# fmidev/RoadSurf

Measured on AMD Instinct MI355X. Metric: point_timesteps_per_s, higher is better.
Workload: dtype f64

## Files before the change

### roadsurf_amd/csrc/rs_cluster.hip

```cpp
#include <hip/hip_runtime.h>
#include <hipcub/hipcub.hpp>

#include <algorithm>

#include "rs_ens_table.hpp"
#include "rs_group_rule.hpp"
#include "rs_kernels.h"
#include "rs_state.h"

namespace {

constexpr int KEY_BITS = RS_SORT_KEY_BITS;

template <typename T>
__global__ void __launch_bounds__(RS_BLOCK) keys_kernel(const T *__restrict__ state,
                                                        int64_t np_pad, int64_t npoints,
                                                        uint32_t *keys, uint32_t *slots) {
  const int64_t s = (int64_t)blockIdx.x * RS_BLOCK + threadIdx.x;
  if (s >= npoints) return;
  double v = (double)state[(int64_t)RS_ST_BLSCORE * np_pad + s];
  if (!(v >= 0.0)) v = 0.0;
  const double top = (double)((1u << KEY_BITS) - 1u);
  keys[s] = (uint32_t)top - (uint32_t)(v > top ? top : v);
  slots[s] = (uint32_t)s;
// ... 783 lines not shown
}
}

int32_t rs_cluster_ens_waves(const RsEnsSpec *sp) {
  if (rs_ens::cols(sp) < 0) return -1;
  const int32_t entries = 64 * sp->max_members * (int32_t)(sizeof(int32_t) + sizeof(uint16_t)),
                row = ENS_ROW * sp->max_members * (int32_t)sizeof(double);
  return std::max(1, std::min(ENS_MAX_WAVES, (ENS_LDS_BUDGET - entries) / row));
}

size_t rs_cluster_ens_lds_bytes(const RsEnsSpec *sp) {
  const int32_t waves = rs_cluster_ens_waves(sp);
  if (waves < 0) return 0;
  return (size_t)sp->max_members * ((size_t)waves * ENS_ROW * sizeof(double) + 64 * (sizeof(int32_t) + sizeof(uint16_t)));
}

hipError_t rs_cluster_outputs_ens(const void *const src[6], bool f32, const int32_t *table, const int32_t *inv,
                                  int64_t npoints, int64_t src_stride, int32_t nrows, const RsEnsSpec &spec,
                                  double *acc_row0, hipStream_t stream) {
  const int32_t waves = rs_cluster_ens_waves(&spec);
  if (waves < 0 || nrows < 1 || npoints < 1) return hipErrorInvalidValue;
  EnsArgs a;
  for (int f = 0; f < 6; ++f) a.src[f] = src[f];
  a.table = table;
  a.inv = inv;
  a.acc = acc_row0;
  a.npoints = npoints;
  a.stride = src_stride;
  a.nrows = nrows;
  a.ngroups = spec.ngroups;
  a.max_members = spec.max_members;
  a.nquant = spec.nquant;
  a.cols = rs_ens::cols(&spec);
  a.waves = waves;
  for (int j = 0; j < RS_ENS_MAX_QUANT; ++j) a.quant[j] = j < spec.nquant ? spec.quant[j] : 0.0;
  const int64_t station_blocks = ((int64_t)spec.ngroups + 63) / 64;
  const int64_t want_row_blocks = std::max<int64_t>(1, 6144 / station_blocks);
  const int64_t rows_each = std::max<int64_t>(1, ((int64_t)nrows + want_row_blocks - 1) / want_row_blocks);
  a.rows_per_block = (int32_t)std::min<int64_t>(INT32_MAX / 2, (rows_each + waves - 1) / waves * waves);
  const int64_t row_blocks = ((int64_t)nrows + a.rows_per_block - 1) / a.rows_per_block;
  const dim3 grid((unsigned)station_blocks, (unsigned)row_blocks);
  const size_t lds = rs_cluster_ens_lds_bytes(&spec);
  if (f32)
    hipLaunchKernelGGL(ens_stats_kernel<float>, grid, dim3(64 * waves), lds, stream, a);
  else
    hipLaunchKernelGGL(ens_stats_kernel<double>, grid, dim3(64 * waves), lds, stream, a);
  return hipGetLastError();
}

int32_t rs_cluster_prob_cols(const RsProbSpec *sp) {
  if (!sp || sp->ngroups < 1 || sp->max_members < 1 || sp->max_members > RS_ENS_MAX_MEMBERS || sp->nconds < 1 ||
      sp->nconds > RS_PROB_MAX_CONDS)
    return -1;
  for (int32_t c = 0; c < sp->nconds; ++c) {
    const RsProbCond &k = sp->cond[c];
    if (k.use <= 0 || (k.use >> RS_EPI_VARS) != 0) return -1;
    for (int v = 0; v < RS_EPI_VARS; ++v)
      if (k.above[v] != k.above[v] || k.below[v] != k.below[v]) return -1;
  }
  return 1 + 2 * sp->nconds;
}

int32_t rs_cluster_prob_needs_deficit(const RsProbSpec *sp) {
  if (rs_cluster_prob_cols(sp) < 0) return -1;
  for (int32_t c = 0; c < sp->nconds; ++c)
    if ((sp->cond[c].use >> 6) & 1) return 1;
  return 0;
}

namespace {
constexpr int PROB_ROWS = 4;
constexpr int PROB_WAVES = 4;
constexpr int PROB_WORDS = 4;

struct ProbBitsArgs {
  const void *src[RS_EPI_VARS];
  const int32_t *order;
  int32_t *ever;
  uint32_t *words;
  int64_t npoints, stride, wstride;
  int32_t nrows, nconds;
  RsProbCond cond[RS_PROB_MAX_CONDS];
};

template <typename T>
__global__ void __launch_bounds__(RS_BLOCK) prob_bits_kernel(const ProbBitsArgs a) {
  const int64_t s = (int64_t)blockIdx.x * RS_BLOCK + threadIdx.x;
  if (s >= a.npoints) return;
  const int64_t p = a.order ? (int64_t)a.order[s] : s;
  const bool own = p >= 0 && p < a.npoints;
  uint32_t ever = own ? (uint32_t)a.ever[p] : 0u;
  const bool with_deficit = a.src[6] != nullptr;
#pragma unroll 1
  for (int32_t r0 = 0; r0 < a.nrows; r0 += PROB_ROWS) {
    T x[PROB_ROWS][RS_EPI_VARS];
#pragma unroll
    for (int q = 0; q < PROB_ROWS; ++q) {
      const int32_t r = r0 + q < a.nrows ? r0 + q : a.nrows - 1;
#pragma unroll
      for (int f = 0; f < 6; ++f) x[q][f] = static_cast<const T *>(a.src[f])[(int64_t)r * a.stride + s];
      x[q][6] = with_deficit ? static_cast<const T *>(a.src[6])[(int64_t)r * a.stride + s] : (T)0;
    }
#pragma unroll
    for (int q = 0; q < PROB_ROWS; ++q) {
      if (r0 + q >= a.nrows) break;
      const double v[RS_EPI_VARS] = {(double)x[q][0], (double)x[q][1], (double)x[q][2], (double)x[q][3],
                                     (double)x[q][4], (double)x[q][5], (double)x[q][6]};
      const bool valid = v[0] != -9999.0;
      uint32_t now = 0;
#pragma unroll
      for (int c = 0; c < RS_PROB_MAX_CONDS; ++c) {
        if (c >= a.nconds) break;
        const int32_t use = a.cond[c].use;
        bool ok = valid;
#pragma unroll
        for (int k = 0; k < RS_EPI_VARS; ++k)
          if ((use >> k) & 1) ok = ok && a.cond[c].above[k] < v[k] && v[k] < a.cond[c].below[k];
        if ((use >> 6) & 1) ok = ok && v[6] != -9999.0;
        now |= (ok ? 1u : 0u) << c;
      }
      ever |= now;
      a.words[(int64_t)(r0 + q) * a.wstride + s] = valid ? (now | ((ever & 0xffu) << 8) | (1u << 16)) : 0u;
    }
  }
  if (own) a.ever[p] = (int32_t)ever;
}

struct ProbCountArgs {
  const uint32_t *words;
  const int32_t *table;
  const int32_t *inv;
  double *acc;
  int64_t npoints, wstride;
  int32_t nrows, ngroups, max_members, nconds, cols, rows_per_block;
};

__global__ void __launch_bounds__(64 * PROB_WAVES) prob_count_kernel(const ProbCountArgs a) {
  extern __shared__ int32_t prob_slot[];
  const int lane = threadIdx.x & 63, wave = threadIdx.x >> 6;
  const int64_t g = (int64_t)blockIdx.x * 64 + lane;
  const bool live = g < a.ngroups;
  int32_t first = 0, cnt = 0;
  if (live) {
    const int64_t s0 = a.table[g], s1 = a.table[g + 1];
    if (s0 >= 0 && s0 < a.npoints && s1 > s0) {
      int64_t c = s1 - s0;
      if (c > a.max_members) c = a.max_members;
      if (c > a.npoints - s0) c = a.npoints - s0;
      first = (int32_t)s0;
      cnt = (int32_t)c;
    }
  }
  int32_t incl = cnt;
#pragma unroll
  for (int d = 1; d < 64; d <<= 1) {
    const int32_t u = __shfl_up(incl, d, 64);
    if (lane >= d) incl += u;
  }
  const int32_t off = incl - cnt;
  const int32_t *entry = a.table + ((int64_t)a.ngroups + 1);
  for (int32_t j = wave; j < cnt; j += PROB_WAVES) {
    const int64_t p = entry[(int64_t)first + j];
    int32_t s = -1;
    if (p >= 0 && p < a.npoints) {
      const int64_t q = a.inv[p];
      if (q >= 0 && q < a.npoints) s = (int32_t)q;
    }
    prob_slot[off + j] = s;
  }
  __syncthreads();

  const int32_t r_lo = (int32_t)blockIdx.y * a.rows_per_block,
                r_hi = a.nrows - r_lo < a.rows_per_block ? a.nrows : r_lo + a.rows_per_block;
  const int32_t *mine = prob_slot + off;
#pragma unroll 1
  for (int32_t r = r_lo + wave; r < r_hi; r += PROB_WAVES) {
    const uint32_t *w = a.words + (int64_t)r * a.wstride;
    int32_t nvalid = 0, now[RS_PROB_MAX_CONDS], by[RS_PROB_MAX_CONDS];
#pragma unroll
    for (int c = 0; c < RS_PROB_MAX_CONDS; ++c) now[c] = by[c] = 0;
    for (int32_t j0 = 0; j0 < cnt; j0 += PROB_WORDS) {
      uint32_t x[PROB_WORDS];
#pragma unroll
      for (int q = 0; q < PROB_WORDS; ++q) {
        const int32_t s = j0 + q < cnt ? mine[j0 + q] : -1;
        x[q] = s >= 0 ? w[s] : 0u;
      }
#pragma unroll
      for (int q = 0; q < PROB_WORDS; ++q) {
        nvalid += (int32_t)((x[q] >> 16) & 1u);
#pragma unroll
        for (int c = 0; c < RS_PROB_MAX_CONDS; ++c) {
          if (c >= a.nconds) break;
          now[c] += (int32_t)((x[q] >> c) & 1u);
          by[c] += (int32_t)((x[q] >> (8 + c)) & 1u);
        }
      }
    }
    if (live) {
      double *cell = a.acc + ((int64_t)r * a.ngroups + g) * a.cols;
      cell[0] = (double)nvalid;
#pragma unroll
      for (int c = 0; c < RS_PROB_MAX_CONDS; ++c) {
        if (c >= a.nconds) break;
        cell[1 + c] = (double)now[c];
        cell[1 + a.nconds + c] = (double)by[c];
      }
    }
  }
}
}

hipError_t rs_cluster_outputs_prob(const void *const src[6], const void *deficit, bool f32, const int32_t *order,
                                   const int32_t *table, const int32_t *inv, int64_t npoints, int64_t src_stride,
                                   int32_t nrows, const RsProbSpec &spec, int32_t *ever, uint32_t *words,
                                   int64_t wstride, double *acc_row0, hipStream_t stream) {
  const int32_t cols = rs_cluster_prob_cols(&spec);
  if (cols < 0 || nrows < 1 || npoints < 1 || wstride < npoints) return hipErrorInvalidValue;
  ProbBitsArgs b;
  for (int f = 0; f < 6; ++f) b.src[f] = src[f];
  b.src[6] = rs_cluster_prob_needs_deficit(&spec) == 1 ? deficit : nullptr;
  b.order = order;
  b.ever = ever;
  b.words = words;
  b.npoints = npoints;
  b.stride = src_stride;
  b.wstride = wstride;
  b.nrows = nrows;
  b.nconds = spec.nconds;
  for (int c = 0; c < RS_PROB_MAX_CONDS; ++c) b.cond[c] = spec.cond[c < spec.nconds ? c : 0];
  if (f32)
    hipLaunchKernelGGL(prob_bits_kernel<float>, grid1(npoints), dim3(RS_BLOCK), 0, stream, b);
  else
    hipLaunchKernelGGL(prob_bits_kernel<double>, grid1(npoints), dim3(RS_BLOCK), 0, stream, b);
  if (hipError_t e = hipGetLastError(); e != hipSuccess) return e;
  ProbCountArgs a;
  a.words = words;
  a.table = table;
  a.inv = inv;
  a.acc = acc_row0;
  a.npoints = npoints;
  a.wstride = wstride;
  a.nrows = nrows;
  a.ngroups = spec.ngroups;
  a.max_members = spec.max_members;
  a.nconds = spec.nconds;
  a.cols = cols;
  const int64_t station_blocks = ((int64_t)spec.ngroups + 63) / 64;
  const int64_t want_row_blocks = std::max<int64_t>(1, 6144 / station_blocks);
  const int64_t rows_each = std::max<int64_t>(1, ((int64_t)nrows + want_row_blocks - 1) / want_row_blocks);
  a.rows_per_block = (int32_t)std::min<int64_t>(INT32_MAX / 2, (rows_each + PROB_WAVES - 1) / PROB_WAVES * PROB_WAVES);
  const int64_t row_blocks = ((int64_t)nrows + a.rows_per_block - 1) / a.rows_per_block;
  const dim3 grid((unsigned)station_blocks, (unsigned)row_blocks);
  const size_t lds = (size_t)64 * spec.max_members * sizeof(int32_t);
  hipLaunchKernelGGL(prob_count_kernel, grid, dim3(64 * PROB_WAVES), lds, stream, a);
  return hipGetLastError();
}

hipError_t rs_cluster_identity(int32_t *order, int64_t np_pad, hipStream_t stream) {
  hipLaunchKernelGGL(iota_kernel, grid1(np_pad), dim3(RS_BLOCK), 0, stream, order, np_pad);
  return hipGetLastError();
}

size_t rs_cluster_scratch_bytes(int64_t npoints) {
  size_t bytes = 0;
  uint32_t *k = nullptr;
  (void)hipcub::DeviceRadixSort::SortPairs(nullptr, bytes, k, k, k, k, (int)npoints, 0, KEY_BITS);
  return bytes;
}

hipError_t rs_cluster_sort(const double *state, bool f32, int64_t np_pad, int64_t npoints,
                           uint32_t *scratch, void *tmp, size_t tmp_bytes, hipStream_t stream) {
  uint32_t *kin = scratch, *kout = scratch + np_pad, *sin = scratch + 2 * np_pad,
           *sout = scratch + 3 * np_pad;
  if (f32)
    hipLaunchKernelGGL(keys_kernel<float>, grid1(npoints), dim3(RS_BLOCK), 0, stream,
                       reinterpret_cast<const float *>(state), np_pad, npoints, kin, sin);
  else
    hipLaunchKernelGGL(keys_kernel<double>, grid1(npoints), dim3(RS_BLOCK), 0, stream, state, np_pad,
                       npoints, kin, sin);
  hipError_t e = hipGetLastError();
  if (e != hipSuccess) return e;
  return hipcub::DeviceRadixSort::SortPairs(tmp, tmp_bytes, kin, kout, sin, sout, (int)npoints, 0,
                                            KEY_BITS, stream);
}

namespace {
constexpr int CS_TILE = 1024;

__device__ __forceinline__ uint32_t wave_incl_scan(uint32_t v, uint32_t lane) {
#pragma unroll
  for (int off = 1; off < 64; off <<= 1) {
    const uint32_t u = (uint32_t)__shfl_up((int)v, off, 64);
    if (lane >= (uint32_t)off) v += u;
  }
  return v;
}

__global__ void __launch_bounds__(256) cs_hist_kernel(const uint32_t *__restrict__ keys,
                                                      const uint32_t *__restrict__ via, int64_t n, int shift,
                                                      int nbins, int ntiles, uint32_t *__restrict__ H) {
  __builtin_amdgcn_s_setprio(3);
  extern __shared__ uint32_t cs_h[];
  for (int b = threadIdx.x; b < nbins; b += 256) cs_h[b] = 0u;
  __syncthreads();
  const int64_t base = (int64_t)blockIdx.x * CS_TILE;
  for (int i = threadIdx.x; i < CS_TILE; i += 256) {
    const int64_t idx = base + i;
    if (idx < n) atomicAdd(&cs_h[(keys[via ? (int64_t)via[idx] : idx] >> shift) & (uint32_t)(nbins - 1)], 1u);
  }
  __syncthreads();
  for (int b = threadIdx.x; b < nbins; b += 256) H[(int64_t)blockIdx.x * nbins + b] = cs_h[b];
}

__global__ void __launch_bounds__(64) cs_binscan_kernel(uint32_t *H, uint32_t *T, int nbins, int ntiles,
                                                        uint32_t *class_total, int class_shift) {
  __builtin_amdgcn_s_setprio(3);
  const int bin = (int)blockIdx.x * 64 + (int)threadIdx.x;
  uint32_t run = 0u;
  if (bin < nbins) {
#pragma unroll 8
    for (int t = 0; t < ntiles; ++t) {
      const uint32_t v = H[(int64_t)t * nbins + bin];
      H[(int64_t)t * nbins + bin] = run;
      run += v;
    }
    T[bin] = run;
  }
  if (class_total) {
    uint32_t sum = run;
#pragma unroll
    for (int off = 32; off > 0; off >>= 1) sum += (uint32_t)__shfl_xor((int)sum, off, 64);
    if (threadIdx.x == 0 && (int)blockIdx.x * 64 < nbins) atomicAdd(&class_total[((int)blockIdx.x * 64) >> class_shift], sum);
  }
}

__global__ void __launch_bounds__(64) cs_scatter_kernel(const uint32_t *__restrict__ keys,
                                                        const uint32_t *__restrict__ via, int64_t n,
                                                        int shift, int nbits, int ntiles,
                                                        const uint32_t *__restrict__ H,
                                                        const uint32_t *__restrict__ T,
                                                        uint32_t *__restrict__ perm_out) {
  __builtin_amdgcn_s_setprio(3);
  extern __shared__ uint32_t cs_cur[];
  const int nbins = 1 << nbits;
  const uint32_t lane = threadIdx.x;
  const int64_t base = (int64_t)blockIdx.x * CS_TILE;
  {
    constexpr int ROWS = 16;
    uint32_t carry = 0u;
    for (int r0 = 0; r0 < nbins; r0 += 64 * ROWS) {
      uint32_t tv[ROWS], hv[ROWS];
#pragma unroll
      for (int q = 0; q < ROWS; ++q) {
        const int b = r0 + q * 64 + (int)lane;
        tv[q] = b < nbins ? T[b] : 0u;
        hv[q] = b < nbins ? H[(int64_t)blockIdx.x * nbins + b] : 0u;
      }
#pragma unroll
      for (int q = 0; q < ROWS; ++q) {
        const int b = r0 + q * 64 + (int)lane;
        const uint32_t incl = wave_incl_scan(tv[q], lane);
        if (b < nbins) cs_cur[b] = carry + incl - tv[q] + hv[q];
        carry += (uint32_t)__shfl((int)incl, 63, 64);
      }
    }
  }
  __syncthreads();
  constexpr int CS_BATCH = 8;
  for (int r0 = 0; r0 < CS_TILE / 64; r0 += CS_BATCH) {
    if (base + (int64_t)r0 * 64 >= n) break;
    uint32_t kreg[CS_BATCH], sreg[CS_BATCH];
#pragma unroll
    for (int q = 0; q < CS_BATCH; ++q) {
      const int64_t idx = base + (int64_t)(r0 + q) * 64 + lane;
      sreg[q] = (idx < n && via) ? via[idx] : (uint32_t)idx;
    }
#pragma unroll
    for (int q = 0; q < CS_BATCH; ++q) {
      const int64_t idx = base + (int64_t)(r0 + q) * 64 + lane;
      kreg[q] = idx < n ? ((keys[sreg[q]] >> shift) & (uint32_t)(nbins - 1)) : 0u;
    }
#pragma unroll
  for (int q = 0; q < CS_BATCH; ++q) {
    const int64_t idx = base + (int64_t)(r0 + q) * 64 + lane;
    const bool valid = idx < n;
    const uint32_t key = kreg[q];
    unsigned long long same = __ballot(valid);
    for (int bit = 0; bit < nbits; ++bit) {
      const bool one = (key >> bit) & 1u;
      const unsigned long long b = __ballot(one);
      same &= one ? b : ~b;
    }
    const uint32_t rank = (uint32_t)__popcll(same & ((1ull << lane) - 1ull));
    uint32_t start = 0u;
    if (valid) {
      start = cs_cur[key];
      perm_out[start + rank] = sreg[q];
    }
    __builtin_amdgcn_wave_barrier();
    if (valid && rank == 0u) cs_cur[key] = start + (uint32_t)__popcll(same);
    __builtin_amdgcn_wave_barrier();
  }
  }
}
}

__global__ void __launch_bounds__(64) cs_wave_table_kernel(uint32_t *__restrict__ class_total,
                                                           int class_bits, int32_t *__restrict__ wstart,
                                                           int32_t *__restrict__ wcnt, int32_t maxw) {
  __builtin_amdgcn_s_setprio(3);
  const uint32_t lane = threadIdx.x;
  const int nclasses = 1 << class_bits;
  uint32_t n = 0u;
  if ((int)lane < nclasses) {
    n = class_total[lane];
    class_total[lane] = 0u;
  }
  const uint32_t waves = (n + 63u) >> 6;
  const uint32_t sbase = wave_incl_scan(n, lane) - n, wbase = wave_incl_scan(waves, lane) - waves;
  uint32_t total = 0u;
  for (int c = 0; c < nclasses; ++c) {
    const uint32_t nc = (uint32_t)__shfl((int)n, c, 64), sb = (uint32_t)__shfl((int)sbase, c, 64),
                   wb = (uint32_t)__shfl((int)wbase, c, 64), wc = (nc + 63u) >> 6;
    for (uint32_t k = lane; k < wc; k += 64u) {
      const uint32_t idx = wb + k;
      if ((int32_t)idx < maxw) {
        wstart[idx] = (int32_t)(sb + 64u * k);
        const uint32_t left = nc - 64u * k;
        wcnt[idx] = (int32_t)(left < 64u ? left : 64u);
      }
    }
    total = wb + wc;
  }
  for (uint32_t idx = total + lane; (int32_t)idx < maxw; idx += 64u) {
    wstart[idx] = 0;
    wcnt[idx] = 0;
  }
}

hipError_t rs_cluster_wave_table(int class_bits, uint32_t *class_total, int32_t *wstart, int32_t *wcnt,
                                 int32_t maxw, hipStream_t stream) {
  if (class_bits < 1 || class_bits > 6 || !class_total) return hipErrorInvalidValue;
  hipLaunchKernelGGL(cs_wave_table_kernel, dim3(1), dim3(64), 0, stream, class_total, class_bits, wstart, wcnt, maxw);
  return hipGetLastError();
}

size_t rs_cluster_count_scratch_bytes(int64_t npoints, int nbits) {
  const int64_t ntiles = (npoints + CS_TILE - 1) / CS_TILE;
  return ((size_t)(1 << nbits) * (size_t)ntiles + (size_t)(1 << nbits)) * sizeof(uint32_t);
}

hipError_t rs_cluster_count_sort(int64_t np_pad, int64_t npoints, int nbits, uint32_t *scratch, void *tmp,
                                 size_t tmp_bytes, hipStream_t stream, uint32_t *class_total, int class_bits,
                                 int low_bits) {
  if (nbits < 1 || nbits > 12 || low_bits < 0 || low_bits > 12 ||
      tmp_bytes < rs_cluster_count_scratch_bytes(npoints, nbits > low_bits ? nbits : low_bits))
    return hipErrorInvalidValue;
  const int ntiles = (int)((npoints + CS_TILE - 1) / CS_TILE);
  uint32_t *H = static_cast<uint32_t *>(tmp);
  const uint32_t *via = nullptr;
  if (low_bits > 0) {
    const int nb = 1 << low_bits;
    uint32_t *T = H + (size_t)nb * ntiles;
    hipLaunchKernelGGL(cs_hist_kernel, dim3(ntiles), dim3(256), nb * sizeof(uint32_t), stream, scratch, via,
                       npoints, 0, nb, ntiles, H);
    hipLaunchKernelGGL(cs_binscan_kernel, dim3((nb + 63) / 64), dim3(64), 0, stream, H, T, nb, ntiles,
                       (uint32_t *)nullptr, 0);
    hipLaunchKernelGGL(cs_scatter_kernel, dim3(ntiles), dim3(64), nb * sizeof(uint32_t), stream, scratch, via,
                       npoints, 0, low_bits, ntiles, H, T, scratch + np_pad);
    via = scratch + np_pad;
  }
  const int nbins = 1 << nbits;
  uint32_t *T = H + (size_t)nbins * ntiles;
  hipLaunchKernelGGL(cs_hist_kernel, dim3(ntiles), dim3(256), nbins * sizeof(uint32_t), stream, scratch, via,
                     npoints, low_bits, nbins, ntiles, H);
  const bool classes = class_total && class_bits >= 1 && nbits - class_bits >= 6;
  hipLaunchKernelGGL(cs_binscan_kernel, dim3((nbins + 63) / 64), dim3(64), 0, stream, H, T, nbins, ntiles,
                     classes ? class_total : nullptr, nbits - class_bits);
  hipLaunchKernelGGL(cs_scatter_kernel, dim3(ntiles), dim3(64), nbins * sizeof(uint32_t), stream, scratch, via,
                     npoints, low_bits, nbits, ntiles, H, T, scratch + 3 * np_pad);
  return hipGetLastError();
}

hipError_t rs_cluster_sort_keys(int64_t np_pad, int64_t npoints, uint32_t *scratch, void *tmp,
                                size_t tmp_bytes, hipStream_t stream) {
  uint32_t *kin = scratch, *kout = scratch + np_pad, *sin = scratch + 2 * np_pad,
           *sout = scratch + 3 * np_pad;
  return hipcub::DeviceRadixSort::SortPairs(tmp, tmp_bytes, kin, kout, sin, sout, (int)npoints, 0,
                                            KEY_BITS, stream);
}

namespace {
__global__ void __launch_bounds__(RS_BLOCK) again_flags_kernel(const double *__restrict__ state,
                                                               int64_t np_pad, int64_t npoints,
                                                               int32_t *flags, int32_t *iota) {
  const int64_t p = (int64_t)blockIdx.x * RS_BLOCK + threadIdx.x;
  if (p >= npoints) return;
  flags[p] = ((int32_t)state[(int64_t)RS_ST_CPL_FLAGS * np_pad + p]) & 1;
  iota[p] = (int32_t)p;
}
}

size_t rs_cpl_select_scratch_bytes(int64_t npoints) {
  size_t bytes = 0;
  int32_t *x = nullptr;
  (void)hipcub::DeviceSelect::Flagged(nullptr, bytes, x, x, x, x, (int)npoints);
  return bytes;
}

hipError_t rs_cpl_select_again(const double *state, int64_t np_pad, int64_t npoints, int32_t *flags,
                               int32_t *list, int32_t *count_dev, void *tmp, size_t tmp_bytes,
                               hipStream_t stream) {
  int32_t *iota = flags + npoints;
  hipLaunchKernelGGL(again_flags_kernel, grid1(npoints), dim3(RS_BLOCK), 0, stream, state, np_pad,
                     npoints, flags, iota);
  hipError_t e = hipGetLastError();
  if (e != hipSuccess) return e;
  return hipcub::DeviceSelect::Flagged(tmp, tmp_bytes, iota, flags, list, count_dev, (int)npoints, stream);
}

static RowMap row_map(int nlayers, int cpl_rows) {
  RowMap rows;
  rows.nlayers = nlayers;
  rows.nscal = RS_ST_BLSCORE - RS_ST_TNW1 + 1;
  rows.ncpl = cpl_rows >= 1 ? RS_ST_CPL_RESUME - RS_ST_CPL_ITER + 1 : 0;
  rows.nsave = cpl_rows >= 2 ? RS_ST_CPL_SAVE_ALBEDO - RS_ST_CPL_SAVE_TSURF + 1 : 0;
  return rows;
}

hipError_t rs_cluster_inverse(const int32_t *order, int64_t npoints, int32_t *inv, hipStream_t stream) {
  hipLaunchKernelGGL(inverse_kernel, grid1(npoints), dim3(RS_BLOCK), 0, stream, order, npoints, inv);
  return hipGetLastError();
}

hipError_t rs_cluster_fanout(const double *state_src, double *state_dst, bool f32, const int32_t *order_dst,
                             const int32_t *parent, const int32_t *inv_src, int64_t np_pad_src, int64_t npoints_src,
                             int64_t np_pad_dst, int64_t npoints_dst, int nlayers, int cpl_rows, hipStream_t stream) {
  dim3 g = grid1(npoints_dst);
  const RowMap rows = row_map(nlayers, cpl_rows);
  g.y = (unsigned)rows.total();
  if (f32)
    hipLaunchKernelGGL(fanout_kernel<float>, g, dim3(RS_BLOCK), 0, stream, reinterpret_cast<const float *>(state_src),
                       reinterpret_cast<float *>(state_dst), order_dst, parent, inv_src, np_pad_src, npoints_src,
                       np_pad_dst, npoints_dst, rows);
  else
    hipLaunchKernelGGL(fanout_kernel<double>, g, dim3(RS_BLOCK), 0, stream, state_src, state_dst, order_dst, parent,
                       inv_src, np_pad_src, npoints_src, np_pad_dst, npoints_dst, rows);
  return hipGetLastError();
}

hipError_t rs_cluster_apply(const double *state_src, double *state_dst, bool f32,
                            const int32_t *order_src, int32_t *order_dst, const uint32_t *perm,
                            int64_t np_pad, int64_t npoints, int nlayers, int cpl_rows,
                            hipStream_t stream) {
  dim3 g = grid1(np_pad);
  const RowMap rows = row_map(nlayers, cpl_rows);
  g.y = (unsigned)rows.total();
  if (f32)
    hipLaunchKernelGGL(apply_kernel<float>, g, dim3(RS_BLOCK), 0, stream,
                       reinterpret_cast<const float *>(state_src), reinterpret_cast<float *>(state_dst),
                       order_src, order_dst, perm, np_pad, npoints, rows);
  else
    hipLaunchKernelGGL(apply_kernel<double>, g, dim3(RS_BLOCK), 0, stream, state_src, state_dst,
                       order_src, order_dst, perm, np_pad, npoints, rows);
  return hipGetLastError();
}
```

### roadsurf_amd/csrc/rs_kernels.h

```cpp
#pragma once
#include <hip/hip_runtime.h>
#include <cstddef>
#include <type_traits>
#include "../../include/roadsurf.h"
#include "rs_synth.h"
#include "rs_raw.hpp"
#include "rs_step_select.hpp"

namespace rs {

struct Writeback {
  double *sw, *sw_dir, *lw;
  int64_t t_stride;
};

struct StepArgs {
  const void *consts = nullptr;
  RsForcing f{};
  RsOutputs o{};
  RsPointParams pp{};
  double *state = nullptr;
  int64_t npoints = 0, np_pad = 0;
  int32_t t0 = 0, nsteps = 0;
  Writeback wb{};
  const int32_t *cpl_list = nullptr;
  int32_t cpl_nlist = 0, cpl_stop = 0;
  int32_t cpl_inner = 0, cpl_prio = 0;
  const int32_t *out_index = nullptr;
  const int32_t *wave_start = nullptr, *wave_cnt = nullptr;
  int32_t wave_n = 0;
  int32_t knots_tdew = 0;
  int32_t surface_prio = 0;
  const double *knots = nullptr;
  const int32_t *knot_gather = nullptr;
  int32_t knot_k0 = 0, knot_n = 0, spk = 0, start_hour = 0;
  double r_spk = 0.0;
  RawForcing raw{};
  double *diag = nullptr;
};
static_assert(std::is_trivially_copyable<StepArgs>::value, "StepArgs is a kernel argument");
static_assert(sizeof(StepArgs) == 912 && offsetof(StepArgs, f) == 8 && offsetof(StepArgs, o) == 136 &&
                  offsetof(StepArgs, pp) == 208 && offsetof(StepArgs, state) == 328 && offsetof(StepArgs, t0) == 352 &&
                  offsetof(StepArgs, wb) == 360 && offsetof(StepArgs, cpl_list) == 392 &&
                  offsetof(StepArgs, out_index) == 416 && offsetof(StepArgs, wave_n) == 440 &&
                  offsetof(StepArgs, knots_tdew) == 444 && offsetof(StepArgs, surface_prio) == 448 &&
                  offsetof(StepArgs, knots) == 456 && offsetof(StepArgs, r_spk) == 488 &&
                  offsetof(StepArgs, raw) == 496 && offsetof(StepArgs, diag) == 904,
              "the kernels' view of StepArgs");

struct InitArgs {
  const void *consts;
  RsForcing f;
  RsPointParams pp;
  double *state;
  int64_t npoints, np_pad;
};

struct ForecastArgs {
  const void *consts;
  const void *state;
  int32_t f32;
  int64_t npoints, np_pad;
  RsPreview pv;
  uint32_t *keys, *slots;
  int32_t compact;
  int32_t low_bits;
  int32_t extra_log;
};

struct KnotArgs {
  RsSynthSpec spec;
  double *knots;
  int64_t npoints, np_pad;
  int32_t k0, nknots;
};

struct ExpandArgs {
  RsForcing f;
  const double *knots;
  int64_t npoints, np_pad;
  int32_t k0, t0, spk, start_hour;
  int32_t kfirst, nsteps;
  double r_spk;
  const int32_t *gather;
};

}

hipError_t rs_read_div_mismatch(unsigned long long *out , hipStream_t stream);
hipError_t rs_read_div_samples(double *out , hipStream_t stream);
hipError_t rs_read_bl_stats(unsigned long long *out , hipStream_t stream);
hipError_t rs_launch_math_test(int fn, int64_t n, const double *x, double *y, hipStream_t stream);
hipError_t rs_launch_humidity_fill(const double *tair, double *tdew, double *rhz, int64_t n,
                                   hipStream_t stream);
hipError_t rs_upload_math_tables(hipStream_t stream);
hipError_t rs_launch_step(const rs::StepArgs &a, const rs::StepLaunch &l, hipStream_t stream);
struct RsPlan;
int rs_cpl_replay_raw(RsPlan *pl, const rs::RawForcing *raw, const RsOutputs *o, const RsPointParams *pp,
                      int32_t t0, int32_t nsteps, bool out_by_point, int32_t *rounds);
uint64_t rs_a32_limit(void);
bool rs_step_raw_ok(const RsPlan *pl);
int rs_step_raw(RsPlan *pl, const rs::RawForcing *raw, const double *sun, const RsOutputs *o,
                const RsPointParams *pp, int32_t t0, int32_t nsteps, bool out_by_point);
hipError_t rs_launch_cpl_window_bounds(const rs::StepArgs &a, int32_t *out, hipStream_t stream);
size_t rs_cpl_select_scratch_bytes(int64_t npoints);
hipError_t rs_cpl_select_again(const double *state, int64_t np_pad, int64_t npoints, int32_t *flags,
                               int32_t *list, int32_t *count_dev, void *tmp, size_t tmp_bytes,
                               hipStream_t stream);
hipError_t rs_launch_init(const rs::InitArgs &a, hipStream_t stream);
hipError_t rs_launch_knots(const rs::KnotArgs &a, int32_t nknots, hipStream_t stream);
hipError_t rs_launch_expand(const rs::ExpandArgs &a, int32_t nintervals, hipStream_t stream);
#define RS_CLOCK_PROBE_MAX_US 10000u
hipError_t rs_launch_clock_probe(uint64_t *out, uint32_t spin_us, hipStream_t stream);
hipError_t rs_launch_count_failed(const double *st, int64_t np_pad, int64_t npoints,
                                  unsigned long long *out, hipStream_t stream);

hipError_t rs_launch_forecast_keys(const rs::ForecastArgs &a, hipStream_t stream);

#define RS_SORT_KEY_BITS 24
hipError_t rs_cluster_identity(int32_t *order, int64_t np_pad, hipStream_t stream);
hipError_t rs_cluster_outputs_by_point(const double *const src[6], double *const dst[6], const int32_t *order,
                                       int64_t npoints, int64_t src_stride, int32_t nrows, int64_t dst_rows,
                                       int64_t dst_row0, hipStream_t stream);
hipError_t rs_cluster_summary_reset(double *acc, int64_t np_pad, hipStream_t stream);
hipError_t rs_cluster_outputs_summary(const void *const src[6], bool f32, const int32_t *order, int64_t npoints,
                                      int64_t src_stride, int32_t nrows, int32_t index0, int32_t index_step,
                                      const RsSummarySpec &spec, double *acc, int64_t np_pad, hipStream_t stream);
int32_t rs_cluster_group_cols(const RsGroupSpec *spec);
int32_t rs_cluster_group_path(const RsGroupSpec *spec);
hipError_t rs_cluster_group_reset(double *acc, int64_t acc_rows, const RsGroupSpec &spec, hipStream_t stream);
hipError_t rs_cluster_outputs_groups(const void *const src[6], bool f32, const int32_t *order, const int32_t *group,
                                     int64_t npoints, int64_t src_stride, int32_t nrows, const RsGroupSpec &spec,
                                     double *acc_row0, hipStream_t stream);
int32_t rs_cluster_ens_waves(const RsEnsSpec *spec);
size_t rs_cluster_ens_lds_bytes(const RsEnsSpec *spec);
hipError_t rs_cluster_outputs_ens(const void *const src[6], bool f32, const int32_t *table, const int32_t *inv,
                                  int64_t npoints, int64_t src_stride, int32_t nrows, const RsEnsSpec &spec,
                                  double *acc_row0, hipStream_t stream);
int32_t rs_cluster_episode_cols(const RsEpisodeSpec *spec);
hipError_t rs_cluster_episodes_reset(double *acc, int64_t np_pad, const RsEpisodeSpec &spec, hipStream_t stream);
hipError_t rs_cluster_outputs_episodes(const void *const src[6], const void *deficit, bool f32, const int32_t *order,
                                       int64_t npoints, int64_t src_stride, int32_t nrows, int32_t index0,
                                       int32_t index_step, const RsEpisodeSpec &spec, double *acc, int64_t np_pad,
                                       hipStream_t stream);
hipError_t rs_cluster_episodes_finish(double *acc, int64_t npoints, int64_t np_pad, const RsEpisodeSpec &spec,
                                      hipStream_t stream);
int32_t rs_cluster_prob_cols(const RsProbSpec *spec);
int32_t rs_cluster_prob_needs_deficit(const RsProbSpec *spec);
hipError_t rs_cluster_outputs_prob(const void *const src[6], const void *deficit, bool f32, const int32_t *order,
                                   const int32_t *table, const int32_t *inv, int64_t npoints, int64_t src_stride,
                                   int32_t nrows, const RsProbSpec &spec, int32_t *ever, uint32_t *words,
                                   int64_t wstride, double *acc_row0, hipStream_t stream);
hipError_t rs_grid_gather(const double *src, int32_t nrows, int64_t n_nodes, int64_t src_stride, const int32_t *node,
                          const double *weight, int32_t stencil, const int32_t *order, double present_above,
                          double missing, double *dst, int64_t dst_stride, int64_t npoints, hipStream_t stream);
size_t rs_cluster_scratch_bytes(int64_t npoints);
hipError_t rs_cluster_sort(const double *state, bool f32, int64_t np_pad, int64_t npoints,
                           uint32_t *scratch, void *tmp, size_t tmp_bytes, hipStream_t stream);
hipError_t rs_cluster_sort_keys(int64_t np_pad, int64_t npoints, uint32_t *scratch, void *tmp,
                                size_t tmp_bytes, hipStream_t stream);
size_t rs_cluster_count_scratch_bytes(int64_t npoints, int nbits);
hipError_t rs_cluster_wave_table(int class_bits, uint32_t *class_total, int32_t *wstart, int32_t *wcnt,
                                 int32_t maxw, hipStream_t stream);
hipError_t rs_cluster_count_sort(int64_t np_pad, int64_t npoints, int nbits, uint32_t *scratch, void *tmp,
                                 size_t tmp_bytes, hipStream_t stream, uint32_t *class_total = nullptr,
                                 int class_bits = 0, int low_bits = 0);
int rs_forecast_key_bits(int32_t mode);
int rs_forecast_key_low_bits(int32_t mode);
hipError_t rs_cluster_apply(const double *state_src, double *state_dst, bool f32,
                            const int32_t *order_src, int32_t *order_dst, const uint32_t *perm,
                            int64_t np_pad, int64_t npoints, int nlayers, int cpl_rows,
                            hipStream_t stream);
hipError_t rs_cluster_inverse(const int32_t *order, int64_t npoints, int32_t *inv, hipStream_t stream);
hipError_t rs_cluster_fanout(const double *state_src, double *state_dst, bool f32, const int32_t *order_dst,
                             const int32_t *parent, const int32_t *inv_src, int64_t np_pad_src, int64_t npoints_src,
                             int64_t np_pad_dst, int64_t npoints_dst, int nlayers, int cpl_rows, hipStream_t stream);

size_t rs32_constants_bytes(void);
hipError_t rs32_upload_constants(void *dst, const RsConstants *c, hipStream_t stream);
hipError_t rs32_launch_step(const rs::StepArgs &a, const rs::StepLaunch &l, hipStream_t stream);
hipError_t rs32_launch_init(const rs::InitArgs &a, hipStream_t stream);
hipError_t rs32_launch_expand(const rs::ExpandArgs &a, int32_t nintervals, hipStream_t stream);
```

### roadsurf_amd/csrc/rs_kernels.hip

```cpp
#include <hip/hip_runtime.h>
#include <cstdlib>
#include "rs_physics.hpp"
#include "rs_state.h"
#include "rs_synth.h"
#include "rs_kernels.h"

#ifndef RS_CPL_WAVES
#define RS_CPL_WAVES 2
#endif
#ifndef RS_REGIME_WINDOW
#define RS_REGIME_WINDOW 30
#endif

namespace rs {

constexpr int kBlock = RS_BLOCK;

typedef RsConstantsDev __attribute__((address_space(4))) ConstsAS;
template <class Args>
__device__ __forceinline__ const ConstsAS &consts_of(Args a) {
  return *(const ConstsAS *)a->consts;
}

template <int NL, int NREG>
// ... 206 lines not shown
      dg[(int64_t)RS_DG_MAXIT_OLD * np + p] = old;
      dg[(int64_t)RS_DG_MAXIT_BL * np + p] = x.BLCond;
    }
    dg[(int64_t)RS_DG_MAXIT_N * np + p] = n + 1.0;
  }
}

#include "rs_general_body.inc"

template <bool FULL, class Prof, bool SKY = false, bool SCORE = true, bool CPL = false,
          bool REPLAY = false, bool A32 = false, bool DIAG = false>
__device__ __forceinline__ void time_loop(const MathTab &mt, Prof &T, Scalars &s, int32_t &score,
                                          uint32_t point = 0u) {
  static_assert(!A32 || (!SKY && !CPL), "32-bit window offsets: the plain lock-step kernels only");
  static_assert(FULL || !SKY, "sky view belongs to the FULL feature set");
  static_assert(FULL || !CPL, "coupling belongs to the FULL feature set");
  static_assert(CPL || !REPLAY, "replays belong to coupling");
  KernArgs ka = kernargs();
  const uint32_t lane = REPLAY ? point : threadIdx.x;
  const int64_t row0 = REPLAY ? 0 : (int64_t)blockIdx.x * kBlock;
  const int32_t nsteps = ka->nsteps, t0 = ka->t0;
  const double tbot = (ka->pp.tbottom + row0)[lane];
  SkyPoint sky;
  if (SKY) sky = sky_point(ka, row0, lane);
  const bool sky_on = sky.on;
  int32_t initlen = 0;
  bool relax = false;
  double relax_dt = 0, relax_dv = 0, relax_dr = 0;
  if (FULL) {
    initlen = ka->pp.initlen ? (ka->pp.initlen + row0)[lane] : 0;
    if (consts_of(ka).use_relaxation && ka->pp.tair_relax) {
      double tairR, vzR, rhR;
      relax_targets(ka, row0, lane, tairR, vzR, rhR);
      relax = !(tairR < R4(-100.0) || tairR > R4(100.0) || vzR < R4(0.0) || vzR > R4(100.0) ||
                rhR < R4(0.0) || rhR > 110);
      relax_dt = tairR - s.tair_end;
      relax_dv = vzR - s.vz_end;
      relax_dr = rhR - s.rh_end;
    }
  }

  auto fail_at = [&](int32_t idx) {
    s.failed = true;
    ka->state[(int64_t)RS_ST_FAILED * ka->np_pad + row0 + lane] = (double)idx;
  };
  CplWindow cw;
  if (CPL) cpl_window(ka, consts_of(ka), row0, lane, cw);
  const bool cpl_on = cw.on;
  const int32_t cpl_cs = cw.cs, cpl_ce = cw.ce;
  bool parked = false;
  int32_t next_i = t0;
  double cpl_lastobs = 0.0, cpl_swcorr = 0.0, cpl_lwcorr = 0.0;
  if (CPL) {
    double *st = ka->state;
    const int64_t np = ka->np_pad, p = row0 + lane;
    cpl_lastobs = st[(int64_t)RS_ST_CPL_LASTOBS * np + p];
    cpl_swcorr = st[(int64_t)RS_ST_CPL_SWCORR * np + p];
    cpl_lwcorr = st[(int64_t)RS_ST_CPL_LWCORR * np + p];
    parked = (((int32_t)st[(int64_t)RS_ST_CPL_FLAGS * np + p]) & 1) != 0;
    next_i = (int32_t)st[(int64_t)RS_ST_CPL_RESUME * np + p];
    if (REPLAY) {
      parked = false;
      next_i = cpl_cs;
    }
  }
  double r_swcof = R4(1.0), r_lwcof = R4(1.0);
  bool stale_now = false;
  auto blank_rows = [&](int32_t i_from) {
    for (int32_t ii = i_from; ii < t0 + nsteps; ++ii) {
      int64_t r;
      if (output_row<false>(ka, ii, r)) store_outputs<false, false>(ka, r, row0, lane, s, false);
    }
  };
  if (!CPL && s.failed) blank_rows(t0);
  Forcing nxt = load_forcing<FULL, A32>(ka, row0, lane, 0);
  for (int32_t kv = 0; kv < nsteps; ++kv) {
    asm volatile("" : "+s"(ka));
    const ConstsAS &c = consts_of(ka);
    const int32_t k = __builtin_amdgcn_readfirstlane(kv);
    const int32_t i = t0 + k;
    const Forcing f = nxt;
    int64_t orow = 0;
    const bool owrite = output_row<true>(ka, i, orow);

    if (CPL && (parked || i != next_i)) {
      if (k + 1 < nsteps) nxt = load_forcing<FULL, A32>(ka, row0, lane, k + 1);
      continue;
    }
    if (CPL) next_i = i + 1;
    if (s.failed) {
      if (CPL && owrite && (!REPLAY || i > cpl_ce)) store_outputs<CPL, A32>(ka, orow, row0, lane, s, false);
      continue;
    }
    double tair = f.tair, vz = f.vz, rhz = f.rhz;
    s.tnw1 = T.get(1);
    s.tnw2 = T.get(2);
    if (i == 1 && vz < R4(0.4)) vz = R4(0.4);
    const double prec_ts = RS_DIVC(f.prec, 3600.0, r_3600) * c.DTSecs;

    double sw_dir = 0.0, lw_net = 0.0;
    if (SKY) {
      const int64_t row = (int64_t)k * ka->f.t_stride + row0;
      const LaneOff L(lane);
      sw_dir = L.ld(ka->f.sw_dir + row);
      lw_net = L.ld(ka->f.lw_net + row);
    }
    CouplingInputs cp;
    if (i < c.SimLen) {
      if (REPLAY && i == cpl_cs) {
        const Forcing g = gather_forcing(ka, row0 + lane, cpl_ce + 1, t0);
        if (check_values(c, g, s.tsurf, FULL && ka->f.tdew != nullptr)) fail_at(cpl_ce + 1);
      } else {
        Forcing chk = f;
        chk.vz = vz;
        if (check_values(c, chk, s.tsurf, FULL && ka->f.tdew != nullptr)) fail_at(i);
      }
      if (SKY) {
        if (REPLAY && i == cpl_cs) {
          if (sky_on) {
            const int64_t off = (int64_t)(cpl_ce + 1 - t0) * ka->f.t_stride + row0 + lane;
            if (sky_limits_bad(ka->f.sw_dir[off], ka->f.lw_net[off])) fail_at(cpl_ce + 1);
          }
        } else if (sky_on && sky_limits_bad(sw_dir, lw_net))
          fail_at(i);
        sw_dir = sky_clamp_direct(sw_dir, f.sw);
      }
      if (CPL && cpl_on) {
        cp.in_phase = (i >= cpl_cs && i <= cpl_ce);
        if (REPLAY && i == cpl_cs) cp.in_phase = false;
        if (REPLAY && i == cpl_cs) {
          double *st = ka->state;
          const int64_t np = ka->np_pad, p = row0 + lane;
          cpl_restore_surface<true>(st, np, p, s);
          const int N = T.nlayers();
          for (int j = 1; j <= N; ++j) {
            st[(int64_t)(RS_ST_CPL_STALE_TMP0 + j - 1) * np + p] = T.get(j);
            T.set(j, st[(int64_t)(RS_ST_CPL_SAVE_TMP0 + j - 1) * np + p]);
          }
          stale_now = true;
          cpl_rewind_coefs(st[(int64_t)RS_ST_CPL_RADCOEFF * np + p], f.sw, f.lw, SKY && sky_on, r_swcof, r_lwcof);
          st[(int64_t)RS_ST_CPL_SWCOF * np + p] = r_swcof;
          st[(int64_t)RS_ST_CPL_LWCOF * np + p] = r_lwcof;
        }
        if (!REPLAY && i == cpl_cs) {
          double *st = ka->state;
          const int64_t np = ka->np_pad, p = row0 + lane;
          cpl_save_surface(st, np, p, s);
          const int N = T.nlayers();
          for (int j = 1; j <= N; ++j) st[(int64_t)(RS_ST_CPL_SAVE_TMP0 + j - 1) * np + p] = T.get(j);
        }
        if (i > cpl_ce) cpl_decayed_coefs(c, mt, i, cpl_ce, cpl_swcorr, cpl_lwcorr, cp.sw_cof, cp.lw_cof);
        if (REPLAY && i >= cpl_cs && i <= cpl_ce) {
          cp.sw_cof = r_swcof;
          cp.lw_cof = r_lwcof;
        }
        if (cp.in_phase) snow_ice_check(c, cpl_lastobs, s);
      }
      if (FULL) {
        if ((i <= initlen || c.force_tsurf) && f.tsurfobs > R4(-100.0) &&
            (!CPL || !cpl_on || i < cpl_cs)) {
          T.set(1, f.tsurfobs);
          T.set(2, f.tsurfobs);
          const double depth = (c.tsurfOutputDepth >= R4(0.0)) ? c.tsurfOutputDepth : f.depth;
          s.tsurf = surface_temperature(c, T, tbot, depth);
        }
        if (relax) {
          if (i == initlen) {
            double tairR, vzR, rhR;
            relax_targets(ka, row0, lane, tairR, vzR, rhR);
            relax_dt = tairR - tair;
            relax_dv = vzR - vz;
            relax_dr = rhR - rhz;
            double *st = ka->state;
            const int64_t np = ka->np_pad, p = row0 + lane;
            st[(int64_t)RS_ST_TAIR_END * np + p] = tair;
            st[(int64_t)RS_ST_VZ_END * np + p] = vz;
            st[(int64_t)RS_ST_RH_END * np + p] = rhz;
          }
          if (i > initlen) relax_apply(relax_factor(c, mt, i, initlen), relax_dt, relax_dv, relax_dr, tair, vz, rhz);
        }
      }
    } else {
      if (FULL) s.tsurf = surface_temperature(c, T, tbot, f.depth);
      if (CPL && cpl_on) cpl_last_values(c, mt, cw, cpl_swcorr, cpl_lwcorr, ka->state, ka->np_pad, row0 + lane, cp);
    }
    if (CPL) cp.last_tsurf_obs = cpl_lastobs;
    double sw_in = f.sw, lw_in = f.lw;
    if (SKY && sky_on) {
      int64_t hstride;
      const double *hrow = horizon_row(ka, sky.hcol, hstride);
      if (!sky_view_radiation(ka->f.sun + (int64_t)k * RS_SUN_COLS, sky.sinlat, sky.coslat, sky.lonrad, sky.coslon,
                              sky.sinlon, sky.skyv, ka->pp.albedo_surroundings, hrow, hstride, sw_in, sw_dir, lw_in, lw_net))
        fail_at(i);
    }
    if (SKY) sky_write_back(ka, k, row0, sky_on, sw_dir, sw_in, lw_in, [&](double *base, double v) { base[lane] = v; });
    if (DIAG)
      bl_diagnose(&c, mt.expT, mt.logT, mt.K, s.tsurf, tair, vz, rhz, f.hour, i, ka->diag, ka->np_pad, row0 + lane);
    const Fluxes fx =
        model_step_fluxes<SCORE>(c, mt, s, tair, vz, rhz, prec_ts, sw_in, lw_in, f.phase, f.hour, cp);
    if (SCORE) {
      score += (fx.trips & 63) - 5;
      if ((fx.trips & 64) && k >= nsteps - RS_REGIME_WINDOW) score |= 1 << 30;
    }
    if (k + 1 < nsteps) nxt = load_forcing<FULL, A32>(ka, row0, lane, k + 1);
    if (REPLAY) {
      const GlobalProfile Tstale{ka->state + (int64_t)RS_ST_CPL_STALE_TMP0 * ka->np_pad + row0 + lane,
                                 ka->np_pad};
      model_step_ground<Prof, GlobalProfile>(c, s, T, tbot, tair, fx, f.depth, cp,
                                             stale_now ? &Tstale : nullptr);
      stale_now = false;
    } else {
      model_step_ground<Prof, Prof, FULL>(c, s, T, tbot, tair, fx, f.depth, cp);
    }
    if (owrite) store_outputs<CPL, A32>(ka, orow, row0, lane, s, true);
    if (!CPL && s.failed) blank_rows(i + 1);
    if (CPL && cpl_on && i < c.SimLen && i == cpl_ce)
      cpl_window_end(ka->state, ka->np_pad, row0 + lane, cw, s, cpl_swcorr, cpl_lwcorr, cpl_lastobs, parked);
  }
  if (CPL) ka->state[(int64_t)RS_ST_CPL_RESUME * ka->np_pad + row0 + lane] = (double)next_i;
}

__device__ __forceinline__ double bl_score_key(int32_t score, const Scalars &s) {
  const int32_t extra = score & 0x3fffffff;
  const int32_t lo = extra > 0x7ffff ? 0x7ffff : extra;
  const int32_t covered = (s.wat > 0.0 || s.snow > 0.0 || s.ice > 0.0 || s.ice2 > 0.0 || s.dep > 0.0) ? 1 : 0;
  return (double)(lo | (covered << 19) | (((score >> 30) & 1) << 20));
}

template <int NL>
__device__ __forceinline__ void lane_profile(RegProfile<NL> &, double *, const StepArgs &) {}
template <int NL, int NREG>
__device__ __forceinline__ void lane_profile(HybridProfile<NL, NREG> &T, double *lds, const StepArgs &) {
  T.col = lds + threadIdx.x;
}
__device__ __forceinline__ void lane_profile(LdsProfile &T, double *lds, const StepArgs &a) {
  T.col = lds + threadIdx.x;
  T.n = consts_of(&a).NLayers;
}

template <class Prof, bool FULL, bool SKY = false, bool SCORE = true, bool CPL = false, bool REPLAY = false,
          bool A32 = false, bool DIAG = false>
__device__ __forceinline__ void step_lanes(const StepArgs &a, double *math_lds, double *prof_lds) {
  const MathTab mt = fill_math_tables(math_lds);
  __syncthreads();
  const int64_t g = (int64_t)blockIdx.x * kBlock + threadIdx.x;
  if (g >= (REPLAY ? (int64_t)a.cpl_nlist : a.npoints)) return;
  const int64_t p = REPLAY ? (int64_t)a.cpl_list[g] : g;
  if (REPLAY && a.cpl_prio) __builtin_amdgcn_s_setprio(2);
  Prof T;
  lane_profile(T, prof_lds, a);
  Scalars s;
  int32_t score = 0;
#ifdef RS_WAVE_TIMING
  constexpr bool WT = !FULL && std::is_same<Prof, RegProfile<15>>::value;
  const uint64_t wt0 = WT ? __builtin_amdgcn_s_memrealtime() : 0;
#endif
  for (int32_t rnd = 0;; ++rnd) {
    load_state<FULL>(a.state, a.np_pad, p, T, s);
    time_loop<FULL, Prof, SKY, SCORE, CPL, REPLAY, A32, DIAG>(mt, T, s, score, REPLAY ? (uint32_t)p : 0u);
    store_state<FULL>(a.state, a.np_pad, p, T, s);
    if (!REPLAY || rnd + 1 >= a.cpl_inner) break;
    if ((((int32_t)a.state[(int64_t)RS_ST_CPL_FLAGS * a.np_pad + p]) & 1) == 0) break;
  }
  if (SCORE) a.state[(int64_t)RS_ST_BLSCORE * a.np_pad + p] = bl_score_key(score, s);
#ifdef RS_WAVE_TIMING
  if (WT) {
    a.state[(int64_t)RS_ST_VZ_END * a.np_pad + p] = (double)(wt0 & 0xffffffffffffull);
    a.state[(int64_t)RS_ST_RH_END * a.np_pad + p] = (double)(__builtin_amdgcn_s_memrealtime() & 0xffffffffffffull);
  }
#endif
}

template <int NL, bool FULL, bool SCORE = true, bool A32 = false>
__global__ void __launch_bounds__(kBlock, FULL ? 3 : 4) step_kernel_reg(const StepArgs a) {
  __shared__ double math_lds[RS_MATH_LDS_DOUBLES];
  step_lanes<RegProfile<NL>, FULL, false, SCORE, false, false, A32>(a, math_lds, nullptr);
}

#ifndef RS_HYBRID_REG
#define RS_HYBRID_REG 7
#endif
template <bool SCORE, bool A32>
__global__ void __launch_bounds__(kBlock, 4) step_kernel_hybrid(const StepArgs a) {
  __shared__ double math_lds[RS_MATH_LDS_DOUBLES];
  __shared__ double prof_lds[(15 - RS_HYBRID_REG) * kBlock];
  step_lanes<HybridProfile<15, RS_HYBRID_REG>, true, false, SCORE, false, false, A32>(a, math_lds, prof_lds);
}

template <bool FULL, bool DIAG = false>
__global__ void __launch_bounds__(kBlock, 4) step_kernel_lds(const StepArgs a) {
  extern __shared__ double lds[];
  __shared__ double math_lds[RS_MATH_LDS_DOUBLES];
  step_lanes<LdsProfile, FULL, false, true, false, false, false, DIAG>(a, math_lds, lds);
}

#ifdef RS_EAIR_SURFACE
enum { PR_TAIR = 0, PR_VZ, PR_RHZ, PR_RAIN, PR_SNOW, PR_AVC, PR_SW, PR_LW, PR_OBS, PR_LEAN = PR_OBS, PR_FULL = PR_OBS + 1 };
#else
enum { PR_TAIR = 0, PR_VZ, PR_RHZ, PR_RAIN, PR_SNOW, PR_AVC, PR_EAIR, PR_SW, PR_LW, PR_OBS, PR_LEAN = PR_OBS, PR_FULL = PR_OBS + 1 };
#endif
template <int NPREP>
struct DuoMailT {
  double v[2][2][64];
  uint32_t failed[64];
  double prep[2][NPREP][64];
  uint32_t prep_bad[2][64];
};

template <bool FULL, bool SKYG = false, class Mail>
__device__ __forceinline__ void duo_put_prep(Mail &mail, int buf, uint32_t lane, const ForcingPrep &q) {
  double (*w)[64] = mail.prep[buf];
  w[PR_TAIR][lane] = q.tair; w[PR_VZ][lane] = q.vz; w[PR_RHZ][lane] = q.rhz; w[PR_RAIN][lane] = q.rain;
  w[PR_SNOW][lane] = q.snow;
  w[PR_AVC][lane] = q.AirHCap * q.AirDens;
#ifndef RS_EAIR_SURFACE
  w[PR_EAIR][lane] = q.EAir;
#endif
  if (!SKYG) {
    w[PR_SW][lane] = q.sw;
    w[PR_LW][lane] = q.lw;
  }
  if (FULL) w[PR_OBS][lane] = q.tsurfobs;
  mail.prep_bad[buf][lane] = (q.bad ? 1u : 0u) | (q.night ? 2u : 0u) | (q.bad_rw ? 8u : 0u);
}
template <bool FULL, bool SKYG = false, class C, class Mail>
__device__ __forceinline__ ForcingPrep duo_get_prep(const C &c, const Mail &mail, int buf, uint32_t lane,
                                                    const uint32_t *skyfl = nullptr) {
  const double (*w)[64] = mail.prep[buf];
  ForcingPrep q;
  q.tair = w[PR_TAIR][lane]; q.vz = w[PR_VZ][lane]; q.rhz = w[PR_RHZ][lane]; q.rain = w[PR_RAIN][lane];
  q.snow = w[PR_SNOW][lane];
  const double AirVCap = w[PR_AVC][lane];
  q.AirVCap = AirVCap;
#ifndef RS_EAIR_SURFACE
  q.EAir = w[PR_EAIR][lane];
#endif
  q.sw = w[PR_SW][lane]; q.lw = w[PR_LW][lane];
  if (FULL) q.tsurfobs = w[PR_OBS][lane];
  uint32_t flags = mail.prep_bad[buf][lane];
  if (SKYG) flags |= skyfl[buf * 64 + lane];
  {
    const double fricN = c.TrfFricNgt, fricD = c.TrFfricDay;
    q.night = (flags & 2u) != 0u;
    q.trffric = q.night ? fricN : fricD;
  }
#ifndef RS_BL_LAST
  q.PsychC = R4(0.1) * (R4(0.00063) * (q.tair + R4(273.15)) + R4(0.47496));
#endif
  q.den0 = AirVCap * (q.tair + R4(273.15));
  q.vkvz = c.VK_Const * q.vz;
  q.avk = AirVCap * c.VK_Const;
  q.bad = (flags & 1u) != 0u;
  q.stop = SKYG && (flags & 4u) != 0u;
  q.bad_rw = (flags & 8u) != 0u;
  return q;
}

__device__ __forceinline__ void duo_meet() { asm volatile("s_waitcnt lgkmcnt(0)\n\ts_barrier" ::: "memory"); }

template <int NL, bool SCORE, bool FULL = false, bool SKY = false, bool SKYG = false, bool OUTIDX = false,
          bool CPL = false, bool REPLAY = false>
__device__ __forceinline__ void duo_surface(const MathTab &mt, DuoMailT<FULL ? PR_FULL : PR_LEAN> &mail, const StepArgs &a,
                                            const uint32_t *skyfl = nullptr) {
  static_assert(FULL || !SKY, "sky view belongs to the FULL feature set");
  static_assert(!(SKY && SKYG), "the sky view is this wave's or the ground wave's");
  static_assert(FULL || !CPL, "coupling belongs to the FULL feature set");
  static_assert(CPL || !REPLAY, "replays belong to coupling");
  KernArgs ka = kernargs();
  const uint32_t ml = threadIdx.x & 63u;
  const int64_t listed = REPLAY ? (int64_t)blockIdx.x * 64 + ml : 0;
  const int64_t row0 = REPLAY ? 0 : a.wave_start ? (int64_t)a.wave_start[blockIdx.x] : (int64_t)blockIdx.x * 64;
  const uint32_t lane = REPLAY ? (listed < a.cpl_nlist ? (uint32_t)a.cpl_list[listed] : 0u) : ml;
  const int64_t p = row0 + lane;
  const bool live = REPLAY ? listed < a.cpl_nlist
                           : a.wave_start ? (int32_t)lane < a.wave_cnt[blockIdx.x] : p < a.npoints;
  RegProfile<2> T;
  Scalars s;
  {
    RegProfile<NL> all;
    if (live) {
      load_state<false>(a.state, a.np_pad, p, all, s);
    } else {
      for (int j = 1; j <= NL; ++j) all.set(j, 0.0);
      s = Scalars();
      s.failed = true;
    }
    T.set(1, all.get(1));
    T.set(2, all.get(2));
  }
  SkyPoint sky;
  if (SKY && live) sky = sky_point(ka, p);
  const bool sky_on = sky.on;
  const int32_t nsteps = ka->nsteps, t0 = ka->t0;
  CplWindow cw;
  if (CPL && live) cpl_window(ka, consts_of(ka), p, 0u, cw);
  const bool cpl_on = cw.on;
  const int32_t cpl_cs = cw.cs, cpl_ce = cw.ce;
  bool parked = false;
  int32_t next_i = t0;
  double cpl_lastobs = 0.0, cpl_swcorr = 0.0, cpl_lwcorr = 0.0;
  if (CPL && live) {
    const double *st = a.state;
    const int64_t np = a.np_pad;
    cpl_lastobs = st[(int64_t)RS_ST_CPL_LASTOBS * np + p];
    cpl_swcorr = st[(int64_t)RS_ST_CPL_SWCORR * np + p];
    cpl_lwcorr = st[(int64_t)RS_ST_CPL_LWCORR * np + p];
    parked = (((int32_t)st[(int64_t)RS_ST_CPL_FLAGS * np + p]) & 1) != 0;
    next_i = (int32_t)st[(int64_t)RS_ST_CPL_RESUME * np + p];
    if (REPLAY) {
      parked = false;
      next_i = cpl_cs;
    }
  }
  double r_swcof = R4(1.0), r_lwcof = R4(1.0);
  mail.v[0][0][ml] = T.get(2);
  mail.failed[ml] = (s.failed || (CPL && (parked || t0 != next_i))) ? 1u : 0u;
  duo_meet();
  auto fail_at = [&](int32_t idx) {
    s.failed = true;
    ka->state[(int64_t)RS_ST_FAILED * ka->np_pad + row0 + lane] = (double)idx;
    mail.failed[ml] = 1u;
  };
  auto blank_rows = [&](int32_t i_from) {
    for (int32_t ii = i_from; ii < t0 + nsteps; ++ii) {
      int64_t r;
      if (output_row<false>(ka, ii, r)) {
        if (OUTIDX && ka->out_index) store_outputs<true, false>(ka, r, row0, lane, s, false);
        else store_outputs<false, false>(ka, r, row0, lane, s, false);
      }
    }
  };
  if (live && s.failed && !REPLAY) blank_rows(CPL && next_i > t0 ? next_i : t0);
  int32_t score = 0;
  const int32_t odec = ka->o.decimate > 1 ? ka->o.decimate : 1;
  const int64_t ostride = ka->o.t_stride;
  int32_t owait = 0;
  int64_t orow_next = 0;
  if (!OUTIDX) {
    const int32_t r = t0 - 1, m = r % odec;
    owait = __builtin_amdgcn_readfirstlane(m == 0 ? 0 : odec - m);
    const int32_t row = __builtin_amdgcn_readfirstlane(r / odec + (m == 0 ? 0 : 1));
    orow_next = ((int64_t)row - ka->o.row0) * ostride;
  }
  for (int32_t kv = 0; kv < nsteps; ++kv) {
    asm volatile("" : "+s"(ka));
    const ConstsAS &c = consts_of(ka);
    const int32_t k = __builtin_amdgcn_readfirstlane(kv);
    const int32_t i = t0 + k;
    int64_t orow = orow_next;
    bool owrite = owait == 0;
    if (OUTIDX) owrite = output_row<true>(ka, i, orow);
    double t3 = mail.v[k & 1][1][ml];
    bool go = true;
    if (CPL) {
      go = !(parked || i != next_i);
      if (go) next_i = i + 1;
    }
    if (go && !s.failed) {
      const ForcingPrep q = duo_get_prep<FULL, SKYG>(c, mail, k & 1, ml, skyfl);
      if (i < c.SimLen) {
        const bool rewind = REPLAY && i == cpl_cs;
        if ((rewind ? q.bad_rw : q.bad) | check_values_tsurf(c, s.tsurf)) fail_at(rewind ? cpl_ce + 1 : i);
      }
      if (SKYG && q.stop) fail_at(i);
      s.tnw1 = T.get(1);
      s.tnw2 = T.get(2);
      CouplingInputs cp;
      if (CPL && cpl_on) {
        if (i < c.SimLen) {
          cp.in_phase = (i >= cpl_cs && i <= cpl_ce);
          if (REPLAY && i == cpl_cs) {
            cp.in_phase = false;
            double *st = ka->state;
            const int64_t np = ka->np_pad, pp_ = row0 + lane;
            cpl_restore_surface<true>(st, np, pp_, s);
            T.set(1, st[(int64_t)(RS_ST_CPL_SAVE_TMP0 + 0) * np + pp_]);
            T.set(2, st[(int64_t)(RS_ST_CPL_SAVE_TMP0 + 1) * np + pp_]);
            t3 = st[(int64_t)(RS_ST_CPL_SAVE_TMP0 + 2) * np + pp_];
            cpl_rewind_coefs(st[(int64_t)RS_ST_CPL_RADCOEFF * np + pp_], q.sw, q.lw, false, r_swcof, r_lwcof);
            st[(int64_t)RS_ST_CPL_SWCOF * np + pp_] = r_swcof;
            st[(int64_t)RS_ST_CPL_LWCOF * np + pp_] = r_lwcof;
          }
          if (!REPLAY && i == cpl_cs) {
            double *st = ka->state;
            const int64_t np = ka->np_pad, pp_ = row0 + lane;
            cpl_save_surface(st, np, pp_, s);
            st[(int64_t)(RS_ST_CPL_SAVE_TMP0 + 0) * np + pp_] = T.get(1);
            st[(int64_t)(RS_ST_CPL_SAVE_TMP0 + 1) * np + pp_] = T.get(2);
          }
          if (i > cpl_ce) cpl_decayed_coefs(c, mt, i, cpl_ce, cpl_swcorr, cpl_lwcorr, cp.sw_cof, cp.lw_cof);
          if (REPLAY && i >= cpl_cs && i <= cpl_ce) {
            cp.sw_cof = r_swcof;
            cp.lw_cof = r_lwcof;
          }
          if (cp.in_phase) snow_ice_check(c, cpl_lastobs, s);
        } else {
          cpl_last_values(c, mt, cw, cpl_swcorr, cpl_lwcorr, ka->state, ka->np_pad, row0 + lane, cp);
        }
      }
      if (CPL) cp.last_tsurf_obs = cpl_lastobs;
      if (FULL) {
        if (i < c.SimLen) {
          if (q.tsurfobs > R4(-100.0)) {
            T.set(1, q.tsurfobs);
            T.set(2, q.tsurfobs);
            s.tsurf = (T.get(1) + T.get(2)) / R4(2.0);
          }
        } else {
          s.tsurf = (T.get(1) + T.get(2)) / R4(2.0);
        }
      }
      const double tair = q.tair;
      ForcingPrep qs = q;
      if (SKY) {
        const int64_t row = (int64_t)k * ka->f.t_stride + row0;
        const LaneOff L(lane);
        double sw_dir = L.ld(ka->f.sw_dir + row), lw_net = L.ld(ka->f.lw_net + row);
        if (i < c.SimLen) {
          if (sky_on && sky_limits_bad(sw_dir, lw_net)) fail_at(i);
          sw_dir = sky_clamp_direct(sw_dir, q.sw);
        }
        if (sky_on) {
          int64_t hstride;
          const double *hrow = horizon_row(ka, sky.hcol, hstride);
          if (!sky_view_radiation(ka->f.sun + (int64_t)k * RS_SUN_COLS, sky.sinlat, sky.coslat, sky.lonrad, sky.coslon,
                                  sky.sinlon, sky.skyv, ka->pp.albedo_surroundings, hrow, hstride, qs.sw, sw_dir, qs.lw,
                                  lw_net))
            fail_at(i);
        }
        sky_write_back(ka, k, row0, sky_on, sw_dir, qs.sw, qs.lw, [&](double *base, double v) { L.st(base, v); });
      }
      const Fluxes fx = model_step_fluxes_prepped<SCORE ? 1 : 2>(c, mt, s, qs, cp);
      if (SCORE) {
        score += (fx.trips & 63) - 5;
        if ((fx.trips & 64) && k >= nsteps - RS_REGIME_WINDOW) score |= 1 << 30;
      } else if (k == nsteps - 1) {
        score = fx.trips;
      }
      model_step_ground<RegProfile<2>, RegProfile<2>, false>(c, s, T, t3, tair, fx, R4(-9999.9), cp);
      if (owrite) {
        if (OUTIDX && ka->out_index) store_outputs<true, false>(ka, orow, row0, lane, s, true);
        else store_outputs<false, true>(ka, orow, row0, lane, s, true);
      }
      if (s.failed) blank_rows(REPLAY && cpl_ce + 1 > i + 1 ? cpl_ce + 1 : i + 1);
      if (CPL && cpl_on && i < c.SimLen && i == cpl_ce)
        cpl_window_end(ka->state, ka->np_pad, row0 + lane, cw, s, cpl_swcorr, cpl_lwcorr, cpl_lastobs, parked);
    }
    if (CPL) mail.failed[ml] = (s.failed || parked || (i + 1) != next_i) ? 1u : 0u;
    mail.v[(k & 1) ^ 1][0][ml] = T.get(2);
    if (!OUTIDX) {
      if (owrite) {
        orow_next += ostride;
        owait = odec - 1;
      } else {
        --owait;
      }
    }
    duo_meet();
  }
  if (CPL && live) a.state[(int64_t)RS_ST_CPL_RESUME * a.np_pad + p] = (double)next_i;
  if (live) {
    double *st = a.state;
    const int64_t np = a.np_pad;
    st[(int64_t)(RS_ST_TMP0 + 0) * np + p] = T.get(1);
    st[(int64_t)(RS_ST_TMP0 + 1) * np + p] = T.get(2);
    st[(int64_t)RS_ST_TNW1 * np + p] = s.tnw1;
    st[(int64_t)RS_ST_TNW2 * np + p] = s.tnw2;
    st[(int64_t)RS_ST_TSURF * np + p] = s.tsurf;
    st[(int64_t)RS_ST_WAT * np + p] = s.wat;
    st[(int64_t)RS_ST_SNOW * np + p] = s.snow;
    st[(int64_t)RS_ST_ICE * np + p] = s.ice;
    st[(int64_t)RS_ST_ICE2 * np + p] = s.ice2;
    st[(int64_t)RS_ST_DEP * np + p] = s.dep;
    st[(int64_t)RS_ST_Q2MELT * np + p] = s.q2melt;
    st[(int64_t)RS_ST_T4MELT * np + p] = s.t4melt;
    st[(int64_t)RS_ST_ALBEDO * np + p] = s.albedo;
    st[(int64_t)RS_ST_VERYCOLD * np + p] = s.verycold ? 1.0 : 0.0;
    st[(int64_t)RS_ST_BLSCORE * np + p] = SCORE ? bl_score_key(score, s) : (double)score;
  }
}

template <bool FULL>
struct KnotLerp {
  double v0[FULL ? 7 : 6], dv[FULL ? 7 : 6];
  int32_t ph0, ph1;
  int32_t spk, k, r, hour, night;
  double span, r_spk;
};
template <bool FULL>
__device__ __forceinline__ void knot_begin(KernArgs ka, KnotLerp<FULL> &K, int32_t i0) {
  K.spk = ka->spk;
  {
    const uint64_t u = (uint64_t)__double_as_longlong((double)K.spk);
    const uint32_t lo = __builtin_amdgcn_readfirstlane((uint32_t)u), hi = __builtin_amdgcn_readfirstlane((uint32_t)(u >> 32));
    K.span = __longlong_as_double((long long)(((uint64_t)hi << 32) | lo));
  }
  K.r_spk = ka->r_spk;
  const int32_t t = i0 - 1;
  K.k = __builtin_amdgcn_readfirstlane(t / K.spk);
  K.r = t - K.k * K.spk;
  K.hour = 0;
  K.night = 0;
}
template <bool FULL>
__device__ __forceinline__ Forcing knot_forcing(KernArgs ka, int64_t col, bool live, KnotLerp<FULL> &K,
                                                int32_t &kcur, int32_t i) {
  const int32_t k = K.k, r = K.r;
  if (k != kcur) {
    kcur = k;
    const ConstsAS &c = consts_of(ka);
    K.hour = (k + ka->start_hour) % 24;
    const bool night = ((double)K.hour >= c.NightOn) || ((double)K.hour <= c.NightOff);
    K.night = __builtin_amdgcn_readfirstlane(night ? 1 : 0);
    const int fld[7] = {0, 2, 3, 4, 5, 6, 1};
    const int64_t np = ka->np_pad;
    const double *ka_ = ka->knots + ((int64_t)(k - ka->knot_k0) * RS_KNOT_FIELDS) * np + col;
    const bool has_b = (k + 1 - ka->knot_k0) < ka->knot_n;
    const double *kb_ = ka_ + (int64_t)RS_KNOT_FIELDS * np;
#pragma unroll
    for (int q = 0; q < (FULL ? 7 : 6); ++q) {
      K.v0[q] = live ? ka_[(int64_t)fld[q] * np] : 0.0;
      const double v1 = (live && has_b) ? kb_[(int64_t)fld[q] * np] : K.v0[q];
      K.dv[q] = v1 - K.v0[q];
    }
    K.ph0 = live ? (int32_t)ka_[8 * np] : 0;
    K.ph1 = (live && has_b) ? (int32_t)kb_[8 * np] : K.ph0;
  }
  const int32_t spk = FULL ? ka->spk : K.spk;
  const double secs = (double)r, span = FULL ? (double)spk : K.span, r_spk = FULL ? ka->r_spk : K.r_spk;
  Forcing f;
  f.tair = K.v0[0] + rs_div_u(secs * K.dv[0], span, r_spk);
  f.vz = K.v0[1] + rs_div_u(secs * K.dv[1], span, r_spk);
  f.rhz = K.v0[2] + rs_div_u(secs * K.dv[2], span, r_spk);
  f.prec = K.v0[3] + rs_div_u(secs * K.dv[3], span, r_spk);
  f.sw = K.v0[4] + rs_div_u(secs * K.dv[4], span, r_spk);
  f.lw = K.v0[5] + rs_div_u(secs * K.dv[5], span, r_spk);
  f.phase = (r == 0) ? K.ph0 : K.ph1;
  f.hour = K.hour;
  f.tdew = 0.0;
  f.tsurfobs = R4(-9999.9);
  if (FULL) {
    f.tdew = K.v0[6] + rs_div_u(secs * K.dv[6], span, r_spk);
    if (i == 1 && live) f.tsurfobs = (ka->knots + ((int64_t)(k - ka->knot_k0) * RS_KNOT_FIELDS + 7) * ka->np_pad)[col];
  }
  f.depth = R4(-9999.9);
  K.r = r + 1;
  if (K.r == spk) {
    K.r = 0;
    K.k = k + 1;
  }
  return f;
}

enum { FSET_ALL = 0, FSET_GROUND = 1, FSET_SKY = 2 };
__device__ __forceinline__ constexpr int raw_nfields(int fset) { return fset == FSET_ALL ? 8 : fset == FSET_GROUND ? 6 : 4; }
__device__ __forceinline__ constexpr int raw_field_of(int fset, int q) {
  return fset == FSET_SKY ? (q == 0 ? RAW_SW : q == 1 ? RAW_LW : q == 2 ? RAW_SWDIR : RAW_LWNET)
                          : (q == 0 ? RAW_TAIR : q == 1 ? RAW_VZ : q == 2 ? RAW_RHZ : q == 3 ? RAW_PREC
                             : q == 4 ? RAW_TDEW : q == 5 ? RAW_OBS : q == 6 ? RAW_SW : RAW_LW);
}
constexpr int kRawObs = 5;
template <int NF>
struct RawLerp {
  double v0[NF], dv[NF];
  uint64_t mode;
  int32_t single;
  int32_t seg, seg_end;
  uint32_t mixed, imask;
  uint32_t wsel;
};

__device__ __forceinline__ double raw_slow_value(KernArgs ka, int fld, int64_t col, int32_t i) {
  const double thr = raw_threshold(fld);
  double v = raw_miss();
  const int nsrc = ka->raw.nsrc;
  const int64_t np = ka->raw.np_pad;
  for (int s = 0; s < nsrc; ++s) {
    const double *x = ka->raw.src[s].fld[fld];
    if (!x) continue;
    const RawPlanStep st = raw_plan_at(ka->raw.src[s].plan, i);
    if (st.kind == RAW_NONE) continue;
    const double a = x[(int64_t)st.rp * np + col], b = x[(int64_t)(st.rp + 1) * np + col];
    double vs;
    if (raw_source_value(st, a, b, thr, vs)) v = vs;
  }
  return v;
}

template <int FSET>
__device__ __forceinline__ void raw_resolve(KernArgs ka, int64_t col, bool live, RawLerp<raw_nfields(FSET)> &R) {
  constexpr int NF = raw_nfields(FSET);
  const RawSeg __attribute__((address_space(4))) *sg =
      (const RawSeg __attribute__((address_space(4))) *)ka->raw.segs + R.seg;
  R.seg_end = sg->i1;
  const int32_t i0 = sg->i0;
  const int nsrc = ka->raw.nsrc;
  const int64_t np = ka->raw.np_pad;
  uint64_t mode = 0;
  uint32_t mixed = 0u, imask = 0u, wsel = 0u;
  for (int s = 0; s < nsrc; ++s)
    if (sg->kind[s] == RAW_INTERP) imask |= 1u << s;
#pragma unroll
  for (int q = 0; q < NF; ++q) {
    const int fld = raw_field_of(FSET, q);
    const double thr = raw_threshold(fld);
    int32_t wl = 4;
    bool okl = true;
    double a_w = raw_miss(), d_w = 0.0;
    for (int s = 0; s < nsrc; ++s) {
      const double *x = ka->raw.src[s].fld[fld];
      const int32_t kind = sg->kind[s], rp = sg->rp[s];
      if (!x || kind == RAW_NONE) continue;
      const double *xa = x + (int64_t)rp * np + col;
      const double a = *xa;
      if (kind == RAW_COPY) {
        if (a > thr) {
          wl = 4;
          a_w = a;
          d_w = 0.0;
          okl = !rs_is_neg_zero(a);
        }
      } else {
        const double b = xa[np];
        if (a > thr && b > thr) {
          const double d = b - a;
          const double den = raw_plan_at(ka->raw.src[s].plan, i0).den;
          const double ad = __builtin_fabs(d);
          wl = s;
          a_w = a;
          d_w = d;
          okl = (__builtin_fabs(a) < __builtin_inf()) && (__builtin_fabs(b) < __builtin_inf()) &&
                (den * ad < 1e290) && (d == 0.0 || ad >= 1e-290);
        }
      }
    }
    const int32_t w0 = __builtin_amdgcn_readfirstlane(wl);
    const bool all_ok = __builtin_amdgcn_ballot_w64(live && !okl) == 0ull;
    const bool same = __builtin_amdgcn_ballot_w64(live && wl != w0) == 0ull;
    if (all_ok && same) mode |= 1ull << (10 * w0 + q);
    else if (all_ok) mixed |= 1u << q;
    else mode |= 1ull << (50 + q);
    wsel |= (uint32_t)wl << (3 * q);
    R.v0[q] = a_w;
    R.dv[q] = d_w;
  }
  R.mode = mode;
  R.mixed = mixed;
  R.imask = imask;
  R.wsel = wsel;
  int32_t single = (((mode >> 50) & 1023ull) || mixed) ? -1 : 4;
  for (int s = 0; s < RS_MAX_SOURCES; ++s)
    if ((mode >> (10 * s)) & 1023ull) single = (single == 4) ? s : -1;
  R.single = single;
}

template <int FSET>
__device__ __forceinline__ void raw_values(KernArgs ka, int64_t col, bool live, RawLerp<raw_nfields(FSET)> &R,
                                           int32_t i, bool need_obs, double (&val)[raw_nfields(FSET)]) {
  constexpr int NF = raw_nfields(FSET);
  const int32_t t = i - 1;
  if (t >= R.seg_end) {
    R.seg += 1;
    raw_resolve<FSET>(ka, col, live, R);
  }
  if (R.single >= 0) {
    double num = 0.0, den = 1.0, rden = 1.0;
    if (R.single < RS_MAX_SOURCES) {
      const RawPlanStep st = raw_plan_at(ka->raw.src[R.single].plan, t);
      num = st.num;
      den = st.den;
      rden = st.rden;
    }
    if (rden != 0.0) {
#pragma unroll
      for (int q = 0; q < NF; ++q) val[q] = R.v0[q] + raw_quot(num * R.dv[q], den, rden);
      return;
    }
  }
#pragma unroll
  for (int q = 0; q < NF; ++q) asm volatile("" : "=v"(val[q]));
  const uint32_t keep = (FSET != FSET_SKY && !need_obs) ? ~(1u << kRawObs) : ~0u;
  uint32_t slow = (uint32_t)(R.mode >> 50) & 1023u & keep;
#pragma nounroll
  for (int s = 0; s < RS_MAX_SOURCES; ++s) {
    const uint32_t m = (uint32_t)(R.mode >> (10 * s)) & 1023u & keep;
    if (m == 0u) continue;
    const RawPlanStep st = raw_plan_at(ka->raw.src[s].plan, t);
    if (st.rden == 0.0) {
      slow |= m;
      continue;
    }
#pragma unroll
    for (int q = 0; q < NF; ++q)
      if (m & (1u << q)) val[q] = R.v0[q] + raw_quot(st.num * R.dv[q], st.den, st.rden);
  }
  {
    const uint32_t m = (uint32_t)(R.mode >> 40) & 1023u & keep;
#pragma unroll
    for (int q = 0; q < NF; ++q)
      if (m & (1u << q)) val[q] = R.v0[q] + 0.0;
  }
  uint32_t mix = R.mixed & keep;
  if (mix) {
    for (int s = 0; s < RS_MAX_SOURCES; ++s)
      if ((R.imask & (1u << s)) && raw_plan_at(ka->raw.src[s].plan, t).rden == 0.0) {
        slow |= mix;
        mix = 0u;
      }
  }
  if (mix) {
#pragma unroll
    for (int q = 0; q < NF; ++q)
      if (mix & (1u << q)) val[q] = R.v0[q] + 0.0;
#pragma nounroll
    for (int s = 0; s < RS_MAX_SOURCES; ++s) {
      if (!(R.imask & (1u << s))) continue;
      const RawPlanStep st = raw_plan_at(ka->raw.src[s].plan, t);
#pragma unroll
      for (int q = 0; q < NF; ++q)
        if (mix & (1u << q)) {
          const double cand = R.v0[q] + raw_quot(st.num * R.dv[q], st.den, st.rden);
          if (((R.wsel >> (3 * q)) & 7u) == (uint32_t)s) val[q] = cand;
        }
    }
  }
  if (slow) {
#pragma unroll
    for (int q = 0; q < NF; ++q)
      if (slow & (1u << q)) val[q] = raw_slow_value(ka, raw_field_of(FSET, q), col, t);
  }
}

template <int FSET>
__device__ __forceinline__ Forcing raw_forcing(KernArgs ka, int64_t col, bool live, bool rejected,
                                               RawLerp<raw_nfields(FSET)> &R, int32_t i, bool need_obs) {
  double val[raw_nfields(FSET)];
  raw_values<FSET>(ka, col, live, R, i, need_obs, val);
  Forcing f;
  f.tair = rejected ? raw_miss() : val[0];
  f.vz = val[1];
  f.rhz = val[2];
  f.prec = val[3];
  f.tdew = val[4];
  f.tsurfobs = need_obs ? val[kRawObs] : raw_miss();
  f.sw = FSET == FSET_ALL ? val[FSET == FSET_ALL ? 6 : 0] : 0.0;
  f.lw = FSET == FSET_ALL ? val[FSET == FSET_ALL ? 7 : 0] : 0.0;
  f.phase = -9999;
  f.hour = ((const int32_t __attribute__((address_space(4))) *)ka->raw.hour)[i - 1];
  f.depth = raw_miss();
  return f;
}

enum { SRC_WINDOW = 0, SRC_KNOTS = 1, SRC_RAW = 2 };
template <int NL, int SRC = SRC_WINDOW, bool FULL = false, bool SKYG = false, bool CPL = false, bool REPLAY = false>
__device__ __forceinline__ void duo_ground(const MathTab &mt, DuoMailT<FULL ? PR_FULL : PR_LEAN> &mail, const StepArgs &a) {
  constexpr bool KNOTS = SRC == SRC_KNOTS, RAW = SRC == SRC_RAW;
  static_assert(FULL || !CPL, "coupling belongs to the FULL feature set");
  static_assert(!RAW || FULL, "the driver's series carry the FULL feature set");
  static_assert(!SKYG || RAW, "a sky wave exists only where the forcing is made from the raw series");
  static_assert(!REPLAY || (CPL && RAW && !SKYG), "replay rounds in this flavour: raw series, no sky view");
  static_assert(!KNOTS || (!CPL && !REPLAY), "the knot-reading source steps every index of the launch in order");
  KernArgs ka = kernargs();
  const uint32_t ml = threadIdx.x & 63u;
  const int64_t listed = REPLAY ? (int64_t)blockIdx.x * 64 + ml : 0;
  const int64_t row0 = REPLAY ? 0 : a.wave_start ? (int64_t)a.wave_start[blockIdx.x] : (int64_t)blockIdx.x * 64;
  const uint32_t lane = REPLAY ? (listed < a.cpl_nlist ? (uint32_t)a.cpl_list[listed] : 0u) : ml;
  const int64_t p = row0 + lane;
  const bool live = REPLAY ? listed < a.cpl_nlist
                           : a.wave_start ? (int32_t)lane < a.wave_cnt[blockIdx.x] : p < a.npoints;
  double Tg[NL - 2];
#pragma unroll
  for (int j = 3; j <= NL; ++j) Tg[j - 3] = live ? a.state[(int64_t)(RS_ST_TMP0 + j - 1) * a.np_pad + p] : 0.0;
  const double tbot = live ? ka->pp.tbottom[p] : 0.0;
  mail.v[0][1][ml] = Tg[0];
  const int32_t nsteps = ka->nsteps, t0 = ka->t0;
  int32_t initlen = 0;
  bool relax = false;
  double relax_dt = 0, relax_dv = 0, relax_dr = 0;
  auto relax_targets = [&](double &tairR, double &vzR, double &rhR) {
    tairR = (double)(float)ka->pp.tair_relax[p];
    vzR = (double)(float)ka->pp.vz_relax[p];
    rhR = (double)(float)ka->pp.rh_relax[p];
  };
  if (FULL && live) {
    initlen = ka->pp.initlen ? ka->pp.initlen[p] : 0;
    if (consts_of(ka).use_relaxation && ka->pp.tair_relax) {
      double tairR, vzR, rhR;
      relax_targets(tairR, vzR, rhR);
      relax = !(tairR < R4(-100.0) || tairR > R4(100.0) || vzR < R4(0.0) || vzR > R4(100.0) ||
                rhR < R4(0.0) || rhR > 110);
      relax_dt = tairR - a.state[(int64_t)RS_ST_TAIR_END * a.np_pad + p];
      relax_dv = vzR - a.state[(int64_t)RS_ST_VZ_END * a.np_pad + p];
      relax_dr = rhR - a.state[(int64_t)RS_ST_RH_END * a.np_pad + p];
    }
  }
  int32_t cpl_cs = 0x7fffffff, cpl_ce = 0x7ffffff0;
  if (CPL && live) {
    const int32_t cidx = ka->pp.coupling_index ? ka->pp.coupling_index[p] : 0;
    if (consts_of(ka).use_coupling && ka->pp.coupling_index && !(ka->pp.coupling_tsurf[p] < -100 || cidx < 1)) {
      cpl_cs = ((double)cidx <= consts_of(ka).cplLenR) ? 1 : cidx - consts_of(ka).cplLenI;
      cpl_ce = cidx;
    }
  }
  const int64_t rcol_ = (RAW && live) ? (ka->raw.col ? (int64_t)ka->raw.col[p] : p) : 0;
  bool anchor_due = false;
  double anchor_t = 0, anchor_v = 0, anchor_r = 0;
  double obs_cur = R4(-9999.9);
  KnotLerp<FULL> klerp;
  klerp.night = 0;
  auto prep = [&](const ConstsAS &c, const Forcing &f, int32_t in, double &obs) -> ForcingPrep {
    if (!FULL) return forcing_prep<KNOTS>(c, mt, f, in, in < c.SimLen, klerp.night != 0);
    bool bad;
    const bool has_tdew = RAW ? true : KNOTS ? (ka->knots_tdew & 2) != 0 : ka->f.tdew != nullptr;
    double vz = forcing_prep_head(c, f, in, in < c.SimLen, has_tdew, bad);
    double tair = f.tair, rhz = f.rhz;
    obs = R4(-9999.9);
    if (in < c.SimLen) {
      if ((in <= initlen || c.force_tsurf) && f.tsurfobs > R4(-100.0) && (!CPL || in < cpl_cs)) obs = f.tsurfobs;
      if (relax) {
        if (in == initlen) {
          double tairR, vzR, rhR;
          relax_targets(tairR, vzR, rhR);
          relax_dt = tairR - tair;
          relax_dv = vzR - vz;
          relax_dr = rhR - rhz;
          anchor_due = true;
          anchor_t = tair;
          anchor_v = vz;
          anchor_r = rhz;
        }
        if (in > initlen) {
          double e;
          const uint32_t d = (uint32_t)(in - initlen);
          if (c.relax_tab && d <= (uint32_t)c.SimLen) {
            e = ((const double *)c.relax_tab)[d];
          } else {
            const double den = (double)(4.f * 3600.f);
            e = rs_exp(mt, rs_div(-((c.DTSecs * in) - (c.DTSecs * initlen)), den));
          }
          tair = tair - relax_dt * e;
          vz = vz - relax_dv * e;
          rhz = rhz - relax_dr * e;
          if (rhz > R4(100.)) rhz = R4(100.0);
        }
      }
    }
    ForcingPrep q = forcing_prep_tail<KNOTS>(c, mt, f, tair, vz, rhz, bad, klerp.night != 0);
    q.tsurfobs = obs;
    if (REPLAY && live && in == cpl_cs && in < c.SimLen) {
      Forcing g = Forcing();
      const int32_t tb = cpl_ce;
      g.tair = ka->raw.status && ka->raw.status[rcol_] != 0 ? raw_miss() : raw_slow_value(ka, RAW_TAIR, rcol_, tb);
      g.vz = raw_slow_value(ka, RAW_VZ, rcol_, tb);
      g.rhz = raw_slow_value(ka, RAW_RHZ, rcol_, tb);
      g.prec = raw_slow_value(ka, RAW_PREC, rcol_, tb);
      g.sw = raw_slow_value(ka, RAW_SW, rcol_, tb);
      g.lw = raw_slow_value(ka, RAW_LW, rcol_, tb);
      g.tdew = raw_slow_value(ka, RAW_TDEW, rcol_, tb);
      q.bad_rw = check_values_forcing(c, g) | (g.tdew < -90) | (g.tdew > R4(100.0));
    }
    return q;
  };
  Forcing nxt = Forcing();
  int32_t kcur = -1;
  const int64_t kcol = (KNOTS && live) ? (ka->knot_gather ? (int64_t)ka->knot_gather[p] : p) : 0;
  constexpr int FSET = SKYG ? FSET_GROUND : FSET_ALL;
  RawLerp<raw_nfields(FSET)> rlerp;
  const int64_t rcol = rcol_;
  const bool rejected = RAW && live && ka->raw.status && ka->raw.status[rcol] != 0;
  auto obs_wanted = [&](const ConstsAS &c, int32_t in) -> bool {
    return c.force_tsurf || __builtin_amdgcn_ballot_w64(live && in <= initlen) != 0ull;
  };
  if (RAW) {
    rlerp.seg = ka->raw.seg0;
    raw_resolve<FSET>(ka, rcol, live, rlerp);
  }
  {
    const ConstsAS &c0 = consts_of(ka);
    if (KNOTS) {
      knot_begin<FULL>(ka, klerp, t0);
      nxt = knot_forcing<FULL>(ka, kcol, live, klerp, kcur, t0);
    } else if (RAW) nxt = raw_forcing<FSET>(ka, rcol, live, rejected, rlerp, t0, obs_wanted(c0, t0));
    else if (live) nxt = load_forcing<FULL, true>(ka, row0, lane, 0);
    duo_put_prep<FULL, SKYG>(mail, 0, ml, prep(c0, nxt, t0, obs_cur));
  }
  duo_meet();
  for (int32_t kv = 0; kv < nsteps; ++kv) {
    asm volatile("" : "+s"(ka));
    const ConstsAS &c = consts_of(ka);
    const int32_t k = __builtin_amdgcn_readfirstlane(kv);
    if (!KNOTS && !RAW && k + 1 < nsteps && live) nxt = load_forcing<FULL, true>(ka, row0, lane, k + 1);
    double t2 = mail.v[k & 1][0][ml];
    if (REPLAY && !mail.failed[ml] && t0 + k == cpl_cs && t0 + k < c.SimLen && live) {
      const double *sv = ka->state + (int64_t)RS_ST_CPL_SAVE_TMP0 * ka->np_pad + p;
      const int64_t np = ka->np_pad;
      double cur = sv[(int64_t)2 * np];
      double Gprev = c.lk[2].condDZ * (cur - sv[np]);
#pragma unroll
      for (int j = 3; j <= NL; ++j) {
        const double tnext = (j == NL) ? tbot : sv[(int64_t)j * np];
        const double stale = Tg[j - 3];
        Tg[j - 3] = layer_step(c, j, cur, stale, tnext, Gprev, nullptr);
        cur = tnext;
      }
    } else
    if (!mail.failed[ml]) {
      if (CPL && !REPLAY && t0 + k == cpl_cs && t0 + k < c.SimLen && live) {
#pragma unroll
        for (int j = 3; j <= NL; ++j) ka->state[(int64_t)(RS_ST_CPL_SAVE_TMP0 + j - 1) * ka->np_pad + p] = Tg[j - 3];
      }
      if (FULL) {
        if (obs_cur > R4(-100.0)) t2 = obs_cur;
        if (anchor_due && live) {
          double *st = ka->state;
          st[(int64_t)RS_ST_TAIR_END * ka->np_pad + p] = anchor_t;
          st[(int64_t)RS_ST_VZ_END * ka->np_pad + p] = anchor_v;
          st[(int64_t)RS_ST_RH_END * ka->np_pad + p] = anchor_r;
        }
      }
      double Gprev = c.lk[2].condDZ * (Tg[0] - t2);
#pragma unroll
      for (int j = 3; j <= NL; ++j) {
        const double tj = Tg[j - 3];
        const double tnext = (j == NL) ? tbot : Tg[j - 2];
        Tg[j - 3] = layer_step(c, j, tj, tj, tnext, Gprev, nullptr);
      }
    }
    if (FULL) anchor_due = false;
    mail.v[(k & 1) ^ 1][1][ml] = Tg[0];
    if (k + 1 < nsteps) {
      const int32_t in = t0 + k + 1;
      if (KNOTS) nxt = knot_forcing<FULL>(ka, kcol, live, klerp, kcur, in);
      if (RAW) nxt = raw_forcing<FSET>(ka, rcol, live, rejected, rlerp, in, obs_wanted(c, in));
      duo_put_prep<FULL, SKYG>(mail, (k & 1) ^ 1, ml, prep(c, nxt, in, obs_cur));
    }
    duo_meet();
  }
  if (live) {
#pragma unroll
    for (int j = 3; j <= NL; ++j) a.state[(int64_t)(RS_ST_TMP0 + j - 1) * a.np_pad + p] = Tg[j - 3];
  }
}

__device__ __forceinline__ void duo_sky(DuoMailT<PR_FULL> &mail, uint32_t *skyfl, const StepArgs &a) {
  KernArgs ka = kernargs();
  const uint32_t lane = threadIdx.x & 63u;
  const int64_t row0 = a.wave_start ? (int64_t)a.wave_start[blockIdx.x] : (int64_t)blockIdx.x * 64;
  const int64_t p = row0 + lane;
  const bool live = a.wave_start ? (int32_t)lane < a.wave_cnt[blockIdx.x] : p < a.npoints;
  SkyPoint sky;
  if (live) sky = sky_point(ka, p);
  const bool sky_on = sky.on;
  const int64_t rcol = live ? (ka->raw.col ? (int64_t)ka->raw.col[p] : p) : 0;
  RawLerp<4> R;
  R.seg = ka->raw.seg0;
  raw_resolve<FSET_SKY>(ka, rcol, live, R);
  const int32_t nsteps = ka->nsteps, t0 = ka->t0;
  auto put = [&](int buf, int32_t in) {
    const ConstsAS &c = consts_of(ka);
    double val[4];
    raw_values<FSET_SKY>(ka, rcol, live, R, in, false, val);
    double sw = val[0], lw = val[1], sw_dir = val[2], lw_net = val[3];
    bool bad = false, stop = false;
    if (in < c.SimLen) {
      bad = (sw < c.chk[1]) | (lw < c.chk[1]) | (sw > c.chk[5]) | (lw > c.chk[6]);
      if (sky_on && sky_limits_bad(sw_dir, lw_net)) bad = true;
      sw_dir = sky_clamp_direct(sw_dir, sw);
    }
    if (sky_on) {
      const double *sunrow = ka->f.sun + (int64_t)(in - t0) * RS_SUN_COLS;
      int64_t hstride;
      const double *hrow = horizon_row(ka, sky.hcol, hstride);
      if (!sky_view_radiation(sunrow, sky.sinlat, sky.coslat, sky.lonrad, sky.coslon, sky.sinlon, sky.skyv,
                              ka->pp.albedo_surroundings, hrow, hstride, sw, sw_dir, lw, lw_net))
        stop = true;
    }
    mail.prep[buf][PR_SW][lane] = sw;
    mail.prep[buf][PR_LW][lane] = lw;
    skyfl[buf * 64 + lane] = (bad ? 1u : 0u) | (stop ? 4u : 0u);
  };
  put(0, t0);
  duo_meet();
  for (int32_t kv = 0; kv < nsteps; ++kv) {
    asm volatile("" : "+s"(ka));
    const int32_t k = __builtin_amdgcn_readfirstlane(kv);
    if (k + 1 < nsteps) put((k & 1) ^ 1, t0 + k + 1);
    duo_meet();
  }
}

template <int NL, bool SCORE, int SRC = SRC_WINDOW, bool FULL = false, bool SKY = false, bool CPL = false,
          bool REPLAY = false>
#ifndef RS_DUO_LEAN_WAVES
#define RS_DUO_LEAN_WAVES 4
#endif
__global__ void __launch_bounds__((SKY && SRC == SRC_RAW) ? 192 : 128, REPLAY ? 3 : FULL ? 4 : RS_DUO_LEAN_WAVES) step_kernel_duo(const StepArgs a) {
  static_assert(!CPL || SRC == SRC_RAW, "coupling in the two-wavefront flavour: the driver path's lock-step chunks");
  constexpr bool SKYG = SKY && SRC == SRC_RAW;
  __shared__ double math_lds[RS_MATH_LDS_DOUBLES];
  __shared__ DuoMailT<FULL ? PR_FULL : PR_LEAN> mail;
  __shared__ uint32_t skyfl[SKYG ? 2 * 64 : 1];
  const MathTab mt = fill_math_tables(math_lds);
  __syncthreads();
  if (a.wave_start && a.wave_cnt[blockIdx.x] == 0) return;
  if (threadIdx.x < 64) {
    if (a.surface_prio) __builtin_amdgcn_s_setprio(1);
    duo_surface<NL, SCORE, FULL, SKY && !SKYG, SKYG, SRC == SRC_RAW, CPL, REPLAY>(mt, mail, a, skyfl);
  } else if (!SKYG || threadIdx.x < 128) {
    duo_ground<NL, SRC, FULL, SKYG, CPL, REPLAY>(mt, mail, a);
  } else {
    if constexpr (SKYG) duo_sky(mail, skyfl, a);
  }
}

template <bool DIAG = false>
__global__ void __launch_bounds__(kBlock, 3) step_kernel_sky(const StepArgs a) {
  extern __shared__ double lds[];
  __shared__ double math_lds[RS_MATH_LDS_DOUBLES];
  step_lanes<LdsProfile, true, true, true, false, false, false, DIAG>(a, math_lds, lds);
}

template <int W>
__global__ void __launch_bounds__(kBlock, W) step_kernel_sky_h(const StepArgs a) {
  __shared__ double math_lds[RS_MATH_LDS_DOUBLES];
  __shared__ double prof_lds[(15 - RS_HYBRID_REG) * kBlock];
  step_lanes<HybridProfile<15, RS_HYBRID_REG>, true, true>(a, math_lds, prof_lds);
}

template <bool SKY>
__global__ void __launch_bounds__(kBlock, 3) step_kernel_cpl(const StepArgs a) {
  extern __shared__ double lds[];
  __shared__ double math_lds[RS_MATH_LDS_DOUBLES];
  step_lanes<LdsProfile, true, SKY, true, true>(a, math_lds, lds);
}

template <int W, bool SKY = false>
__global__ void __launch_bounds__(kBlock, W) step_kernel_cpl_h(const StepArgs a) {
  __shared__ double math_lds[RS_MATH_LDS_DOUBLES];
  __shared__ double prof_lds[(15 - RS_HYBRID_REG) * kBlock];
  step_lanes<HybridProfile<15, RS_HYBRID_REG>, true, SKY, true, true>(a, math_lds, prof_lds);
}

template <int W, bool SKY = false>
__global__ void __launch_bounds__(kBlock, W) step_kernel_cpl_replay_h(const StepArgs a) {
  __shared__ double math_lds[RS_MATH_LDS_DOUBLES];
  __shared__ double prof_lds[(15 - RS_HYBRID_REG) * kBlock];
  step_lanes<HybridProfile<15, RS_HYBRID_REG>, true, SKY, false, true, true>(a, math_lds, prof_lds);
}

template <bool SKY>
__global__ void __launch_bounds__(kBlock, 3) step_kernel_cpl_replay(const StepArgs a) {
  extern __shared__ double lds[];
  __shared__ double math_lds[RS_MATH_LDS_DOUBLES];
  const MathTab mt = fill_math_tables(math_lds);
  __syncthreads();
  const int64_t g = (int64_t)blockIdx.x * kBlock + threadIdx.x;
  if (g >= (int64_t)a.cpl_nlist) return;
  const int64_t p = (int64_t)a.cpl_list[g];
  if (a.cpl_prio) __builtin_amdgcn_s_setprio(2);
  LdsProfile T{lds + threadIdx.x, consts_of(&a).NLayers};
  Scalars s;
  int32_t score = 0;
  for (int32_t rnd = 0;; ++rnd) {
    load_state<true>(a.state, a.np_pad, p, T, s);
    time_loop<true, LdsProfile, SKY, false, true, true>(mt, T, s, score, (uint32_t)p);
    store_state<true>(a.state, a.np_pad, p, T, s);
    if (rnd + 1 >= a.cpl_inner) break;
    if ((((int32_t)a.state[(int64_t)RS_ST_CPL_FLAGS * a.np_pad + p]) & 1) == 0) break;
  }
}

template <bool DIAG = false>
__global__ void __launch_bounds__(kBlock, RS_CPL_WAVES) step_kernel_coupled(const StepArgs a) {
  extern __shared__ double lds[];
  __shared__ double math_lds[RS_MATH_LDS_DOUBLES];
  const MathTab mt = fill_math_tables(math_lds);
  __syncthreads();
  const int64_t g = (int64_t)blockIdx.x * kBlock + threadIdx.x;
  if (g >= (a.cpl_list ? (int64_t)a.cpl_nlist : a.npoints)) return;
  const int64_t p = a.cpl_list ? (int64_t)a.cpl_list[g] : g;
  if (a.cpl_prio) __builtin_amdgcn_s_setprio(2);
  const int NLc = consts_of(&a).NLayers;
  LdsProfile T{lds + threadIdx.x, NLc};
  Scalars s;
  Coupling q;
  load_state<true>(a.state, a.np_pad, p, T, s);
  load_coupling(a.state, a.np_pad, p, q);
  time_loop_coupled<LdsProfile, DIAG>(mt, T, s, q, a.state, a.np_pad, p);
  store_state<true, LdsProfile, true>(a.state, a.np_pad, p, T, s);
  store_coupling(a.state, a.np_pad, p, q);
}

__global__ void __launch_bounds__(kBlock) synth_knots_kernel(const KnotArgs a) {
  const int64_t p = (int64_t)blockIdx.x * kBlock + threadIdx.x;
  if (p >= a.npoints) return;
  const int64_t gid = a.spec.point_offset + (a.spec.order ? (int64_t)a.spec.order[p] : p);
  const RsSynthPoint pc = rs_sy_point(a.spec.seed, gid);
  for (int32_t y = 0; y < a.nknots; ++y) {
    const RsSynthKnot q = rs_sy_knot_of(&pc, a.spec.seed, gid, a.k0 + y, a.spec.start_hour);
    double *base = a.knots + ((int64_t)y * RS_KNOT_FIELDS) * a.np_pad + p;
    base[0 * a.np_pad] = q.tair;
    base[1 * a.np_pad] = q.tdew;
    base[2 * a.np_pad] = q.vz;
    base[3 * a.np_pad] = q.rhz;
    base[4 * a.np_pad] = q.prec;
    base[5 * a.np_pad] = q.sw;
    base[6 * a.np_pad] = q.lw;
    base[7 * a.np_pad] = q.tsurf0;
    base[8 * a.np_pad] = (double)q.phase;
  }
}

__device__ __forceinline__ bool knot_interval_fast(double v0, double dv) {
  const double ad = __builtin_fabs(dv);
  return (dv == 0.0 || (ad >= 0x1p-1015 && ad < 0x1p1017)) && !(v0 == 0.0 && __builtin_signbit(v0));
}
__device__ __forceinline__ double knot_value_ieee(double v0, double dv, int32_t r, double secs, double span) {
  return r == 0 ? v0 : v0 + (secs * dv) / span;
}

__global__ void __launch_bounds__(kBlock) expand_kernel(const ExpandArgs a) {
  const bool TDEW = a.f.tdew != nullptr, OBS = a.f.tsurfobs != nullptr, DEPTH = a.f.depth != nullptr;
  __builtin_amdgcn_s_setprio(3);
  const int64_t p = (int64_t)blockIdx.x * kBlock + threadIdx.x;
  if (p >= a.npoints) return;
  const int32_t k = a.kfirst + (int32_t)blockIdx.y;
  int32_t tlo = k * a.spk, thi = tlo + a.spk;
  if (tlo < a.t0 - 1) tlo = a.t0 - 1;
  if (thi > a.t0 - 1 + a.nsteps) thi = a.t0 - 1 + a.nsteps;
  if (tlo >= thi) return;
  const int64_t kcol = a.gather ? (int64_t)a.gather[p] : p;
  const double *ka = a.knots + ((int64_t)(k - a.k0) * RS_KNOT_FIELDS) * a.np_pad + kcol;
  const double *kb = ka + (int64_t)RS_KNOT_FIELDS * a.np_pad;
  const bool need_b = (thi - 1) > k * a.spk;
  double v0[7], dv[7];
  bool fast = true;
#pragma unroll
  for (int q = 0; q < 7; ++q) {
    v0[q] = ka[(int64_t)q * a.np_pad];
    const double v1 = need_b ? kb[(int64_t)q * a.np_pad] : v0[q];
    dv[q] = v1 - v0[q];
    fast = fast && knot_interval_fast(v0[q], dv[q]);
  }
  const bool ieee = a.spk > 128 || __builtin_amdgcn_ballot_w64(!fast) != 0ull;
  const double ts0 = ka[7 * a.np_pad];
  const int32_t ph0 = (int32_t)ka[8 * a.np_pad];
  const int32_t ph1 = need_b ? (int32_t)kb[8 * a.np_pad] : ph0;
  const double span = (double)a.spk;
  const int64_t col0 = (int64_t)blockIdx.x * kBlock;
  for (int32_t t = tlo; t < thi; ++t) {
    const int32_t r = t - k * a.spk;
    const double secs = (double)r;
    const int64_t row = (int64_t)(t - (a.t0 - 1)) * a.f.t_stride + col0;
    const LaneOff L(threadIdx.x);
    double v[7];
    if (!ieee) {
#pragma unroll
      for (int q = 0; q < 7; ++q) v[q] = v0[q] + rs_div_u(secs * dv[q], span, a.r_spk);
    } else {
#pragma unroll
      for (int q = 0; q < 7; ++q) v[q] = knot_value_ieee(v0[q], dv[q], r, secs, span);
    }
    L.st((double *)a.f.tair + row, v[0]);
    if (TDEW) L.st((double *)a.f.tdew + row, v[1]);
    L.st((double *)a.f.vz + row, v[2]);
    L.st((double *)a.f.rhz + row, v[3]);
    L.st((double *)a.f.prec + row, v[4]);
    L.st((double *)a.f.sw + row, v[5]);
    L.st((double *)a.f.lw + row, v[6]);
    if (OBS) L.st((double *)a.f.tsurfobs + row, (t == 0) ? ts0 : -9999.9);
    if (DEPTH) L.st((double *)a.f.depth + row, -9999.9);
    L.st((int32_t *)a.f.precphase + row, (r == 0) ? ph0 : ph1);
  }
  if (p == 0 && !a.f.hour_pstride)
    for (int32_t t = tlo; t < thi; ++t)
      ((int32_t *)a.f.hour)[t - (a.t0 - 1)] = rs_sy_hour(t + 1, a.spk, a.start_hour);
}

__global__ void __launch_bounds__(kBlock) math_test_kernel(int fn, int64_t n, const double *x,
                                                           double *y) {
  __shared__ double math_lds[RS_MATH_LDS_DOUBLES];
  const MathTab mt = fill_math_tables(math_lds);
  __syncthreads();
  const int64_t i = (int64_t)blockIdx.x * kBlock + threadIdx.x;
  if (i >= n) return;
  if (fn == 2) y[i] = rs_div(x[i], x[n + i]);
  else if (fn == 3) y[i] = rs_sqrt(x[i]);
  else y[i] = fn == 0 ? rs_exp(mt, x[i]) : rs_log(mt, x[i]);
}

__device__ __forceinline__ double calc_tdew_or_rh(const MathTab &mt, double t, double tdew,
                                                  double rh) {
  const double Alphaw = 17.269, Alphai = 21.875, Betaw = 237.3, Betai = 265.5, AFact = 0.61078;
  const double Alpha = (t >= 0.0) ? Alphaw : Alphai;
  const double Beta = (t >= 0.0) ? Betaw : Betai;
  const double EsatT = AFact * rs_exp(mt, Alpha * t / (t + Beta));
  if (!(tdew != tdew) && tdew > -1000) {
    const double EsatTD = AFact * rs_exp(mt, Alpha * tdew / (tdew + Beta));
    const double x = (EsatTD / EsatT) * 100.0;
    return (100.0 < x) ? 100.0 : x;
  }
  if (!(rh != rh) && rh > -1) {
    const double Epr = 0.01 * rh * EsatT;
    const double XX = rs_log(mt, Epr / AFact);
    return Beta * XX / (Alpha - XX);
  }
  return __builtin_nan("");
}

__global__ void __launch_bounds__(kBlock) humidity_fill_kernel(const double *__restrict__ tair,
                                                               double *tdew, double *rhz,
                                                               int64_t n) {
  __shared__ double math_lds[RS_MATH_LDS_DOUBLES];
  const MathTab mt = fill_math_tables(math_lds);
  __syncthreads();
  const int64_t i = (int64_t)blockIdx.x * kBlock + threadIdx.x;
  if (i >= n) return;
  const double t = tair[i];
  double td = tdew[i], rh = rhz[i];
  if (td < -100 && rh > -100 && t > -100) td = calc_tdew_or_rh(mt, t, -9999.9, rh);
  if (rh < -100 && td > -100 && t > -100) rh = calc_tdew_or_rh(mt, t, td, -9999.9);
  tdew[i] = td;
  rhz[i] = rh;
}

__global__ void __launch_bounds__(kBlock) count_failed_kernel(const double *st, int64_t np_pad,
                                                              int64_t npoints,
                                                              unsigned long long *out) {
  const int64_t p = (int64_t)blockIdx.x * kBlock + threadIdx.x;
  const bool bad = p < npoints && st[(int64_t)RS_ST_FAILED * np_pad + p] != 0.0;
  const unsigned long long m = __ballot(bad);
  if ((threadIdx.x & 63) == 0 && m) atomicAdd(out, (unsigned long long)__popcll(m));
}

__global__ void __launch_bounds__(64) clock_probe_kernel(uint64_t *out, uint32_t spin_us) {
  const uint64_t c0 = __builtin_readcyclecounter();
  const uint64_t r0 = __builtin_amdgcn_s_memrealtime();
  uint64_t r1 = r0;
  bool ok = false;
  for (int it = 0; it < (1 << 16); ++it) {
    if (r1 - r0 >= (uint64_t)spin_us * 100ull) {
      ok = true;
      break;
    }
    __builtin_amdgcn_s_sleep(32);
    r1 = __builtin_amdgcn_s_memrealtime();
  }
  const uint64_t c1 = __builtin_readcyclecounter();
  if (threadIdx.x == 0) {
    out[0] = c1 - c0;
    out[1] = ok ? r1 - r0 : 0;
  }
}

__global__ void __launch_bounds__(kBlock) cpl_window_bounds_kernel(const StepArgs a, int32_t *out) {
  const int64_t p = (int64_t)blockIdx.x * kBlock + threadIdx.x;
  if (p >= a.npoints) return;
  const ConstsAS &c = consts_of(&a);
  if ((((int32_t)a.state[(int64_t)RS_ST_CPL_FLAGS * a.np_pad + p]) & 1) == 0) return;
  const int32_t cidx = a.pp.coupling_index[p];
  if (a.pp.coupling_tsurf[p] < -100 || cidx < 1) return;
  const int32_t cs = ((double)cidx <= c.cplLenR) ? 1 : cidx - c.cplLenI;
  atomicMin(&out[0], cs);
  atomicMax(&out[1], cidx);
}

__global__ void __launch_bounds__(kBlock) forecast_key_kernel(const ForecastArgs a) {
  __builtin_amdgcn_s_setprio(3);
  const int64_t s = (int64_t)blockIdx.x * kBlock + threadIdx.x;
  if (s >= a.npoints) return;
  const ConstsAS &c = consts_of(&a);
  const int64_t np = a.np_pad;
  auto st = [&](int row) -> double {
    return a.f32 ? (double)((const float *)a.state)[(int64_t)row * np + s]
                 : ((const double *)a.state)[(int64_t)row * np + s];
  };
  const double ts_now = st(RS_ST_TSURF);
  const bool has_snow = st(RS_ST_SNOW) > 0.0, has_ice = st(RS_ST_ICE) > 0.0 || st(RS_ST_ICE2) > 0.0,
             has_wet = st(RS_ST_WAT) > 0.0 || st(RS_ST_DEP) > 0.0;
  const int32_t cover = (has_snow || has_ice || has_wet) ? 1 : 0;
  const int32_t sclass = has_snow ? 3 : has_ice ? 2 : has_wet ? 1 : 0;
  const int64_t pq = a.pv.index ? (int64_t)a.pv.index[s] : s;
  auto preview = [&](const double *const *row, const double *const *row_b, int q) -> double {
    const double v = row[q][pq];
    return row_b[q] ? v + a.pv.w[q] * (row_b[q][pq] - v) : v;
  };
  const double ta_now = a.pv.tair_now ? a.pv.tair_now[pq] : preview(a.pv.tair, a.pv.tair_b, 0);
  const double stab_num = -c.VK_Const * c.ZRefT * c.Grav;
  int32_t unst = 0, farc = 0, extra = 0, maxtrip = 5;
  float stab_lo = 2.f, stab_hi = -2.f;
  for (int q = 0; q < a.pv.n; ++q) {
    const double ta = preview(a.pv.tair, a.pv.tair_b, q);
    double vz = preview(a.pv.vz, a.pv.vz_b, q);
    const double hour = (double)a.pv.hour[q];
    const double calm = (hour >= c.NightOn || hour <= c.NightOff) ? c.CalmLimNgt : c.CalmLimDay;
    if (vz < calm) vz = calm;
    const double ts = ts_now + a.pv.alpha * (ta - ta_now);
    const double TaK = ta + R4(273.15);
    const double dens = R4(100000.0) / (R4(287.05) * TaK);
    const double hcap = R4(1005.0) + (TaK - R4(250.0)) * (TaK - R4(250.0)) / R4(3364.);
    const double avc = hcap * dens;
    const float dT = (float)(ts - ta), den0 = (float)(avc * TaK), vkvz = (float)(c.VK_Const * vz),
                avk = (float)(avc * c.VK_Const), snum = (float)stab_num, lU = (float)c.logUstar,
                lC = (float)c.logCond;
    float psim = 0.f, psih = 0.f, bl = 0.f, stab_last = 0.f;
    int32_t nnear = 0, nfar = 0, j = 1;
    for (; j <= RS_BL_MAXIT; ++j) {
      const float old = bl;
      const float us = vkvz * __builtin_amdgcn_rcpf(lU + psim);
      bl = avk * us * __builtin_amdgcn_rcpf(lC + psih);
      float stab = snum * bl * dT * __builtin_amdgcn_rcpf(den0 * (us * us * us));
      if (stab > 1.f) stab = 1.f;
      stab_last = stab;
      if (stab > 0.f) {
        psih = 4.7f * stab;
        psim = psih;
      } else {
        const float arg = (1.f + __builtin_amdgcn_sqrtf(1.f - 16.f * stab)) * 0.5f;
        if (arg < 1.064453125f) ++nnear; else ++nfar;
        psih = -2.f * __logf(arg);
        psim = 0.6f * psih;
      }
      if (j >= 5 && __builtin_fabsf(bl - old) < 0.001f) break;
    }
    if (j > RS_BL_MAXIT) j = RS_BL_MAXIT;
    extra += j - 5;
    maxtrip = j > maxtrip ? j : maxtrip;
    stab_lo = stab_last < stab_lo ? stab_last : stab_lo;
    stab_hi = stab_last > stab_hi ? stab_last : stab_hi;
    if (nnear + nfar > 0) {
      ++unst;
      if (nfar >= nnear) ++farc;
    }
  }
  if (a.extra_log && stab_hi >= 1.f && stab_lo < 1.f) maxtrip = 31;
  if (a.extra_log) {
    const double last = st(RS_ST_BLSCORE);
    if (last >= 5.0 && last <= (double)RS_BL_MAXIT) {
      const int32_t lt = (int32_t)last;
      maxtrip = lt > maxtrip ? lt : maxtrip;
    }
  }
  if (extra > 4095) extra = 4095;
  uint32_t ground = 0u;
  {
    int32_t m9 = a.pv.mode;
    bool want = false;
    for (; m9 > 0; m9 /= 10) want |= (m9 % 10) == 9;
    if (want) {
      const int NL = c.NLayers;
      int32_t deepest = 0, first = 0;
      for (int j = NL; j >= 1; --j)
        if (st(RS_ST_TMP0 + j - 1) < 0.0) {
          if (!deepest) deepest = j;
          first = j;
        }
      if (NL > 15) deepest = (deepest * 15) / NL;
      const int32_t top = first > 0 ? first - 1 : 0;
      ground = ((uint32_t)deepest << 3) | (uint32_t)(top > 7 ? 7 : top);
    }
  }
  int32_t m = a.pv.mode;
  m = (m == 0) ? 14 : (m == 1) ? 124 : (m == 2) ? 134 : (m == 3) ? 1234 : m;
  int32_t div = 1;
  while (m / div >= 10) div *= 10;
  uint32_t key = 0;
  int bits = 0;
  for (; div >= 1; div /= 10) {
    const int d = (m / div) % 10;
    if (d == 1) { key = (key << 4) | (uint32_t)unst; bits += 4; }
    else if (d == 2) { key = (key << 4) | (uint32_t)farc; bits += 4; }
    else if (d == 3) { key = (key << 1) | (uint32_t)cover; bits += 1; }
    else if (d == 4) { key = (key << 12) | (uint32_t)extra; bits += 12; }
    else if (d == 5) { key = (key << 2) | (uint32_t)sclass; bits += 2; }
    else if (d == 6) { key = (key << 5) | (uint32_t)(extra > 31 ? 31 : extra); bits += 5; }
    else if (d == 0) {
      const int32_t t = maxtrip;
      const uint32_t cls = (uint32_t)(t <= 8 ? t - 5 : t <= 12 ? 4 : t <= 20 ? 5 : t <= 30 ? 6 : 7);
      key = (key << 3) | (a.extra_log ? cls : (uint32_t)(extra > 7 ? 7 : extra));
      bits += 3;
    }
    else if (d == 7) { key = (key << 2) | (uint32_t)(a.pv.n > 3 ? (unst * 3 + a.pv.n / 2) / a.pv.n : unst > 3 ? 3 : unst); bits += 2; }
    else if (d == 8) { key = (key << 2) | (uint32_t)(a.pv.n > 3 ? (farc * 3 + a.pv.n / 2) / a.pv.n : farc > 3 ? 3 : farc); bits += 2; }
  }
  if (a.pv.prec[0]) {
    uint32_t wet = 0u;
    for (int q = 0; q < RS_PREVIEW_MAX; ++q)
      if (a.pv.prec[q] && a.pv.prec[q][pq] > 0.0) wet = 1u;
    key |= wet << bits;
    bits += 1;
  }
  if (a.compact) {
    const int low = a.low_bits;
    a.keys[s] = ((((1u << bits) - 1u) - key) << low) | (low ? ground : 0u);
  } else if (a.low_bits && bits + a.low_bits <= RS_SORT_KEY_BITS) {
    const int low = a.low_bits;
    a.keys[s] = (((((1u << bits) - 1u) - key) << low) | ground) << (RS_SORT_KEY_BITS - bits - low);
  } else {
    if (bits < RS_SORT_KEY_BITS) key <<= (RS_SORT_KEY_BITS - bits);
    else key >>= (bits - RS_SORT_KEY_BITS);
    a.keys[s] = ((1u << RS_SORT_KEY_BITS) - 1u) - key;
  }
  a.slots[s] = (uint32_t)s;
}

}


static inline dim3 grid_for(int64_t n) { return dim3((unsigned)((n + RS_BLOCK - 1) / RS_BLOCK)); }

hipError_t rs_read_div_mismatch(unsigned long long *out , hipStream_t stream) {
  hipError_t e = hipMemcpyFromSymbolAsync(out, HIP_SYMBOL(rs::g_div_mismatch), 3 * sizeof(*out), 0,
                                          hipMemcpyDeviceToHost, stream);
  if (e != hipSuccess) return e;
  return hipStreamSynchronize(stream);
}

hipError_t rs_read_bl_stats(unsigned long long *out , hipStream_t stream) {
  hipError_t e = hipMemcpyFromSymbolAsync(out, HIP_SYMBOL(rs::g_bl_stats), RS_BL_NSTATS * sizeof(*out), 0,
                                          hipMemcpyDeviceToHost, stream);
  if (e != hipSuccess) return e;
  return hipStreamSynchronize(stream);
}

hipError_t rs_read_div_samples(double *out , hipStream_t stream) {
  hipError_t e = hipMemcpyFromSymbolAsync(out, HIP_SYMBOL(rs::g_div_samples), 64 * 4 * sizeof(double), 0,
                                          hipMemcpyDeviceToHost, stream);
  if (e != hipSuccess) return e;
  return hipStreamSynchronize(stream);
}

hipError_t rs_launch_math_test(int fn, int64_t n, const double *x, double *y, hipStream_t stream) {
  hipLaunchKernelGGL(rs::math_test_kernel, grid_for(n), dim3(RS_BLOCK), 0, stream, fn, n, x, y);
  return hipGetLastError();
}

hipError_t rs_launch_humidity_fill(const double *tair, double *tdew, double *rhz, int64_t n,
                                   hipStream_t stream) {
  hipLaunchKernelGGL(rs::humidity_fill_kernel, grid_for(n), dim3(RS_BLOCK), 0, stream, tair, tdew,
                     rhz, n);
  return hipGetLastError();
}

hipError_t rs_upload_math_tables(hipStream_t stream) {
  hipError_t e = hipMemcpyToSymbolAsync(HIP_SYMBOL(rs::c_gl_exp_tab), rs_gl_exp_tab,
                                        sizeof(rs_gl_exp_tab), 0, hipMemcpyHostToDevice, stream);
  if (e != hipSuccess) return e;
  return hipMemcpyToSymbolAsync(HIP_SYMBOL(rs::c_gl_log_tab), rs_gl_log_tab, sizeof(rs_gl_log_tab), 0,
                                hipMemcpyHostToDevice, stream);
}

int rs_forecast_key_low_bits(int32_t m) {
  for (; m > 0; m /= 10)
    if (m % 10 == 9) return 7;
  return 0;
}

int rs_forecast_key_bits(int32_t m) {
  m = (m == 0) ? 14 : (m == 1) ? 124 : (m == 2) ? 134 : (m == 3) ? 1234 : m;
  int bits = 0;
  for (; m > 0; m /= 10) {
    const int d = m % 10;
    bits += d == 1 ? 4 : d == 2 ? 4 : d == 3 ? 1 : d == 4 ? 12 : d == 5 ? 2 : d == 6 ? 5 : d == 7 ? 2 : d == 8 ? 2 : d == 0 ? 3 : 0;
  }
  return bits;
}

hipError_t rs_launch_forecast_keys(const rs::ForecastArgs &a, hipStream_t stream) {
  hipLaunchKernelGGL(rs::forecast_key_kernel, grid_for(a.npoints), dim3(RS_BLOCK), 0, stream, a);
  return hipGetLastError();
}

hipError_t rs_launch_step(const rs::StepArgs &a, const rs::StepLaunch &l, hipStream_t stream) {
  switch (l.kernel) {
#define RS_STEP_CASE(id, ...) \
  case rs::StepKernel::id: hipLaunchKernelGGL((__VA_ARGS__), dim3(l.grid), dim3(l.block), l.lds, stream, a); break;
    RS_STEP_KERNELS_F64(RS_STEP_CASE)
#undef RS_STEP_CASE
    default: return hipErrorInvalidValue;
  }
  return hipGetLastError();
}

hipError_t rs_launch_init(const rs::InitArgs &a, hipStream_t stream) {
  hipLaunchKernelGGL(rs::init_kernel, grid_for(a.npoints), dim3(RS_BLOCK), 0, stream, a);
  return hipGetLastError();
}

hipError_t rs_launch_knots(const rs::KnotArgs &a, int32_t nknots, hipStream_t stream) {
  rs::KnotArgs b = a;
  b.nknots = nknots;
  hipLaunchKernelGGL(rs::synth_knots_kernel, grid_for(a.npoints), dim3(RS_BLOCK), 0, stream, b);
  return hipGetLastError();
}

hipError_t rs_launch_expand(const rs::ExpandArgs &a, int32_t nintervals, hipStream_t stream) {
  dim3 g = grid_for(a.npoints);
  g.y = (unsigned)nintervals;
  hipLaunchKernelGGL(rs::expand_kernel, g, dim3(RS_BLOCK), 0, stream, a);
  return hipGetLastError();
}

hipError_t rs_launch_clock_probe(uint64_t *out, uint32_t spin_us, hipStream_t stream) {
  if (spin_us > RS_CLOCK_PROBE_MAX_US) spin_us = RS_CLOCK_PROBE_MAX_US;
  hipLaunchKernelGGL(rs::clock_probe_kernel, dim3(1), dim3(64), 0, stream, out, spin_us);
  return hipGetLastError();
}

hipError_t rs_launch_cpl_window_bounds(const rs::StepArgs &a, int32_t *out, hipStream_t stream) {
  hipLaunchKernelGGL(rs::cpl_window_bounds_kernel, grid_for(a.npoints), dim3(RS_BLOCK), 0, stream, a, out);
  return hipGetLastError();
}

hipError_t rs_launch_count_failed(const double *st, int64_t np_pad, int64_t npoints,
                                  unsigned long long *out, hipStream_t stream) {
  hipLaunchKernelGGL(rs::count_failed_kernel, grid_for(npoints), dim3(RS_BLOCK), 0, stream, st,
                     np_pad, npoints, out);
  return hipGetLastError();
}
```

### roadsurf_amd/csrc/rs_physics_body.inc

```
namespace RS_NS {

struct Scalars {
  RS_REAL tnw1, tnw2;
  RS_REAL tsurf;
  RS_REAL wat, snow, ice, ice2, dep;
  RS_REAL q2melt, t4melt, albedo;
  RS_REAL tair_end, vz_end, rh_end;
  bool verycold, failed;
};

struct Forcing {
  RS_REAL tair, tdew, vz, rhz, prec, sw, lw, tsurfobs, depth;
  int32_t phase, hour;
};

template <class Prof>
__device__ __forceinline__ RS_REAL temp_at_depth(const RS_CONSTS &c, const Prof &T, RS_REAL tbot,
                                                RS_REAL depth) {
  const int N = T.nlayers();
  if (rs_fabs(depth - R4(0.0)) < R4(0.00001)) return T.get(1);
  if (depth > c.ZDpth[N + 1]) return tbot;
  RS_REAL r = 0.0;
  bool found = false;
#pragma unroll
// ... 327 lines not shown
  return RS_LK(c, j, dryCap) + RS_LK(c, j, WCont) * CHWT;
}

template <class Prof>
__device__ __forceinline__ void melting(Scalars &s, Prof &T, RS_REAL hstor, RS_REAL hs1,
                                        bool in_coupling_phase, RS_REAL last_tsurf_obs) {
  if ((s.snow > R4(0.0)) || (s.ice > R4(0.0)) || (s.ice2 > R4(0.0))) {
    if ((hstor <= R4(0.00001)) || (s.tsurf <= s.t4melt) || (s.q2melt <= 0) ||
        (in_coupling_phase && last_tsurf_obs < s.t4melt)) {
      if (s.tsurf < R4(0.5)) {
        s.q2melt = R4(0.0);
        return;
      } else if (s.tsurf > R4(2.0)) {
        const RS_REAL QAvail = hs1 * (T.get(1) - s.t4melt);
        if (QAvail < s.q2melt) s.q2melt = QAvail;
        return;
      }
    }
    const RS_REAL QAvail = hs1 * (T.get(1) - s.t4melt);
    if (s.q2melt >= QAvail) {
      s.q2melt = QAvail;
      T.set(1, s.t4melt + R4(0.01));
      T.set(2, s.t4melt + R4(0.01));
    } else {
      const RS_REAL QLeftOver = QAvail - s.q2melt;
      T.set(1, s.t4melt + rs_div(QLeftOver, hs1));
      T.set(2, s.t4melt + R4(0.01));
    }
  } else {
    s.q2melt = R4(0.0);
  }
}

__device__ __forceinline__ void road_condition(const RS_CONSTS &c, Scalars &s, RS_REAL evap, bool real = false) {
#ifdef RS_EXP_SURFACE_LIGHT
  if (!real) {
    if (s.verycold && (s.tsurf > c.TLimColdH)) s.verycold = false;
    s.albedo = c.AlbDry;
    return;
  }
#endif
  {
    const bool bare = rs_is_pos_zero(s.wat) && rs_is_pos_zero(s.snow) && rs_is_pos_zero(s.ice) &&
                      rs_is_pos_zero(s.ice2) && rs_is_pos_zero(s.dep) && evap == R4(0.0);
#ifdef RS_BL_STATS
    {
      const unsigned long long act = __builtin_amdgcn_ballot_w64(true);
      const bool nosnow = rs_is_pos_zero(s.snow), noice = rs_is_pos_zero(s.ice) && rs_is_pos_zero(s.ice2);
      const bool nodep = rs_is_pos_zero(s.dep) && !(evap < R4(0.0)), nowat = rs_is_pos_zero(s.wat);
      const bool u11 = __builtin_amdgcn_ballot_w64(bare) == act, u12 = __builtin_amdgcn_ballot_w64(nosnow) == act,
                 u13 = __builtin_amdgcn_ballot_w64(noice) == act, u14 = __builtin_amdgcn_ballot_w64(nodep) == act,
                 u15 = __builtin_amdgcn_ballot_w64(nowat) == act,
                 u16 = __builtin_amdgcn_ballot_w64(nosnow && noice && nodep) == act;
      if ((unsigned long long)__builtin_ctzll(act) == (unsigned long long)(threadIdx.x & 63u)) {
        atomicAdd(&rs::g_bl_stats[10], 1ull);
        if (u11) atomicAdd(&rs::g_bl_stats[11], 1ull);
        if (u12) atomicAdd(&rs::g_bl_stats[12], 1ull);
        if (u13) atomicAdd(&rs::g_bl_stats[13], 1ull);
        if (u14) atomicAdd(&rs::g_bl_stats[14], 1ull);
        if (u15) atomicAdd(&rs::g_bl_stats[15], 1ull);
        if (u16) atomicAdd(&rs::g_bl_stats[16], 1ull);
      }
    }
#endif
    if (RS_BARE_FAST(c) && rs_wave_all(bare)) {
      if (s.verycold && (s.tsurf > c.TLimColdH)) s.verycold = false;
      if (!s.verycold && (s.tsurf < c.TLimColdL)) s.verycold = true;
      s.q2melt = R4(0.0);
      s.albedo = c.AlbDry;
      return;
    }
  }
#ifdef RS_NO_STORAGE_SKIP
  const bool snow_here = true;
#else
  const bool snow_here = !(RS_BARE_FAST(c) && rs_wave_all(rs_is_pos_zero(s.snow)));
#endif
  RS_REAL SnowTran = R4(0.0);
  if (snow_here) {
    SnowTran = c.wSnowTran * s.snow;
    SnowTran = (SnowTran > R4(0.01)) ? SnowTran : R4(0.01);
    if (s.snow < R4(0.2)) SnowTran = SnowTran * 3;
    SnowTran = SnowTran * c.Tph;
  }
  RS_REAL IceWear = c.wIce * s.ice;
  IceWear = (IceWear > R4(0.01)) ? IceWear : R4(0.01);
  IceWear = IceWear * c.Tph;
  RS_REAL IceWear2 = c.wIce2 * s.ice2;
  IceWear2 = (IceWear2 > R4(0.01)) ? IceWear2 : R4(0.01);
  IceWear2 = IceWear2 * c.Tph;
  RS_REAL DepWear = c.wDep * s.dep;
  DepWear = (DepWear > R4(0.01)) ? DepWear : R4(0.01);
  DepWear = DepWear * c.Tph;
  RS_REAL WatWear = c.wWat * s.wat;
  WatWear = (WatWear > R4(0.06)) ? WatWear : R4(0.06);
  WatWear = 10 * WatWear * c.Tph;

  bool wet = false;
  if (s.verycold && (s.tsurf > c.TLimColdH)) s.verycold = false;
  if (!s.verycold && (s.tsurf < c.TLimColdL)) s.verycold = true;

  if ((s.snow <= R4(0.0)) && (s.ice <= R4(0.0)) && (s.dep <= R4(0.0)) && (s.tsurf > c.TLimDew)) {
    if (s.wat > c.MaxPormms)
      s.wat = s.wat - evap;
    else
      s.wat = s.wat - c.PorEvaF * evap;
  }
  if (s.wat > R4(0.0)) {
    if (s.wat < c.WWearLim) WatWear = R4(0.0);
    if (s.wat > c.WWetLim)
      s.wat = s.wat - WatWear;
    else
      s.wat = s.wat - c.DampWearF * WatWear;
  }
  if (s.wat < c.MinWatmms) s.wat = R4(0.0);
  if (s.wat > c.MaxWatmms) s.wat = c.MaxWatmms;
  RS_REAL ext = s.wat - c.MaxPormms;
  ext = (ext > R4(0.)) ? ext : R4(0.);

  if (snow_here) {
    RS_REAL WatSnowRat;
    const RS_REAL RDummy = ext + s.snow;
    if (RDummy > R4(0.001))
      WatSnowRat = rs_div(ext, RDummy);
    else
      WatSnowRat = R4(0.0);
    if (s.snow > R4(0.0)) {
      if (WatSnowRat > c.WetSnowFormR) wet = true;
      if (s.dep > R4(0.0)) {
        s.ice = s.ice + s.dep;
        s.dep = R4(0.0);
      }
      if ((s.q2melt > R4(0.0)) && (s.tsurf >= c.TLimMeltSnow)) {
        const RS_REAL Melted = RS_DIVC(s.q2melt * c.DTSecs, RS_MELTDEN, r_meltDen);
        s.snow = s.snow - R4(1000.) * Melted;
        s.wat = s.wat + R4(1000.) * Melted;
      }
    }
    if (s.snow > R4(0.0)) {
      s.snow = s.snow - SnowTran;
      s.ice = s.ice + c.wSnow2Ice * SnowTran;
      s.ice2 = s.ice2 + c.wSnow2Ice * SnowTran;
    }
    if ((s.snow > R4(0.0)) && wet) {
      if (WatSnowRat > c.WetSnowMeltR) {
        s.wat = s.wat + s.snow;
        s.snow = R4(0.0);
      }
      if (s.tsurf < c.TLimFreeze) {
        s.ice = s.ice + s.snow + s.wat;
        s.ice2 = s.ice2 + s.snow + s.wat;
        s.snow = R4(0.0);
        s.wat = R4(0.0);
      }
    }
    if (s.snow < c.MinSnowmms) s.snow = R4(0.0);
    if (s.snow > c.MaxSnowmms) s.snow = s.snow - (c.MaxSnowmms / R4(2.));
  }

  const bool freezes = s.tsurf < c.TLimFreeze && s.wat > R4(0.0);
#ifdef RS_NO_STORAGE_SKIP
  const bool ice_here = true;
#else
  const bool ice_here = !(RS_BARE_FAST(c) && rs_wave_all(rs_is_pos_zero(s.ice) && rs_is_pos_zero(s.ice2) && !freezes));
#endif
  if (ice_here) {
    if (freezes) {
      s.ice = s.ice + s.wat;
      s.ice2 = s.ice2 + s.wat;
      s.wat = R4(0.0);
    }
    if ((s.snow <= R4(0.)) && (s.ice > R4(0.))) {
      if ((s.q2melt > R4(0.0)) && (s.tsurf >= c.TLimMeltIce)) {
        const RS_REAL Melted = RS_DIVC(s.q2melt * c.DTSecs, RS_MELTDEN, r_meltDen);
        s.ice = s.ice - R4(1000.) * Melted;
        s.ice2 = s.ice2 - R4(1000.) * Melted;
        s.wat = s.wat + R4(1000.) * Melted;
      }
    }
    if (s.ice > R4(0.)) s.ice = s.ice - IceWear;
    if (s.ice2 > R4(0.)) s.ice2 = s.ice2 - IceWear2;
    if (s.ice < c.MinIcemms) s.ice = R4(0.0);
    if (s.ice > c.MaxIcemms) s.ice = c.MaxIcemms;
    if (s.ice2 < c.MinIcemms) s.ice2 = R4(0.0);
    if (s.ice2 > c.MaxIcemms) s.ice2 = c.MaxIcemms;
  }

  if (evap < R4(0.0)) s.dep = s.dep - evap;
  if (s.tsurf > c.TLimMeltDep) {
    s.wat = s.wat + s.dep;
    s.dep = R4(0.0);
  }
  if ((s.snow <= R4(0.0)) && (s.dep > 0)) s.dep = s.dep - DepWear;
  if (s.dep < c.MinDepmms) s.dep = R4(0.0);
  if (s.dep > c.MaxDepmms) {
    s.wat = s.wat + (s.dep - c.MaxDepmms);
    s.dep = c.MaxDepmms;
  }

  if (s.wat < c.MinWatmms) s.wat = R4(0.0);
  if (s.wat > c.MaxWatmms) s.wat = c.MaxWatmms;

  if (!snow_here && !ice_here) {
    s.q2melt = R4(0.0);
    const RS_REAL IceMax = R4(1.5);
    RS_REAL alb = c.AlbDry;
    if (s.dep > R4(0.01)) {
      if (s.dep < IceMax)
        alb = c.AlbDry + RS_DIVC(s.dep, IceMax, r_IceMax) * (c.AlbSnow - c.AlbDry);
      else
        alb = c.AlbSnow;
    }
    s.albedo = alb;
    return;
  }
  s.q2melt = R4(0.0);
  if (s.snow > R4(0.0)) {
    s.q2melt = RS_DIVC(RS_MELTDEN * RS_DIVC(s.snow, R4(1000.), r_1000), c.DTSecs, r_DTSecs);
    s.t4melt = c.TLimMeltSnow;
  }
  if ((s.snow <= R4(0.0)) && (s.ice > R4(0.0))) {
    s.q2melt = RS_DIVC(RS_MELTDEN * RS_DIVC(s.ice, R4(1000.), r_1000), c.DTSecs, r_DTSecs);
    s.t4melt = c.TLimMeltIce;
  }
  if (s.q2melt < R4(0.0)) s.q2melt = R4(0.0);

  {
    RS_REAL IceSum = R4(0.5) * (s.ice + s.ice2) + s.dep;
    const RS_REAL IceMax = R4(1.5);
    if (IceSum < R4(0.0)) IceSum = R4(0.0);
    RS_REAL alb = c.AlbDry;
    if (s.snow > R4(0.01) && s.snow > s.ice) {
      alb = c.AlbSnow;
    } else if (s.ice > R4(0.01) || s.dep > R4(0.01)) {
      if (IceSum < IceMax)
        alb = c.AlbDry + RS_DIVC(IceSum, IceMax, r_IceMax) * (c.AlbSnow - c.AlbDry);
      else
        alb = c.AlbSnow;
    }
    s.albedo = alb;
  }
}

struct Fluxes {
  RS_REAL blcond, le, evap, rnet, trffric;
  int32_t trips;
};

struct CouplingInputs {
  RS_REAL sw_cof = 1.0, lw_cof = 1.0, last_tsurf_obs = 0.0;
  bool in_phase = false;
};

__device__ __forceinline__ void fluxes_pre(const RS_CONSTS &c, const MathTab &mt, Scalars &s,
                                           RS_REAL tair, RS_REAL &vz, RS_REAL rhz, RS_REAL prec_ts,
                                           int32_t phase, int32_t hour, Fluxes &fx) {
  if (!(RS_PREC_FAST(c) && rs_wave_all(prec_ts == R4(0.0))))
    precipitation_to_storage(c, mt, s, phase, prec_ts, tair, rhz);

  const RS_REAL calmN = c.CalmLimNgt, calmD = c.CalmLimDay, fricN = c.TrfFricNgt,
                fricD = c.TrFfricDay;
  const bool night = ((RS_REAL)hour >= c.NightOn) || ((RS_REAL)hour <= c.NightOff);
  const RS_REAL calm = night ? calmN : calmD;
  fx.trffric = night ? fricN : fricD;
  if (vz < calm) vz = calm;
}

__device__ __forceinline__ void fluxes_post(const RS_CONSTS &c, const Scalars &s, RS_REAL sw,
                                            RS_REAL lw, const CouplingInputs &cp, Fluxes &fx) {
  const RS_REAL TsurfK = s.tsurf + R4(273.15);
  const RS_REAL TsurfK2 = TsurfK * TsurfK;
  const RS_REAL RBB = c.Emiss * c.SB_Const * (TsurfK2 * TsurfK2);
  fx.rnet = (R4(1.) - s.albedo) * sw * cp.sw_cof + c.Emiss * lw * cp.lw_cof - RBB;
}

template <bool TRIPS = true>
__device__ __forceinline__ Fluxes model_step_fluxes(const RS_CONSTS &c, const MathTab &mt,
                                                    Scalars &s, RS_REAL tair, RS_REAL vz, RS_REAL rhz,
                                                    RS_REAL prec_ts, RS_REAL sw, RS_REAL lw,
                                                    int32_t phase, int32_t hour,
                                                    const CouplingInputs &cp = CouplingInputs()) {
  Fluxes fx;
  fluxes_pre(c, mt, s, tair, vz, rhz, prec_ts, phase, hour, fx);
  boundary_layer<TRIPS>(c, mt, s.tsurf, tair, vz, rhz, s.wat, fx.blcond, fx.le, fx.evap, fx.trips);
  fluxes_post(c, s, sw, lw, cp, fx);
  return fx;
}

struct ForcingPrep {
  RS_REAL tair, vz, rhz;
  RS_REAL rain, snow;
  RS_REAL trffric;
  RS_REAL AirDens, AirHCap, PsychC, den0, vkvz, avk;
  RS_REAL AirVCap = 0;
#ifndef RS_EAIR_SURFACE
  RS_REAL EAir;
#endif
  RS_REAL sw, lw;
  bool bad;
  bool night = false;
  bool stop = false;
  bool bad_rw = false;
  RS_REAL tsurfobs = R4(-9999.9);
};

__device__ __forceinline__ bool check_values_forcing(const RS_CONSTS &c, const Forcing &f) {
  const RS_REAL hi100 = rs_fmax(f.tair, f.vz);
  const RS_REAL lo01 = rs_fmin(rs_fmin(f.rhz, f.sw), rs_fmin(f.lw, f.prec));
  return (hi100 > RS_CHK(c, 0, R4(100.0))) | (lo01 < RS_CHK(c, 1, R4(-0.1))) |
         (f.tair < RS_CHK(c, 2, R4(-90.0))) | (f.rhz > RS_CHK(c, 3, R4(120.0))) |
         (f.vz < RS_CHK(c, 4, R4(-1.0))) | (f.sw > RS_CHK(c, 5, R4(4000.0))) |
         (f.lw > RS_CHK(c, 6, R4(1000.0))) | (f.prec > RS_CHK(c, 7, R4(500.0)));
}

__device__ __forceinline__ bool check_values_tsurf(const RS_CONSTS &c, RS_REAL tsurf) {
  return rs_fabs(tsurf) > RS_CHK(c, 0, R4(100.0));
}

__device__ __forceinline__ RS_REAL forcing_prep_head(const RS_CONSTS &c, const Forcing &f, int32_t i,
                                                     bool checked, bool has_tdew, bool &bad) {
  RS_REAL vz = f.vz;
  if (i == 1 && vz < R4(0.4)) vz = R4(0.4);
  bad = false;
  if (checked) {
    Forcing chk = f;
    chk.vz = vz;
    bad = check_values_forcing(c, chk);
    if (has_tdew) bad = bad | (f.tdew < -90) | (f.tdew > R4(100.0));
  }
  return vz;
}

__device__ __forceinline__ RS_REAL air_vapour_pressure(const MathTab &mt, RS_REAL tair, RS_REAL rhz) {
  const RS_REAL aa = (tair < 0) ? R4(21.875) : R4(17.269);
  const RS_REAL ba = (tair < 0) ? R4(265.5) : R4(237.3);
  const RS_REAL ESat = R4(0.61078) * rs_exp(mt, rs_dv<false>(aa * tair, tair + ba));
  return rs_min_num_one(R4(0.01) * rhz) * ESat;
}

template <bool NIGHT_U = false>
__device__ __forceinline__ ForcingPrep forcing_prep_tail(const RS_CONSTS &c, const MathTab &mt, const Forcing &f,
                                                         RS_REAL tair, RS_REAL vz, RS_REAL rhz, bool bad,
                                                         bool night_u = false) {
  ForcingPrep q;
  RS_REAL prec_ts = RS_DIVC(f.prec, (RS_REAL)3600.0, r_3600) * c.DTSecs;
  q.bad = bad;
  {
    Scalars z;
    z.wat = R4(0.0);
    z.snow = R4(0.0);
#ifdef RS_BL_STATS
    {
      const unsigned long long act = __builtin_amdgcn_ballot_w64(true);
      const bool dry = __builtin_amdgcn_ballot_w64(prec_ts == R4(0.0)) == act;
      if ((unsigned long long)__builtin_ctzll(act) == (unsigned long long)(threadIdx.x & 63u)) {
        atomicAdd(&rs::g_bl_stats[17], 1ull);
        if (!dry) atomicAdd(&rs::g_bl_stats[18], 1ull);
      }
    }
#endif
    if (!(RS_PREC_FAST(c) && rs_wave_all(prec_ts == R4(0.0))))
      precipitation_to_storage(c, mt, z, f.phase, prec_ts, tair, rhz);
    q.rain = z.wat;
    q.snow = z.snow;
  }
  const RS_REAL calmN = c.CalmLimNgt, calmD = c.CalmLimDay, fricN = c.TrfFricNgt, fricD = c.TrFfricDay;
  const bool night = NIGHT_U ? night_u : ((RS_REAL)f.hour >= c.NightOn) || ((RS_REAL)f.hour <= c.NightOff);
  const RS_REAL calm = night ? calmN : calmD;
  q.trffric = night ? fricN : fricD;
  q.night = night;
  if (vz < calm) vz = calm;
  q.tair = tair;
  q.vz = vz;
  q.rhz = rhz;
  const RS_REAL TaK = tair + R4(273.15);
  q.AirDens = rs_dv<false>(R4(100000.0), R4(287.05) * TaK);
  const RS_REAL dK = (TaK - R4(250.0)) * (TaK - R4(250.0));
  q.AirHCap = R4(1005.0) + RS_DIVC(dK, R4(3364.), r_3364);
  const RS_REAL AirVCap = q.AirHCap * q.AirDens;
  q.PsychC = R4(0.1) * (R4(0.00063) * TaK + R4(0.47496));
  q.den0 = AirVCap * (tair + R4(273.15));
  q.vkvz = c.VK_Const * vz;
  q.avk = AirVCap * c.VK_Const;
#ifndef RS_EAIR_SURFACE
  q.EAir = air_vapour_pressure(mt, tair, rhz);
#endif
  q.sw = f.sw;
  q.lw = f.lw;
  return q;
}

template <bool NIGHT_U = false>
__device__ __forceinline__ ForcingPrep forcing_prep(const RS_CONSTS &c, const MathTab &mt, const Forcing &f,
                                                    int32_t i, bool checked, bool night_u = false) {
  bool bad;
  const RS_REAL vz = forcing_prep_head(c, f, i, checked, false, bad);
  return forcing_prep_tail<NIGHT_U>(c, mt, f, f.tair, vz, f.rhz, bad, night_u);
}

#ifdef RS_BL_STATS
struct BlStatsStep {
  unsigned long long act;
  bool first;
};
__device__ __forceinline__ BlStatsStep bl_stats_step() {
  const unsigned long long act = __builtin_amdgcn_ballot_w64(true);
  const bool first = (unsigned long long)__builtin_ctzll(act) == (unsigned long long)(threadIdx.x & 63u);
  if (first) {
    atomicAdd(&rs::g_bl_stats[0], 1ull);
    atomicAdd(&rs::g_bl_stats[1], (unsigned long long)__builtin_popcountll(act));
  }
  return BlStatsStep{act, first};
}
__device__ __forceinline__ void bl_stats_pass(const BlStatsStep &st, int j, RS_REAL h0, const BlVar &x) {
  const unsigned long long act = st.act;
  const bool first = st.first;
  {
    const bool uns = !(x.PSIH > R4(0.0)), far = x.PSIH < R4(-0.1254);
    const unsigned long long mu = __builtin_amdgcn_ballot_w64(uns), mf = __builtin_amdgcn_ballot_w64(far),
                             ma = __builtin_amdgcn_ballot_w64(true);
    if ((unsigned long long)__builtin_ctzll(ma) == (unsigned long long)(threadIdx.x & 63u)) {
      atomicAdd(&rs::g_bl_stats[19], 1ull);
      atomicAdd(&rs::g_bl_stats[48], (unsigned long long)__builtin_popcountll(ma));
      atomicAdd(&rs::g_bl_stats[46], (unsigned long long)__builtin_popcountll(mu));
      atomicAdd(&rs::g_bl_stats[47], (unsigned long long)__builtin_popcountll(mf));
      if (mu) atomicAdd(&rs::g_bl_stats[20], 1ull);
      if (mf && (mu & ~mf)) atomicAdd(&rs::g_bl_stats[21], 1ull);
      if (mu && (ma & ~mu)) atomicAdd(&rs::g_bl_stats[22], 1ull);
      if (mf) atomicAdd(&rs::g_bl_stats[23], 1ull);
    }
  }
  if (j >= 2 && j <= 4) {
    const bool same = __double_as_longlong((double)h0) == __double_as_longlong((double)x.PSIH);
    const unsigned long long ms = __builtin_amdgcn_ballot_w64(same);
    if (first) {
      if (ms == act) atomicAdd(&rs::g_bl_stats[j], 1ull);
      atomicAdd(&rs::g_bl_stats[3 + j], (unsigned long long)__builtin_popcountll(ms));
    }
  }
}
__device__ __forceinline__ void bl_stats_trips(const BlStatsStep &st, int j) {
  const bool first = st.first;
  {
    const int trips = j > RS_BL_MAXIT ? RS_BL_MAXIT : j;
    int wmax = trips, wsum = trips;
    for (int o = 32; o > 0; o >>= 1) {
      const int other = __shfl_xor(wmax, o, 64);
      wmax = other > wmax ? other : wmax;
      wsum += __shfl_xor(wsum, o, 64);
    }
    auto bin = [](int t) { return t <= 8 ? t - 5 : t <= 12 ? 4 : t <= 20 ? 5 : t < 40 ? 6 : 7; };
    for (int b = 0; b < 8; ++b) {
      const unsigned long long mb = __builtin_amdgcn_ballot_w64(bin(trips) == b);
      if (first && mb) atomicAdd(&rs::g_bl_stats[32 + b], (unsigned long long)__builtin_popcountll(mb));
    }
    {
      const int nh = __builtin_popcountll(__builtin_amdgcn_ballot_w64(trips > 20));
      if (first && nh > 0) atomicAdd(&rs::g_bl_stats[40 + (nh == 1 ? 0 : nh <= 3 ? 1 : nh <= 7 ? 2 : nh <= 15 ? 3 : nh <= 31 ? 4 : 5)], 1ull);
    }
    if (first) {
      atomicAdd(&rs::g_bl_stats[9], (unsigned long long)wsum);
      atomicAdd(&rs::g_bl_stats[8], (unsigned long long)wmax);
      atomicAdd(&rs::g_bl_stats[24 + bin(wmax)], 1ull);
    }
  }
}
#endif

#ifdef RS_BL_LAST
__device__ __forceinline__ RS_REAL le_numerator(const MathTab &mt, RS_REAL tsurf, const ForcingPrep &q) {
  const RS_REAL as = (tsurf < 0) ? R4(21.875) : R4(17.269);
  const RS_REAL bs = (tsurf < 0) ? R4(265.5) : R4(237.3);
  const RS_REAL ESurf = R4(0.61078) * rs_exp(mt, rs_dv<false>(as * tsurf, tsurf + bs));
#ifdef RS_EAIR_SURFACE
  const RS_REAL EAir = air_vapour_pressure(mt, q.tair, q.rhz);
#else
  const RS_REAL EAir = q.EAir;
#endif
  return q.AirVCap * (ESurf - EAir);
}
__device__ __forceinline__ RS_REAL psychrometric(RS_REAL tair) {
  return R4(0.1) * (R4(0.00063) * (tair + R4(273.15)) + R4(0.47496));
}
#ifdef RS_BL_STATS
__device__ __forceinline__ void bl_last_count(bool dead, bool skip, bool all_warm, RS_REAL Stab) {
  const unsigned long long act = __builtin_amdgcn_ballot_w64(true), mu = __builtin_amdgcn_ballot_w64(!(Stab > R4(0.0)));
  if ((unsigned long long)__builtin_ctzll(act) == (unsigned long long)(threadIdx.x & 63u)) {
    if (dead) atomicAdd(&rs::g_bl_stats[53], 1ull);
    if (skip) atomicAdd(&rs::g_bl_stats[54], 1ull);
    if (skip && mu) atomicAdd(&rs::g_bl_stats[55], 1ull);
    if (all_warm) atomicAdd(&rs::g_bl_stats[56], 1ull);
  }
}
#endif

template <int TRIPS = 1>
__device__ __forceinline__ Fluxes model_step_fluxes_prepped(const RS_CONSTS &c, const MathTab &mt,
                                                            Scalars &s, const ForcingPrep &q,
                                                            const CouplingInputs &cp = CouplingInputs()) {
  Fluxes fx;
  s.wat = s.wat + q.rain;
  s.snow = s.snow + q.snow;
  fx.trffric = q.trffric;
  BlInv v;
  BlVar x;
  v.dT = s.tsurf - q.tair;
  v.den0 = q.den0;
  v.vkvz = q.vkvz;
  v.avk = q.avk;
  x.PSIM = R4(0.0);
  x.PSIH = R4(0.0);
  x.BLCond = 0.0;
  const RS_REAL stab_num = bl_stab_num(c);
  const RS_REAL raDen = c.VK_Const * c.VK_Const * q.vz;
  const bool dry = dry_tail_dry(s.wat, raDen);
  const bool warm = dry && dry_tail_warm_t(s.tsurf, q.tair);
  const bool all_warm = rs_wave_all(warm);
  RS_REAL N = R4(0.0);
  bool dead = true;
#ifdef RS_BL_STATS
  const bool need_n = true;
#else
  const bool need_n = !all_warm;
#endif
  if (need_n) {
    asm volatile("");
    N = le_numerator(mt, s.tsurf, q);
    dead = rs_wave_all(warm || (dry && rs_is_pos_normal(N) && dry_tail_psychc(psychrometric(q.tair))));
  }
  RS_REAL Stab = R4(0.0);
  int j = 1;
  bool unstable = false;
#ifdef RS_BL_STATS
  {
    const BlStatsStep st = bl_stats_step();
    for (; j <= RS_BL_MAXIT; ++j) {
      const RS_REAL h0 = x.PSIH;
      const bool done = bl_pass<false>(c, v, x, j, stab_num, Stab);
      bl_arm<false>(mt, Stab, x, TRIPS == 1 ? &unstable : nullptr);
      bl_stats_pass(st, j, h0, x);
      if (done) break;
    }
    bl_stats_trips(st, j);
  }
#else
  for (; j <= RS_BL_MAXIT; ++j) {
    if (j >= 2) bl_arm<false>(mt, Stab, x, TRIPS == 1 ? &unstable : nullptr);
    if (bl_pass<false>(c, v, x, j, stab_num, Stab)) break;
  }
  if (TRIPS == 1 && !(Stab > R4(0.0))) unstable = true;
#endif
  fx.trips = TRIPS == 1 ? j + (unstable ? 64 : 0) : TRIPS == 2 ? (j > RS_BL_MAXIT ? RS_BL_MAXIT : j) : 5;
  fx.blcond = x.BLCond;
  const bool skip = dead && rs_wave_all(Stab > c.stabSafe);
#ifdef RS_BL_STATS
  {
    const RS_REAL raNum = (c.logMom + x.PSIM) * (c.logHeat + x.PSIH);
    dry_tail_count(dry_tail_le(dry_tail_signs(s.wat, raNum, raDen), N, psychrometric(q.tair)), warm && (raNum > R4(0.0)));
    bl_last_count(dead, skip, all_warm, Stab);
  }
#endif
  if (skip) {
    fx.le = R4(0.0);
    fx.evap = R4(0.0);
  } else {
    asm volatile("");
#ifndef RS_BL_STATS
    bl_arm<false>(mt, Stab, x);
#endif
    const RS_REAL raNum = (c.logMom + x.PSIM) * (c.logHeat + x.PSIH);
    if (!need_n) N = le_numerator(mt, s.tsurf, q);
    const RS_REAL WatDen = R4(-0.0050) * s.tsurf * s.tsurf + R4(0.0079) * s.tsurf + R4(1000.0028);
    RS_REAL RAero = rs_dvb<false>(raNum, raDen);
    if (RAero > R4(30.0)) RAero = R4(30.);
    fx.le = rs_dvb<false>(N, psychrometric(q.tair) * RAero);
    const RS_REAL lvap = c.LVap, lfus = c.LFus;
    const RS_REAL lat = (s.tsurf >= R4(0.0)) ? lvap : lfus;
    fx.evap = rs_dvb<false>(fx.le, lat * WatDen) * R4(1000.0) * c.DTSecs;
    if ((fx.le > R4(0.0)) && (s.wat <= R4(0.0))) {
      fx.le = R4(0.0);
      fx.evap = R4(0.0);
    }
  }
#if RS_BL_GUARD && !defined(RS_IEEE_DIV) && !defined(RS_DIV_CHECK) && !defined(RS_NO_BL_GUARD) && !defined(RS_BL_FIXUP)
  if (!(rs_fabs(fx.blcond) < __builtin_inf()) || !(rs_fabs(fx.le) < __builtin_inf())) {
    const BlOut o = boundary_layer_ieee(&c, mt.expT, mt.logT, mt.K, s.tsurf, q.tair, q.vz, q.rhz, s.wat);
    fx.blcond = o.blcond;
    fx.le = o.le;
    fx.evap = o.evap;
  }
#endif
  fluxes_post(c, s, q.sw, q.lw, cp, fx);
  return fx;
}
#else
template <int TRIPS = 1>
__device__ __forceinline__ Fluxes model_step_fluxes_prepped(const RS_CONSTS &c, const MathTab &mt,
                                                            Scalars &s, const ForcingPrep &q,
                                                            const CouplingInputs &cp = CouplingInputs()) {
  Fluxes fx;
  s.wat = s.wat + q.rain;
  s.snow = s.snow + q.snow;
  fx.trffric = q.trffric;
  BlInv v;
  BlVar x;
  BlAux a;
  a.PsychC = q.PsychC;
#ifndef RS_DRY_TAIL
  const RS_REAL WatDen = R4(-0.0050) * s.tsurf * s.tsurf + R4(0.0079) * s.tsurf + R4(1000.0028);
#endif
  v.dT = s.tsurf - q.tair;
  v.den0 = q.den0;
  v.vkvz = q.vkvz;
  v.avk = q.avk;
#ifdef RS_EXP_STAB_CHAIN
  v.kinv = rs_div((RS_REAL)1.0, v.den0 * (v.vkvz * v.vkvz * v.vkvz));
#endif
  x.PSIM = R4(0.0);
  x.PSIH = R4(0.0);
  x.BLCond = 0.0;
  const RS_REAL stab_num = bl_stab_num(c);
  int j = 1;
  bool unstable = false;
#ifdef RS_BL_STATS
  {
    const BlStatsStep st = bl_stats_step();
    for (; j <= RS_BL_MAXIT; ++j) {
      const RS_REAL h0 = x.PSIH;
      const bool done = bl_iteration<false>(c, mt, v, x, j, stab_num, TRIPS == 1 ? &unstable : nullptr);
      bl_stats_pass(st, j, h0, x);
      if (done) break;
    }
    bl_stats_trips(st, j);
  }
#else
#ifdef RS_EXP_PIPE1
  const RS_REAL as_ = (s.tsurf < 0) ? R4(21.875) : R4(17.269);
  const RS_REAL bs_ = (s.tsurf < 0) ? R4(265.5) : R4(237.3);
  const RS_REAL ESurf_ = R4(0.61078) * rs_exp(mt, rs_dv<false>(as_ * s.tsurf, s.tsurf + bs_));
  (void)bl_iteration<false>(c, mt, v, x, 1, stab_num, TRIPS == 1 ? &unstable : nullptr);
  j = 2;
#endif
  for (; j <= RS_BL_MAXIT; ++j)
    if (bl_iteration<false>(c, mt, v, x, j, stab_num, TRIPS == 1 ? &unstable : nullptr)) break;
#endif
  fx.trips = TRIPS == 1 ? j + (unstable ? 64 : 0) : TRIPS == 2 ? (j > RS_BL_MAXIT ? RS_BL_MAXIT : j) : 5;
  fx.blcond = x.BLCond;
  do {
    const RS_REAL raNum = (c.logMom + x.PSIM) * (c.logHeat + x.PSIH), raDen = c.VK_Const * c.VK_Const * q.vz;
#ifdef RS_DRY_TAIL
    const bool signs = dry_tail_signs(s.wat, raNum, raDen);
#endif
#ifdef RS_DRY_ESURF
#ifdef RS_EAIR_SURFACE
    const bool warm = signs && dry_tail_warm_t(s.tsurf, q.tair);
#else
    const bool warm = dry_tail_warm(signs, s.tsurf, q.tair, q.EAir);
#endif
#ifndef RS_BL_STATS
    if (rs_wave_all(warm)) {
      fx.le = R4(0.0);
      fx.evap = R4(0.0);
      break;
    }
#endif
#endif
    const RS_REAL as = (s.tsurf < 0) ? R4(21.875) : R4(17.269);
    const RS_REAL bs = (s.tsurf < 0) ? R4(265.5) : R4(237.3);
#ifdef RS_EXP_SURFACE_LIGHT
    const RS_REAL ESurf = R4(0.61078) + (as + bs) * R4(0.0001) * s.tsurf;
#elif defined(RS_EXP_PIPE1)
    const RS_REAL ESurf = ESurf_;
    (void)as; (void)bs;
#else
    const RS_REAL ESurf = R4(0.61078) * rs_exp(mt, rs_dv<false>(as * s.tsurf, s.tsurf + bs));
#endif
#ifdef RS_EAIR_SURFACE
    const RS_REAL EAir = air_vapour_pressure(mt, q.tair, q.rhz);
#else
    const RS_REAL EAir = q.EAir;
#endif
    const RS_REAL N = q.AirVCap * (ESurf - EAir);
#ifdef RS_DRY_TAIL
    const bool le_dry = dry_tail_le(signs, N, a.PsychC);
#if defined(RS_BL_STATS) && defined(RS_DRY_ESURF)
    dry_tail_count(le_dry, warm);
#endif
    if (rs_wave_all(le_dry)) {
      fx.le = R4(0.0);
      fx.evap = R4(0.0);
      break;
    }
    asm volatile("");
    const RS_REAL WatDen = R4(-0.0050) * s.tsurf * s.tsurf + R4(0.0079) * s.tsurf + R4(1000.0028);
#endif
    RS_REAL RAero = rs_dvb<false>(raNum, raDen);
    if (RAero > R4(30.0)) RAero = R4(30.);
    fx.le = rs_dvb<false>(N, a.PsychC * RAero);
    const RS_REAL lvap = c.LVap, lfus = c.LFus;
    const RS_REAL lat = (s.tsurf >= R4(0.0)) ? lvap : lfus;
    fx.evap = rs_dvb<false>(fx.le, lat * WatDen) * R4(1000.0) * c.DTSecs;
    if ((fx.le > R4(0.0)) && (s.wat <= R4(0.0))) {
      fx.le = R4(0.0);
      fx.evap = R4(0.0);
    }
  } while (false);
#if RS_BL_GUARD && !defined(RS_IEEE_DIV) && !defined(RS_DIV_CHECK) && !defined(RS_NO_BL_GUARD) && !defined(RS_BL_FIXUP)
  if (!(rs_fabs(fx.blcond) < __builtin_inf()) || !(rs_fabs(fx.le) < __builtin_inf())) {
    const BlOut o = boundary_layer_ieee(&c, mt.expT, mt.logT, mt.K, s.tsurf, q.tair, q.vz, q.rhz, s.wat);
    fx.blcond = o.blcond;
    fx.le = o.le;
    fx.evap = o.evap;
  }
#endif
  fluxes_post(c, s, q.sw, q.lw, cp, fx);
  return fx;
}
#endif

__device__ __forceinline__ RS_REAL layer_step(const RS_CONSTS &c, int j, RS_REAL tj, RS_REAL tstale,
                                              RS_REAL tnext, RS_REAL &Gprev, RS_REAL *hs1) {
#ifdef RS_FROZEN_TABLE
  RS_REAL ncap;
  const unsigned long long thawed = __builtin_amdgcn_ballot_w64(tstale >= 0);
#ifdef RS_EXP_SURFACE_LIGHT
  if (j <= 2) {
    ncap = -RS_LK(c, j, capDZF);
    if (hs1) *hs1 = c.hs1F;
  } else
#endif
  if (thawed == 0ull) {
    ncap = -RS_LK(c, j, capDZF);
    if (hs1) *hs1 = c.hs1F;
  } else {
    const RS_REAL vsh = layer_vsh(c, j, tstale, thawed == __builtin_amdgcn_ballot_w64(true));
    if (hs1) *hs1 = RS_DIVC(vsh * c.HSfac1, c.twoDT, r_twoDT);
    ncap = rs_div((RS_REAL)1.0, RS_LK(c, j, DyC) * vsh);
  }
  const RS_REAL G = RS_LK(c, j, condDZ) * (tnext - tj);
  const RS_REAL tn = tj + c.DTSecs * (-ncap * (G - Gprev));
#else
  const RS_REAL vsh = layer_vsh(c, j, tstale);
  if (hs1) *hs1 = RS_DIVC(vsh * c.HSfac1, c.twoDT, r_twoDT);
  const RS_REAL capDZ = -rs_div((RS_REAL)1.0, RS_LK(c, j, DyC) * vsh);
  const RS_REAL G = RS_LK(c, j, condDZ) * (tnext - tj);
  const RS_REAL tn = tj + c.DTSecs * (capDZ * (G - Gprev));
#endif
  Gprev = G;
  return tn;
}

template <class Prof, class Stale = Prof, bool DEPTH = true>
__device__ __forceinline__ void model_step_ground(const RS_CONSTS &c, Scalars &s, Prof &T,
                                                  RS_REAL tbot, RS_REAL tair, const Fluxes &fx,
                                                  RS_REAL depth_i,
                                                  const CouplingInputs &cp = CouplingInputs(),
                                                  const Stale *stale_all = nullptr) {
  const int N = T.nlayers();
  const RS_REAL t1old = T.get(1), t2old = T.get(2);
  const RS_REAL Sens = fx.blcond * (tair - t1old);
  RS_REAL Gprev = fx.rnet - fx.le + fx.trffric + Sens;
  RS_REAL hs1 = 0.0;
  const RS_CONSTS *cl = &c;
#pragma unroll
  for (int j = 1; j <= N; ++j) {
    if (Prof::kUnrolled && RS_LAYER_GROUP > 0 && j > 1 && (j - 1) % RS_LAYER_GROUP == 0)
      asm volatile("" : "+s"(cl));
    const RS_REAL tj = T.get(j);
    const RS_REAL tstale = stale_all ? stale_all->get(j) : (j == 1) ? s.tnw1 : (j == 2) ? s.tnw2 : tj;
    const RS_REAL tnext = (j == N) ? tbot : T.get(j + 1);
    T.set(j, layer_step(*cl, j, tj, tstale, tnext, Gprev, (j == 1) ? &hs1 : nullptr));
  }
  T.pin();

  const RS_REAL T1Ave = (t1old + R4(3.) * t2old) / R4(4.);
  const RS_REAL TN1Ave = (T.get(1) + R4(3.) * T.get(2)) / R4(4.);
  const RS_REAL hstor = hs1 * (TN1Ave - T1Ave);

  melting(s, T, hstor, hs1, cp.in_phase, cp.last_tsurf_obs);

  s.tnw1 = T.get(1);
  s.tnw2 = T.get(2);
  if (DEPTH) {
    const RS_REAL depth = (c.tsurfOutputDepth >= R4(0.0)) ? c.tsurfOutputDepth : depth_i;
    s.tsurf = surface_temperature(c, T, tbot, depth);
  } else {
    s.tsurf = (T.get(1) + T.get(2)) / R4(2.0);
  }

  road_condition(c, s, fx.evap);
}

__device__ __forceinline__ bool check_values(const RS_CONSTS &c, const Forcing &f, RS_REAL tsurf,
                                             bool has_tdew) {
  const RS_REAL hi100 = rs_fmax(f.tair, f.vz);
  const RS_REAL lo01 = rs_fmin(rs_fmin(f.rhz, f.sw), rs_fmin(f.lw, f.prec));
  bool bad = (hi100 > RS_CHK(c, 0, R4(100.0))) | (lo01 < RS_CHK(c, 1, R4(-0.1))) |
             (f.tair < RS_CHK(c, 2, R4(-90.0))) | (f.rhz > RS_CHK(c, 3, R4(120.0))) |
             (f.vz < RS_CHK(c, 4, R4(-1.0))) | (f.sw > RS_CHK(c, 5, R4(4000.0))) |
             (f.lw > RS_CHK(c, 6, R4(1000.0))) | (f.prec > RS_CHK(c, 7, R4(500.0)));
  if (has_tdew) bad = bad | (f.tdew < -90) | (f.tdew > R4(100.0));
  bad = bad | (rs_fabs(tsurf) > RS_CHK(c, 0, R4(100.0)));
  return bad;
}

}
```

Baseline: 26.08 billion.

## Cut register pressure across duo step, forecast keys and counting-sort kernels

In the lean (non-FULL) two-wave step kernel, several forcing fields are now read late from LDS mail instead of being held in registers, the ground temperature exchange is read late, and tbottom is loaded per step. The failed flag is double-buffered, and the lean launch-bounds wave count rises from 4 to 5. The forecast key kernel moves mode-digit parsing to the host and reorders its state loads. The counting-sort kernels switch to 32-bit tile-relative indexing with smaller batch and row counts. The goal is lower VGPR use and higher occupancy, at the cost of extra LDS and global reloads on each step.

```diff
diff --git a/roadsurf_amd/csrc/rs_cluster.hip b/roadsurf_amd/csrc/rs_cluster.hip
--- a/roadsurf_amd/csrc/rs_cluster.hip
+++ b/roadsurf_amd/csrc/rs_cluster.hip
@@ -1109,15 +1109,20 @@
                                                       int nbins, int ntiles, uint32_t *__restrict__ H) {
   __builtin_amdgcn_s_setprio(3);
   extern __shared__ uint32_t cs_h[];
+#pragma unroll 1
   for (int b = threadIdx.x; b < nbins; b += 256) cs_h[b] = 0u;
   __syncthreads();
   const int64_t base = (int64_t)blockIdx.x * CS_TILE;
-  for (int i = threadIdx.x; i < CS_TILE; i += 256) {
-    const int64_t idx = base + i;
-    if (idx < n) atomicAdd(&cs_h[(keys[via ? (int64_t)via[idx] : idx] >> shift) & (uint32_t)(nbins - 1)], 1u);
-  }
+  const int64_t left = n - base;
+  const uint32_t cnt = left < CS_TILE ? (uint32_t)left : (uint32_t)CS_TILE;
+  const uint32_t *vt = via ? via + base : nullptr;
+#pragma unroll
+  for (uint32_t i = threadIdx.x; i < (uint32_t)CS_TILE; i += 256)
+    if (i < cnt) atomicAdd(&cs_h[(keys[vt ? (int64_t)vt[i] : base + i] >> shift) & (uint32_t)(nbins - 1)], 1u);
   __syncthreads();
-  for (int b = threadIdx.x; b < nbins; b += 256) H[(int64_t)blockIdx.x * nbins + b] = cs_h[b];
+  uint32_t *Ht = H + (int64_t)blockIdx.x * nbins;
+#pragma unroll 1
+  for (int b = threadIdx.x; b < nbins; b += 256) Ht[b] = cs_h[b];
 }
 
 __global__ void __launch_bounds__(64) cs_binscan_kernel(uint32_t *H, uint32_t *T, int nbins, int ntiles,
@@ -1154,7 +1159,7 @@
   const uint32_t lane = threadIdx.x;
   const int64_t base = (int64_t)blockIdx.x * CS_TILE;
   {
-    constexpr int ROWS = 16;
+    constexpr int ROWS = 8;
     uint32_t carry = 0u;
     for (int r0 = 0; r0 < nbins; r0 += 64 * ROWS) {
       uint32_t tv[ROWS], hv[ROWS];
@@ -1174,24 +1179,26 @@
     }
   }
   __syncthreads();
-  constexpr int CS_BATCH = 8;
+  constexpr int CS_BATCH = 4;
+  const int64_t left = n - base;
+  const uint32_t cnt = left < CS_TILE ? (uint32_t)left : (uint32_t)CS_TILE;
+  const uint32_t *vt = via ? via + base : nullptr;
   for (int r0 = 0; r0 < CS_TILE / 64; r0 += CS_BATCH) {
-    if (base + (int64_t)r0 * 64 >= n) break;
+    if ((uint32_t)r0 * 64u >= cnt) break;
     uint32_t kreg[CS_BATCH], sreg[CS_BATCH];
 #pragma unroll
     for (int q = 0; q < CS_BATCH; ++q) {
-      const int64_t idx = base + (int64_t)(r0 + q) * 64 + lane;
-      sreg[q] = (idx < n && via) ? via[idx] : (uint32_t)idx;
+      const uint32_t off = (uint32_t)(r0 + q) * 64u + lane;
+      sreg[q] = (off < cnt && vt) ? vt[off] : (uint32_t)base + off;
     }
 #pragma unroll
     for (int q = 0; q < CS_BATCH; ++q) {
-      const int64_t idx = base + (int64_t)(r0 + q) * 64 + lane;
-      kreg[q] = idx < n ? ((keys[sreg[q]] >> shift) & (uint32_t)(nbins - 1)) : 0u;
+      const uint32_t off = (uint32_t)(r0 + q) * 64u + lane;
+      kreg[q] = off < cnt ? ((keys[sreg[q]] >> shift) & (uint32_t)(nbins - 1)) : 0u;
     }
 #pragma unroll
   for (int q = 0; q < CS_BATCH; ++q) {
-    const int64_t idx = base + (int64_t)(r0 + q) * 64 + lane;
-    const bool valid = idx < n;
+    const bool valid = (uint32_t)(r0 + q) * 64u + lane < cnt;
     const uint32_t key = kreg[q];
     unsigned long long same = __ballot(valid);
     for (int bit = 0; bit < nbits; ++bit) {
diff --git a/roadsurf_amd/csrc/rs_kernels.h b/roadsurf_amd/csrc/rs_kernels.h
--- a/roadsurf_amd/csrc/rs_kernels.h
+++ b/roadsurf_amd/csrc/rs_kernels.h
@@ -66,6 +66,8 @@
   int32_t compact;
   int32_t low_bits;
   int32_t extra_log;
+  uint64_t mode_digits;
+  int32_t mode_ndigits, mode_ground;
 };
 
 struct KnotArgs {
diff --git a/roadsurf_amd/csrc/rs_kernels.hip b/roadsurf_amd/csrc/rs_kernels.hip
--- a/roadsurf_amd/csrc/rs_kernels.hip
+++ b/roadsurf_amd/csrc/rs_kernels.hip
@@ -532,7 +532,7 @@
 template <int NPREP>
 struct DuoMailT {
   double v[2][2][64];
-  uint32_t failed[64];
+  uint32_t failed[2][64];
   double prep[2][NPREP][64];
   uint32_t prep_bad[2][64];
 };
@@ -553,19 +553,35 @@
   if (FULL) w[PR_OBS][lane] = q.tsurfobs;
   mail.prep_bad[buf][lane] = (q.bad ? 1u : 0u) | (q.night ? 2u : 0u) | (q.bad_rw ? 8u : 0u);
 }
-template <bool FULL, bool SKYG = false, class C, class Mail>
-__device__ __forceinline__ ForcingPrep duo_get_prep(const C &c, const Mail &mail, int buf, uint32_t lane,
-                                                    const uint32_t *skyfl = nullptr) {
+struct DuoLatePrep : ForcingPrep {
+  const double (*w)[64];
+  uint32_t lane;
+  __device__ __forceinline__ double rhz_late() const { return w[PR_RHZ][lane]; }
+  __device__ __forceinline__ double vz_late() const { return w[PR_VZ][lane]; }
+  __device__ __forceinline__ double sw_late() const { return w[PR_SW][lane]; }
+  __device__ __forceinline__ double lw_late() const { return w[PR_LW][lane]; }
+};
+template <bool FULL, bool SKYG = false, bool LATE = false, class C, class Mail>
+__device__ __forceinline__ auto duo_get_prep(const C &c, const Mail &mail, int buf, uint32_t lane,
+                                             const uint32_t *skyfl = nullptr) {
   const double (*w)[64] = mail.prep[buf];
-  ForcingPrep q;
-  q.tair = w[PR_TAIR][lane]; q.vz = w[PR_VZ][lane]; q.rhz = w[PR_RHZ][lane]; q.rain = w[PR_RAIN][lane];
+  typename std::conditional<LATE, DuoLatePrep, ForcingPrep>::type q;
+  if constexpr (LATE) {
+    q.w = w;
+    q.lane = lane;
+  }
+  q.tair = w[PR_TAIR][lane]; q.vz = w[PR_VZ][lane]; q.rain = w[PR_RAIN][lane];
+  if (!LATE) q.rhz = w[PR_RHZ][lane];
   q.snow = w[PR_SNOW][lane];
   const double AirVCap = w[PR_AVC][lane];
   q.AirVCap = AirVCap;
 #ifndef RS_EAIR_SURFACE
   q.EAir = w[PR_EAIR][lane];
 #endif
-  q.sw = w[PR_SW][lane]; q.lw = w[PR_LW][lane];
+  if (!LATE) {
+    q.sw = w[PR_SW][lane];
+    q.lw = w[PR_LW][lane];
+  }
   if (FULL) q.tsurfobs = w[PR_OBS][lane];
   uint32_t flags = mail.prep_bad[buf][lane];
   if (SKYG) flags |= skyfl[buf * 64 + lane];
@@ -596,6 +612,7 @@
   static_assert(!(SKY && SKYG), "the sky view is this wave's or the ground wave's");
   static_assert(FULL || !CPL, "coupling belongs to the FULL feature set");
   static_assert(CPL || !REPLAY, "replays belong to coupling");
+  constexpr bool LATE = !FULL;
   KernArgs ka = kernargs();
   const uint32_t ml = threadIdx.x & 63u;
   const int64_t listed = REPLAY ? (int64_t)blockIdx.x * 64 + ml : 0;
@@ -644,12 +661,11 @@
   }
   double r_swcof = R4(1.0), r_lwcof = R4(1.0);
   mail.v[0][0][ml] = T.get(2);
-  mail.failed[ml] = (s.failed || (CPL && (parked || t0 != next_i))) ? 1u : 0u;
+  mail.failed[0][ml] = (s.failed || (CPL && (parked || t0 != next_i))) ? 1u : 0u;
   duo_meet();
   auto fail_at = [&](int32_t idx) {
     s.failed = true;
     ka->state[(int64_t)RS_ST_FAILED * ka->np_pad + row0 + lane] = (double)idx;
-    mail.failed[ml] = 1u;
   };
   auto blank_rows = [&](int32_t i_from) {
     for (int32_t ii = i_from; ii < t0 + nsteps; ++ii) {
@@ -680,14 +696,14 @@
     int64_t orow = orow_next;
     bool owrite = owait == 0;
     if (OUTIDX) owrite = output_row<true>(ka, i, orow);
-    double t3 = mail.v[k & 1][1][ml];
+    double t3 = LATE ? 0.0 : mail.v[k & 1][1][ml];
     bool go = true;
     if (CPL) {
       go = !(parked || i != next_i);
       if (go) next_i = i + 1;
     }
     if (go && !s.failed) {
-      const ForcingPrep q = duo_get_prep<FULL, SKYG>(c, mail, k & 1, ml, skyfl);
+      const auto q = duo_get_prep<FULL, SKYG, LATE>(c, mail, k & 1, ml, skyfl);
       if (i < c.SimLen) {
         const bool rewind = REPLAY && i == cpl_cs;
         if ((rewind ? q.bad_rw : q.bad) | check_values_tsurf(c, s.tsurf)) fail_at(rewind ? cpl_ce + 1 : i);
@@ -741,7 +757,7 @@
         }
       }
       const double tair = q.tair;
-      ForcingPrep qs = q;
+      auto qs = q;
       if (SKY) {
         const int64_t row = (int64_t)k * ka->f.t_stride + row0;
         const LaneOff L(lane);
@@ -767,6 +783,7 @@
       } else if (k == nsteps - 1) {
         score = fx.trips;
       }
+      if (LATE) t3 = mail.v[k & 1][1][ml];
       model_step_ground<RegProfile<2>, RegProfile<2>, false>(c, s, T, t3, tair, fx, R4(-9999.9), cp);
       if (owrite) {
         if (OUTIDX && ka->out_index) store_outputs<true, false>(ka, orow, row0, lane, s, true);
@@ -776,7 +793,7 @@
       if (CPL && cpl_on && i < c.SimLen && i == cpl_ce)
         cpl_window_end(ka->state, ka->np_pad, row0 + lane, cw, s, cpl_swcorr, cpl_lwcorr, cpl_lastobs, parked);
     }
-    if (CPL) mail.failed[ml] = (s.failed || parked || (i + 1) != next_i) ? 1u : 0u;
+    mail.failed[(k & 1) ^ 1][ml] = (s.failed || (CPL && (parked || (i + 1) != next_i))) ? 1u : 0u;
     mail.v[(k & 1) ^ 1][0][ml] = T.get(2);
     if (!OUTIDX) {
       if (owrite) {
@@ -792,6 +809,9 @@
   if (live) {
     double *st = a.state;
     const int64_t np = a.np_pad;
+    uint32_t le = ml;
+    if (LATE) asm volatile("" : "+v"(le));
+    const int64_t p = LATE ? row0 + le : row0 + lane;
     st[(int64_t)(RS_ST_TMP0 + 0) * np + p] = T.get(1);
     st[(int64_t)(RS_ST_TMP0 + 1) * np + p] = T.get(2);
     st[(int64_t)RS_ST_TNW1 * np + p] = s.tnw1;
@@ -813,7 +833,7 @@
 template <bool FULL>
 struct KnotLerp {
   double v0[FULL ? 7 : 6], dv[FULL ? 7 : 6];
-  int32_t ph0, ph1;
+  int32_t ph1;
   int32_t spk, k, r, hour, night;
   double span, r_spk;
 };
@@ -836,6 +856,7 @@
 __device__ __forceinline__ Forcing knot_forcing(KernArgs ka, int64_t col, bool live, KnotLerp<FULL> &K,
                                                 int32_t &kcur, int32_t i) {
   const int32_t k = K.k, r = K.r;
+  int32_t ph0 = 0;
   if (k != kcur) {
     kcur = k;
     const ConstsAS &c = consts_of(ka);
@@ -853,8 +874,8 @@
       const double v1 = (live && has_b) ? kb_[(int64_t)fld[q] * np] : K.v0[q];
       K.dv[q] = v1 - K.v0[q];
     }
-    K.ph0 = live ? (int32_t)ka_[8 * np] : 0;
-    K.ph1 = (live && has_b) ? (int32_t)kb_[8 * np] : K.ph0;
+    ph0 = live ? (int32_t)ka_[8 * np] : 0;
+    K.ph1 = (live && has_b) ? (int32_t)kb_[8 * np] : ph0;
   }
   const int32_t spk = FULL ? ka->spk : K.spk;
   const double secs = (double)r, span = FULL ? (double)spk : K.span, r_spk = FULL ? ka->r_spk : K.r_spk;
@@ -865,7 +886,7 @@
   f.prec = K.v0[3] + rs_div_u(secs * K.dv[3], span, r_spk);
   f.sw = K.v0[4] + rs_div_u(secs * K.dv[4], span, r_spk);
   f.lw = K.v0[5] + rs_div_u(secs * K.dv[5], span, r_spk);
-  f.phase = (r == 0) ? K.ph0 : K.ph1;
+  f.phase = (r == 0) ? ph0 : K.ph1;
   f.hour = K.hour;
   f.tdew = 0.0;
   f.tsurfobs = R4(-9999.9);
@@ -1101,7 +1122,8 @@
   double Tg[NL - 2];
 #pragma unroll
   for (int j = 3; j <= NL; ++j) Tg[j - 3] = live ? a.state[(int64_t)(RS_ST_TMP0 + j - 1) * a.np_pad + p] : 0.0;
-  const double tbot = live ? ka->pp.tbottom[p] : 0.0;
+  constexpr bool LATE = !FULL;
+  const double tbot = (live && !LATE) ? ka->pp.tbottom[p] : 0.0;
   mail.v[0][1][ml] = Tg[0];
   const int32_t nsteps = ka->nsteps, t0 = ka->t0;
   int32_t initlen = 0;
@@ -1193,7 +1215,9 @@
   };
   Forcing nxt = Forcing();
   int32_t kcur = -1;
-  const int64_t kcol = (KNOTS && live) ? (ka->knot_gather ? (int64_t)ka->knot_gather[p] : p) : 0;
+  const int32_t kcol32 = (KNOTS && LATE && live) ? (ka->knot_gather ? ka->knot_gather[p] : (int32_t)lane) : 0;
+  const int64_t kcol0 = (KNOTS && LATE && !ka->knot_gather) ? row0 : 0;
+  const int64_t kcol = LATE ? 0 : (KNOTS && live) ? (ka->knot_gather ? (int64_t)ka->knot_gather[p] : p) : 0;
   constexpr int FSET = SKYG ? FSET_GROUND : FSET_ALL;
   RawLerp<raw_nfields(FSET)> rlerp;
   const int64_t rcol = rcol_;
@@ -1209,7 +1233,7 @@
     const ConstsAS &c0 = consts_of(ka);
     if (KNOTS) {
       knot_begin<FULL>(ka, klerp, t0);
-      nxt = knot_forcing<FULL>(ka, kcol, live, klerp, kcur, t0);
+      nxt = knot_forcing<FULL>(ka, LATE ? kcol0 + kcol32 : kcol, live, klerp, kcur, t0);
     } else if (RAW) nxt = raw_forcing<FSET>(ka, rcol, live, rejected, rlerp, t0, obs_wanted(c0, t0));
     else if (live) nxt = load_forcing<FULL, true>(ka, row0, lane, 0);
     duo_put_prep<FULL, SKYG>(mail, 0, ml, prep(c0, nxt, t0, obs_cur));
@@ -1221,7 +1245,8 @@
     const int32_t k = __builtin_amdgcn_readfirstlane(kv);
     if (!KNOTS && !RAW && k + 1 < nsteps && live) nxt = load_forcing<FULL, true>(ka, row0, lane, k + 1);
     double t2 = mail.v[k & 1][0][ml];
-    if (REPLAY && !mail.failed[ml] && t0 + k == cpl_cs && t0 + k < c.SimLen && live) {
+    const double tbot_k = !LATE ? tbot : live ? LaneOff(lane).ld(ka->pp.tbottom + row0) : 0.0;
+    if (REPLAY && !mail.failed[k & 1][ml] && t0 + k == cpl_cs && t0 + k < c.SimLen && live) {
       const double *sv = ka->state + (int64_t)RS_ST_CPL_SAVE_TMP0 * ka->np_pad + p;
       const int64_t np = ka->np_pad;
       double cur = sv[(int64_t)2 * np];
@@ -1234,7 +1259,7 @@
         cur = tnext;
       }
     } else
-    if (!mail.failed[ml]) {
+    if (!mail.failed[k & 1][ml]) {
       if (CPL && !REPLAY && t0 + k == cpl_cs && t0 + k < c.SimLen && live) {
 #pragma unroll
         for (int j = 3; j <= NL; ++j) ka->state[(int64_t)(RS_ST_CPL_SAVE_TMP0 + j - 1) * ka->np_pad + p] = Tg[j - 3];
@@ -1252,7 +1277,7 @@
 #pragma unroll
       for (int j = 3; j <= NL; ++j) {
         const double tj = Tg[j - 3];
-        const double tnext = (j == NL) ? tbot : Tg[j - 2];
+        const double tnext = (j == NL) ? tbot_k : Tg[j - 2];
         Tg[j - 3] = layer_step(c, j, tj, tj, tnext, Gprev, nullptr);
       }
     }
@@ -1260,15 +1285,18 @@
     mail.v[(k & 1) ^ 1][1][ml] = Tg[0];
     if (k + 1 < nsteps) {
       const int32_t in = t0 + k + 1;
-      if (KNOTS) nxt = knot_forcing<FULL>(ka, kcol, live, klerp, kcur, in);
+      if (KNOTS) nxt = knot_forcing<FULL>(ka, LATE ? kcol0 + kcol32 : kcol, live, klerp, kcur, in);
       if (RAW) nxt = raw_forcing<FSET>(ka, rcol, live, rejected, rlerp, in, obs_wanted(c, in));
       duo_put_prep<FULL, SKYG>(mail, (k & 1) ^ 1, ml, prep(c, nxt, in, obs_cur));
     }
     duo_meet();
   }
   if (live) {
+    uint32_t le = ml;
+    if (LATE) asm volatile("" : "+v"(le));
+    const int64_t pe = LATE ? row0 + le : p;
 #pragma unroll
-    for (int j = 3; j <= NL; ++j) a.state[(int64_t)(RS_ST_TMP0 + j - 1) * a.np_pad + p] = Tg[j - 3];
+    for (int j = 3; j <= NL; ++j) a.state[(int64_t)(RS_ST_TMP0 + j - 1) * a.np_pad + pe] = Tg[j - 3];
   }
 }
 
@@ -1322,7 +1350,7 @@
 template <int NL, bool SCORE, int SRC = SRC_WINDOW, bool FULL = false, bool SKY = false, bool CPL = false,
           bool REPLAY = false>
 #ifndef RS_DUO_LEAN_WAVES
-#define RS_DUO_LEAN_WAVES 4
+#define RS_DUO_LEAN_WAVES 5
 #endif
 __global__ void __launch_bounds__((SKY && SRC == SRC_RAW) ? 192 : 128, REPLAY ? 3 : FULL ? 4 : RS_DUO_LEAN_WAVES) step_kernel_duo(const StepArgs a) {
   static_assert(!CPL || SRC == SRC_RAW, "coupling in the two-wavefront flavour: the driver path's lock-step chunks");
@@ -1597,25 +1625,23 @@
 
 __global__ void __launch_bounds__(kBlock) forecast_key_kernel(const ForecastArgs a) {
   __builtin_amdgcn_s_setprio(3);
-  const int64_t s = (int64_t)blockIdx.x * kBlock + threadIdx.x;
-  if (s >= a.npoints) return;
+  const uint32_t s = blockIdx.x * (uint32_t)kBlock + threadIdx.x;
+  if ((int64_t)s >= a.npoints) return;
   const ConstsAS &c = consts_of(&a);
   const int64_t np = a.np_pad;
-  auto st = [&](int row) -> double {
-    return a.f32 ? (double)((const float *)a.state)[(int64_t)row * np + s]
-                 : ((const double *)a.state)[(int64_t)row * np + s];
+  auto st_at = [&](int row, uint32_t slot) -> double {
+    return a.f32 ? (double)((const float *)a.state)[(int64_t)row * np + slot]
+                 : ((const double *)a.state)[(int64_t)row * np + slot];
   };
-  const double ts_now = st(RS_ST_TSURF);
-  const bool has_snow = st(RS_ST_SNOW) > 0.0, has_ice = st(RS_ST_ICE) > 0.0 || st(RS_ST_ICE2) > 0.0,
-             has_wet = st(RS_ST_WAT) > 0.0 || st(RS_ST_DEP) > 0.0;
-  const int32_t cover = (has_snow || has_ice || has_wet) ? 1 : 0;
-  const int32_t sclass = has_snow ? 3 : has_ice ? 2 : has_wet ? 1 : 0;
-  const int64_t pq = a.pv.index ? (int64_t)a.pv.index[s] : s;
+  auto st = [&](int row) -> double { return st_at(row, s); };
+  const uint32_t pq = a.pv.index ? (uint32_t)a.pv.index[s] : s;
+  auto preview_at = [&](const double *const *row, const double *const *row_b, int q, uint32_t col) -> double {
+    const double v = row[q][col];
+    return row_b[q] ? v + a.pv.w[q] * (row_b[q][col] - v) : v;
+  };
   auto preview = [&](const double *const *row, const double *const *row_b, int q) -> double {
-    const double v = row[q][pq];
-    return row_b[q] ? v + a.pv.w[q] * (row_b[q][pq] - v) : v;
+    return preview_at(row, row_b, q, pq);
   };
-  const double ta_now = a.pv.tair_now ? a.pv.tair_now[pq] : preview(a.pv.tair, a.pv.tair_b, 0);
   const double stab_num = -c.VK_Const * c.ZRefT * c.Grav;
   int32_t unst = 0, farc = 0, extra = 0, maxtrip = 5;
   float stab_lo = 2.f, stab_hi = -2.f;
@@ -1625,9 +1651,14 @@
     const double hour = (double)a.pv.hour[q];
     const double calm = (hour >= c.NightOn || hour <= c.NightOff) ? c.CalmLimNgt : c.CalmLimDay;
     if (vz < calm) vz = calm;
+    uint32_t sl = s, pl = pq;
+    asm volatile("" : "+v"(sl), "+v"(pl));
+    const double ts_now = st_at(RS_ST_TSURF, sl);
+    const double ta_now = a.pv.tair_now ? a.pv.tair_now[pl] : preview_at(a.pv.tair, a.pv.tair_b, 0, pl);
     const double ts = ts_now + a.pv.alpha * (ta - ta_now);
     const double TaK = ta + R4(273.15);
     const double dens = R4(100000.0) / (R4(287.05) * TaK);
+    __builtin_amdgcn_sched_barrier(0);
     const double hcap = R4(1005.0) + (TaK - R4(250.0)) * (TaK - R4(250.0)) / R4(3364.);
     const double avc = hcap * dens;
     const float dT = (float)(ts - ta), den0 = (float)(avc * TaK), vkvz = (float)(c.VK_Const * vz),
@@ -1635,6 +1666,7 @@
                 lC = (float)c.logCond;
     float psim = 0.f, psih = 0.f, bl = 0.f, stab_last = 0.f;
     int32_t nnear = 0, nfar = 0, j = 1;
+#pragma nounroll
     for (; j <= RS_BL_MAXIT; ++j) {
       const float old = bl;
       const float us = vkvz * __builtin_amdgcn_rcpf(lU + psim);
@@ -1664,6 +1696,10 @@
     }
   }
   if (a.extra_log && stab_hi >= 1.f && stab_lo < 1.f) maxtrip = 31;
+  const bool has_snow = st(RS_ST_SNOW) > 0.0, has_ice = st(RS_ST_ICE) > 0.0 || st(RS_ST_ICE2) > 0.0,
+             has_wet = st(RS_ST_WAT) > 0.0 || st(RS_ST_DEP) > 0.0;
+  const int32_t cover = (has_snow || has_ice || has_wet) ? 1 : 0;
+  const int32_t sclass = has_snow ? 3 : has_ice ? 2 : has_wet ? 1 : 0;
   if (a.extra_log) {
     const double last = st(RS_ST_BLSCORE);
     if (last >= 5.0 && last <= (double)RS_BL_MAXIT) {
@@ -1674,10 +1710,7 @@
   if (extra > 4095) extra = 4095;
   uint32_t ground = 0u;
   {
-    int32_t m9 = a.pv.mode;
-    bool want = false;
-    for (; m9 > 0; m9 /= 10) want |= (m9 % 10) == 9;
-    if (want) {
+    if (a.mode_ground) {
       const int NL = c.NLayers;
       int32_t deepest = 0, first = 0;
       for (int j = NL; j >= 1; --j)
@@ -1690,14 +1723,10 @@
       ground = ((uint32_t)deepest << 3) | (uint32_t)(top > 7 ? 7 : top);
     }
   }
-  int32_t m = a.pv.mode;
-  m = (m == 0) ? 14 : (m == 1) ? 124 : (m == 2) ? 134 : (m == 3) ? 1234 : m;
-  int32_t div = 1;
-  while (m / div >= 10) div *= 10;
   uint32_t key = 0;
   int bits = 0;
-  for (; div >= 1; div /= 10) {
-    const int d = (m / div) % 10;
+  for (int t = a.mode_ndigits - 1; t >= 0; --t) {
+    const int d = (int)((a.mode_digits >> (4 * t)) & 15u);
     if (d == 1) { key = (key << 4) | (uint32_t)unst; bits += 4; }
     else if (d == 2) { key = (key << 4) | (uint32_t)farc; bits += 4; }
     else if (d == 3) { key = (key << 1) | (uint32_t)cover; bits += 1; }
@@ -1796,7 +1825,20 @@
   return bits;
 }
 
-hipError_t rs_launch_forecast_keys(const rs::ForecastArgs &a, hipStream_t stream) {
+hipError_t rs_launch_forecast_keys(const rs::ForecastArgs &a_, hipStream_t stream) {
+  rs::ForecastArgs a = a_;
+  {
+    int32_t m = a.pv.mode;
+    a.mode_ground = 0;
+    for (int32_t m9 = m; m9 > 0; m9 /= 10) a.mode_ground |= (m9 % 10) == 9;
+    m = (m == 0) ? 14 : (m == 1) ? 124 : (m == 2) ? 134 : (m == 3) ? 1234 : m;
+    a.mode_digits = 0;
+    a.mode_ndigits = 0;
+    for (; m > 0; m /= 10) {
+      a.mode_digits |= (uint64_t)(m % 10) << (4 * a.mode_ndigits);
+      ++a.mode_ndigits;
+    }
+  }
   hipLaunchKernelGGL(rs::forecast_key_kernel, grid_for(a.npoints), dim3(RS_BLOCK), 0, stream, a);
   return hipGetLastError();
 }
diff --git a/roadsurf_amd/csrc/rs_physics_body.inc b/roadsurf_amd/csrc/rs_physics_body.inc
--- a/roadsurf_amd/csrc/rs_physics_body.inc
+++ b/roadsurf_amd/csrc/rs_physics_body.inc
@@ -653,6 +653,10 @@
   bool stop = false;
   bool bad_rw = false;
   RS_REAL tsurfobs = R4(-9999.9);
+  __device__ __forceinline__ RS_REAL rhz_late() const { return rhz; }
+  __device__ __forceinline__ RS_REAL vz_late() const { return vz; }
+  __device__ __forceinline__ RS_REAL sw_late() const { return sw; }
+  __device__ __forceinline__ RS_REAL lw_late() const { return lw; }
 };
 
 __device__ __forceinline__ bool check_values_forcing(const RS_CONSTS &c, const Forcing &f) {
@@ -819,12 +823,13 @@
 #endif
 
 #ifdef RS_BL_LAST
-__device__ __forceinline__ RS_REAL le_numerator(const MathTab &mt, RS_REAL tsurf, const ForcingPrep &q) {
+template <class Q>
+__device__ __forceinline__ RS_REAL le_numerator(const MathTab &mt, RS_REAL tsurf, const Q &q) {
   const RS_REAL as = (tsurf < 0) ? R4(21.875) : R4(17.269);
   const RS_REAL bs = (tsurf < 0) ? R4(265.5) : R4(237.3);
   const RS_REAL ESurf = R4(0.61078) * rs_exp(mt, rs_dv<false>(as * tsurf, tsurf + bs));
 #ifdef RS_EAIR_SURFACE
-  const RS_REAL EAir = air_vapour_pressure(mt, q.tair, q.rhz);
+  const RS_REAL EAir = air_vapour_pressure(mt, q.tair, q.rhz_late());
 #else
   const RS_REAL EAir = q.EAir;
 #endif
@@ -845,9 +850,9 @@
 }
 #endif
 
-template <int TRIPS = 1>
+template <int TRIPS = 1, class Q = ForcingPrep>
 __device__ __forceinline__ Fluxes model_step_fluxes_prepped(const RS_CONSTS &c, const MathTab &mt,
-                                                            Scalars &s, const ForcingPrep &q,
+                                                            Scalars &s, const Q &q,
                                                             const CouplingInputs &cp = CouplingInputs()) {
   Fluxes fx;
   s.wat = s.wat + q.rain;
@@ -935,19 +940,19 @@
   }
 #if RS_BL_GUARD && !defined(RS_IEEE_DIV) && !defined(RS_DIV_CHECK) && !defined(RS_NO_BL_GUARD) && !defined(RS_BL_FIXUP)
   if (!(rs_fabs(fx.blcond) < __builtin_inf()) || !(rs_fabs(fx.le) < __builtin_inf())) {
-    const BlOut o = boundary_layer_ieee(&c, mt.expT, mt.logT, mt.K, s.tsurf, q.tair, q.vz, q.rhz, s.wat);
+    const BlOut o = boundary_layer_ieee(&c, mt.expT, mt.logT, mt.K, s.tsurf, q.tair, q.vz_late(), q.rhz_late(), s.wat);
     fx.blcond = o.blcond;
     fx.le = o.le;
     fx.evap = o.evap;
   }
 #endif
-  fluxes_post(c, s, q.sw, q.lw, cp, fx);
+  fluxes_post(c, s, q.sw_late(), q.lw_late(), cp, fx);
   return fx;
 }
 #else
-template <int TRIPS = 1>
+template <int TRIPS = 1, class Q = ForcingPrep>
 __device__ __forceinline__ Fluxes model_step_fluxes_prepped(const RS_CONSTS &c, const MathTab &mt,
-                                                            Scalars &s, const ForcingPrep &q,
+                                                            Scalars &s, const Q &q,
                                                             const CouplingInputs &cp = CouplingInputs()) {
   Fluxes fx;
   s.wat = s.wat + q.rain;
@@ -1027,7 +1032,7 @@
     const RS_REAL ESurf = R4(0.61078) * rs_exp(mt, rs_dv<false>(as * s.tsurf, s.tsurf + bs));
 #endif
 #ifdef RS_EAIR_SURFACE
-    const RS_REAL EAir = air_vapour_pressure(mt, q.tair, q.rhz);
+    const RS_REAL EAir = air_vapour_pressure(mt, q.tair, q.rhz_late());
 #else
     const RS_REAL EAir = q.EAir;
 #endif
@@ -1058,13 +1063,13 @@
   } while (false);
 #if RS_BL_GUARD && !defined(RS_IEEE_DIV) && !defined(RS_DIV_CHECK) && !defined(RS_NO_BL_GUARD) && !defined(RS_BL_FIXUP)
   if (!(rs_fabs(fx.blcond) < __builtin_inf()) || !(rs_fabs(fx.le) < __builtin_inf())) {
-    const BlOut o = boundary_layer_ieee(&c, mt.expT, mt.logT, mt.K, s.tsurf, q.tair, q.vz, q.rhz, s.wat);
+    const BlOut o = boundary_layer_ieee(&c, mt.expT, mt.logT, mt.K, s.tsurf, q.tair, q.vz_late(), q.rhz_late(), s.wat);
     fx.blcond = o.blcond;
     fx.le = o.le;
     fx.evap = o.evap;
   }
 #endif
-  fluxes_post(c, s, q.sw, q.lw, cp, fx);
+  fluxes_post(c, s, q.sw_late(), q.lw_late(), cp, fx);
   return fx;
 }
 #endif
```

After: 26.60 billion, median of 6. 1.02x the previous value.
